# sangminwoo/SVOL

Hardware: AMD Instinct MI355X
Metric: frames/sec (fwd+matcher+bwd), T=32·P=196·d=256 (higher is better)
Workload: dtype bf16

## Files before the change

### svol_amd/csrc/attention_bf16.hip

```cpp
#include <cstdint>
#include <cstdlib>

#include "attn_call.h"

namespace {

constexpr float LOG2E = 1.4426950408889634f;
constexpr int KT = 128;
constexpr int IMG = KT * 64;
constexpr float LAZY_THR = 4.0f;

struct Args {
    const void *q, *k, *v, *o, *d_o;
    void *out_o, *dq, *dk, *dv;
    const float* kbias;
    float *lse2, *delta;
    int64_t ldq, ldk, ldv, ldo, lddo, lddq, lddk, lddv;
    int B, H, Lq, Lk, dh;
    float scale;
    float premul;
    int ksplit, tiles_per_split;
    float *ws_o, *ws_ml, *ws_dq;
    const int* tile_flags;
    int head_xcd, nxt;
    int tail_last;
    int* redo;
    unsigned *nl2, *nd2;
    float drop_p, drop_inv;
    uint64_t drop_seed;
    const int64_t* drop_step;
    int dq_rot;
};
__device__ __forceinline__ float attn_drop(uint64_t seed, uint64_t row, int key, float p, float inv) {
    return dropout_scale(seed, row, (uint32_t)key, p, inv);
}
__device__ __forceinline__ void attn_drop2(uint32_t rowmix, int key0, uint32_t thr16, float inv, float& s0, float& s1) {
    const uint32_t bits = drop_bits(rowmix, (uint32_t)key0 >> 1);
    s0 = drop_pick(bits, 0u, thr16, inv);
    s1 = drop_pick(bits, 1u, thr16, inv);
}

typedef __attribute__((address_space(3))) h16x4* lds_bf16x4_ptr;

__device__ __forceinline__ int img_off(int row, int ch) { return row * 64 + ((ch ^ ((row >> 2) & 3)) << 4); }

struct Stage { uint4 v[2]; };

__device__ __forceinline__ void load_regs(Stage& s, const h16_t* g, int64_t ld, int row0, int limit, int dh, int tid) {
#pragma unroll
    for (int i = 0; i < 2; ++i) {
        const int c = tid + 256 * i, row = c >> 2, ch = c & 3;
        s.v[i] = (row0 + row < limit && ch * 8 < dh) ? *reinterpret_cast<const uint4*>(g + (int64_t)(row0 + row) * ld + ch * 8)
                                                      : make_uint4(0, 0, 0, 0);
    }
}
__device__ __forceinline__ void store_lds(char* img, const Stage& s, int tid) {
#pragma unroll
    for (int i = 0; i < 2; ++i) {
        const int c = tid + 256 * i, row = c >> 2, ch = c & 3;
        *reinterpret_cast<uint4*>(img + img_off(row, ch)) = s.v[i];
    }
}

typedef __attribute__((address_space(3))) void* lds_vptr;
typedef const __attribute__((address_space(1))) void* gbl_vptr;
__device__ __forceinline__ void dma_piece(char* img, const h16_t* g, int64_t ld, int row0, int piece, int lane) {
    const int row = 16 * piece + (lane >> 2);
    const int ch = (lane & 3) ^ ((lane >> 4) & 3);
    const h16_t* src = g + (int64_t)(row0 + row) * ld + ch * 8;
    __builtin_amdgcn_global_load_lds((gbl_vptr)src, (lds_vptr)(img + piece * 1024), 16, 0, 0);
}
__device__ __forceinline__ void dma_tile(char* img, const h16_t* g, int64_t ld, int row0, int wave, int lane) {
    dma_piece(img, g, ld, row0, 2 * wave, lane);
    dma_piece(img, g, ld, row0, 2 * wave + 1, lane);
}
__device__ __forceinline__ void dma_wait_all() { asm volatile("s_waitcnt vmcnt(0)" ::: "memory"); }
__device__ __forceinline__ void dma_piece_async(char* img, const h16_t* g, int64_t ld, int row0, int piece, int lane) {
    const int row = 16 * piece + (lane >> 2);
    const int ch = (lane & 3) ^ ((lane >> 4) & 3);
    const h16_t* src = g + (int64_t)(row0 + row) * ld + ch * 8;
    const unsigned dst = __builtin_amdgcn_readfirstlane((unsigned)(size_t)(lds_vptr)(img + piece * 1024));
    asm volatile("s_mov_b32 m0, %0\n\tglobal_load_lds_dwordx4 %1, off" ::"s"(dst), "v"(src) : "m0");
}
__device__ __forceinline__ void dma_tile_async(char* img, const h16_t* g, int64_t ld, int row0, int wave, int lane) {
    dma_piece_async(img, g, ld, row0, 2 * wave, lane);
    dma_piece_async(img, g, ld, row0, 2 * wave + 1, lane);
}

__device__ __forceinline__ void load_lane_block(uint4 (&out)[2], const h16_t* g, int64_t ld, int row, bool valid, int dh,
                                                int h) {
#pragma unroll
    for (int s = 0; s < 2; ++s) {
        const int d0 = (2 * s + h) * 8;
        out[s] = (valid && d0 < dh) ? *reinterpret_cast<const uint4*>(g + (int64_t)row * ld + d0) : make_uint4(0, 0, 0, 0);
    }
}

__device__ __forceinline__ void read_rows(uint4 (&a)[2], const char* img, int row, int h) {
#pragma unroll
    for (int s = 0; s < 2; ++s) a[s] = *reinterpret_cast<const uint4*>(img + img_off(row, 2 * s + h));
}

__device__ __forceinline__ void read_tr(uint4 (&a)[2], const char* img, int sub, int lane) {
    const int g = lane >> 4, i = lane & 15, q = i >> 2, p = i & 3, hh = g >> 1;
    const int ch = 2 * (g & 1) + (p >> 1), inner = 8 * (p & 1);
#pragma unroll
    for (int s = 0; s < 2; ++s) {
        const int r1 = 32 * sub + 16 * s + 4 * hh + q;
        const h16x4 lo = SVOL_DS_READ_TR16_H16((lds_bf16x4_ptr)(img + img_off(r1, ch) + inner));
        const h16x4 hi = SVOL_DS_READ_TR16_H16((lds_bf16x4_ptr)(img + img_off(r1 + 8, ch) + inner));
        a[s] = __builtin_bit_cast(uint4, __builtin_shufflevector(lo, hi, 0, 1, 2, 3, 4, 5, 6, 7));
    }
}

__device__ __forceinline__ float max3(float a, float b, float c) {
    float r;
    asm("v_max3_f32 %0, %1, %2, %3" : "=v"(r) : "v"(a), "v"(b), "v"(c));
    return r;
}

__device__ __forceinline__ void mfma_results_ready(f32x16& a, f32x16& b, f32x16& c, f32x16& d) {
    asm volatile("s_nop 15\n\ts_nop 3" : "+v"(a), "+v"(b), "+v"(c), "+v"(d));
}

__device__ __forceinline__ void mfma_results_ready2(f32x16& a, f32x16& b) {
    asm volatile("s_nop 15\n\ts_nop 3" : "+v"(a), "+v"(b));
}

__device__ __forceinline__ f32x16 zero16() {
    f32x16 z;
#pragma unroll
    for (int i = 0; i < 16; ++i) z[i] = 0.f;
    return z;
}

__device__ __forceinline__ f32x16 mma_first(const uint4 (&a)[2], const uint4 (&b)[2]) {
    f32x16 acc = zero16();
#pragma unroll
    for (int s = 0; s < 2; ++s)
        acc = SVOL_MFMA_32x32x16_H16(__builtin_bit_cast(h16x8, a[s]), __builtin_bit_cast(h16x8, b[s]), acc, 0, 0,
                                                      0);
    return acc;
}

__device__ __forceinline__ void mma_second(f32x16& acc, const uint4 (&a)[2], const f32x16& x) {
#pragma unroll
    for (int s = 0; s < 2; ++s) {
        h16x8 b;
#pragma unroll
        for (int j = 0; j < 8; j += 2) {
            const h16x2 pr = cvt_pk_h16(x[8 * s + j], x[8 * s + j + 1]);
            b[j] = pr[0];
            b[j + 1] = pr[1];
        }
        acc = SVOL_MFMA_32x32x16_H16(__builtin_bit_cast(h16x8, a[s]), b, acc, 0, 0, 0);
    }
}

__device__ __forceinline__ void store_acc(const f32x16& acc, h16_t* out, int64_t ld, int row, bool valid, int dh, int h,
                                          float mul) {
    if (!valid) return;
#pragma unroll
    for (int g = 0; g < 4; ++g) {
        const int d0 = 8 * g + 4 * h;
        if (d0 < dh) {
            h16x4 v;
#pragma unroll
            for (int e = 0; e < 4; ++e) v[e] = (h16_t)(acc[4 * g + e] * mul);
            *reinterpret_cast<h16x4*>(out + (int64_t)row * ld + d0) = v;
        }
    }
}

__device__ __forceinline__ void stage_bias(float* sb, const float* kb, int row0, int limit, int tid) {
    if (tid < KT) {
        const int key = row0 + tid;
        sb[tid] = key < limit ? (kb ? kb[key] * LOG2E : 0.f) : -INFINITY;
    }
}

template <bool MASKED>
__global__ __launch_bounds__(256, 2) void attn_fwd_bf16(Args p) {
    const uint64_t dseed = drop_seed_at(p.drop_seed, p.drop_step);
    __shared__ __attribute__((aligned(16))) char smem[4 * IMG + 2 * KT * 4];
    char* sK = smem;
    char* sV = smem + 2 * IMG;
    float* sB = reinterpret_cast<float*>(smem + 4 * IMG);

    const int tid = threadIdx.x, lane = tid & 63, wave = tid >> 6;
    const int r = lane & 31, h = lane >> 5;
    const int b = blockIdx.z, hh = blockIdx.y;
    const int qt = blockIdx.x / p.ksplit, sp = blockIdx.x % p.ksplit;
    const int qrow = qt * 128 + wave * 32 + r;
    const bool qvalid = qrow < p.Lq;
    const h16_t* Q = reinterpret_cast<const h16_t*>(p.q) + (int64_t)b * p.Lq * p.ldq + hh * p.dh;
    const h16_t* K = reinterpret_cast<const h16_t*>(p.k) + (int64_t)b * p.Lk * p.ldk + hh * p.dh;
    const h16_t* V = reinterpret_cast<const h16_t*>(p.v) + (int64_t)b * p.Lk * p.ldv + hh * p.dh;
    const float* kb = p.kbias ? p.kbias + (int64_t)b * p.Lk : nullptr;
    const float c = p.premul != 0.f ? 1.f : p.scale * LOG2E;

    uint4 qb[2];
    load_lane_block(qb, Q, p.ldq, qrow, qvalid, p.dh, h);

    float m = -INFINITY, l = 0.f;
    f32x16 O = zero16();

    const int t0 = sp * p.tiles_per_split;
    const int nt = min((p.Lk + KT - 1) / KT, t0 + p.tiles_per_split);
    Stage sk, sv;
    load_regs(sk, K, p.ldk, t0 * KT, p.Lk, p.dh, tid);
    load_regs(sv, V, p.ldv, t0 * KT, p.Lk, p.dh, tid);
    store_lds(sK, sk, tid);
    store_lds(sV, sv, tid);
    if (MASKED) stage_bias(sB, kb, t0 * KT, p.Lk, tid);
    __syncthreads();

    for (int t = t0; t < nt; ++t) {
        const int cur = (t - t0) & 1;
        if (t + 1 < nt) {
            load_regs(sk, K, p.ldk, (t + 1) * KT, p.Lk, p.dh, tid);
            load_regs(sv, V, p.ldv, (t + 1) * KT, p.Lk, p.dh, tid);
        }
        const char* kimg = sK + cur * IMG;
        const char* vimg = sV + cur * IMG;
        const float* bias = sB + cur * KT;
        f32x16 S[4];
#pragma unroll
        for (int sub = 0; sub < 4; ++sub) {
            uint4 ka[2];
            read_rows(ka, kimg, sub * 32 + r, h);
            S[sub] = mma_first(ka, qb);
        }
        mfma_results_ready(S[0], S[1], S[2], S[3]);
        if (MASKED) {
#pragma unroll
            for (int sub = 0; sub < 4; ++sub)
#pragma unroll
                for (int g = 0; g < 4; ++g) {
                    const f32x4 bb = *reinterpret_cast<const f32x4*>(bias + sub * 32 + 8 * g + 4 * h);
#pragma unroll
                    for (int e = 0; e < 4; ++e) S[sub][4 * g + e] = S[sub][4 * g + e] * c + bb[e];
                }
        }
        float ml[4];
#pragma unroll
        for (int sub = 0; sub < 4; ++sub) {
            float mm = max3(S[sub][0], S[sub][1], S[sub][2]);
#pragma unroll
            for (int i = 3; i < 15; i += 2) mm = max3(mm, S[sub][i], S[sub][i + 1]);
            ml[sub] = max3(mm, S[sub][15], mm);
        }
        float mloc = max3(ml[0], ml[1], fmaxf(ml[2], ml[3]));
        {
            const HalfPair sw = swap_halves(__builtin_bit_cast(unsigned, mloc));
            mloc = fmaxf(__builtin_bit_cast(float, sw.lo), __builtin_bit_cast(float, sw.hi));
        }
        const float thr = MASKED ? LAZY_THR : LAZY_THR / c;
        if (__any(mloc > m + thr)) {
            const float m_new = fmaxf(m, mloc);
            const float m_use = (m_new == -INFINITY) ? 0.f : m_new;
            const float alpha = __builtin_amdgcn_exp2f(MASKED ? (m - m_use) : (m - m_use) * c);
            l *= alpha;
#pragma unroll
            for (int i = 0; i < 16; ++i) O[i] *= alpha;
            m = m_new;
        }
        const float m_use = (m == -INFINITY) ? 0.f : m;
        const float mc = MASKED ? -m_use : -m_use * c;
        float ls[4] = {0.f, 0.f, 0.f, 0.f};
#pragma unroll
        for (int sub = 0; sub < 4; ++sub)
#pragma unroll
            for (int i = 0; i < 16; ++i) {
                S[sub][i] = __builtin_amdgcn_exp2f(MASKED ? S[sub][i] + mc : __builtin_fmaf(S[sub][i], c, mc));
                ls[sub] += S[sub][i];
            }
        l += (ls[0] + ls[1]) + (ls[2] + ls[3]);
        if (p.drop_p > 0.f) {
            const uint32_t rm = drop_row(drop_seed32(dseed), (((uint64_t)b * p.H + hh) * p.Lq + (qvalid ? qrow : 0)));
            const uint32_t thr = drop_thr16(p.drop_p);
#pragma unroll
            for (int sub = 0; sub < 4; ++sub)
#pragma unroll
                for (int g = 0; g < 4; ++g)
#pragma unroll
                    for (int e = 0; e < 4; e += 2) {
                        float s0, s1;
                        attn_drop2(rm, t * KT + sub * 32 + 8 * g + 4 * h + e, thr, p.drop_inv, s0, s1);
                        S[sub][4 * g + e] *= s0;
                        S[sub][4 * g + e + 1] *= s1;
                    }
        }
#pragma unroll
        for (int sub = 0; sub < 4; ++sub) {
            uint4 va[2];
            read_tr(va, vimg, sub, lane);
            mma_second(O, va, S[sub]);
        }
        if (t + 1 < nt) {
            store_lds(sK + (cur ^ 1) * IMG, sk, tid);
            store_lds(sV + (cur ^ 1) * IMG, sv, tid);
            if (MASKED) stage_bias(sB + (cur ^ 1) * KT, kb, (t + 1) * KT, p.Lk, tid);
        }
        __syncthreads();
    }
    const float lt = l + __shfl_xor(l, 32, 64);
    const float m2 = MASKED ? m : m * c;
    if (p.ksplit > 1) {
        if (qvalid) {
            float* wo = p.ws_o + (((int64_t)sp * p.B + b) * p.Lq + qrow) * (p.H * p.dh) + hh * p.dh;
#pragma unroll
            for (int g = 0; g < 4; ++g) {
                const int d0 = 8 * g + 4 * h;
                if (d0 < p.dh) *reinterpret_cast<f32x4*>(wo + d0) = f32x4{O[4 * g], O[4 * g + 1], O[4 * g + 2], O[4 * g + 3]};
            }
            if (h == 0) {
                float* wm = p.ws_ml + ((((int64_t)sp * p.B + b) * p.H + hh) * p.Lq + qrow) * 2;
                wm[0] = m2;
                wm[1] = lt;
            }
        }
        return;
    }
    const float inv = lt > 0.f ? 1.f / lt : 0.f;
    h16_t* Oo = reinterpret_cast<h16_t*>(p.out_o) + (int64_t)b * p.Lq * p.ldo + hh * p.dh;
    store_acc(O, Oo, p.ldo, qrow, qvalid, p.dh, h, inv);
    if (qvalid && h == 0) p.lse2[((int64_t)b * p.H + hh) * p.Lq + qrow] = m2 + __builtin_amdgcn_logf(lt);
}

__global__ void attn_combine_bf16(Args p) {
    const int64_t idx = (int64_t)blockIdx.x * blockDim.x + threadIdx.x;
    const int64_t total = (int64_t)p.B * p.Lq * p.H;
    if (idx >= total) return;
    const int hh = (int)(idx % p.H);
    const int64_t row = idx / p.H;
    const int b = (int)(row / p.Lq), q = (int)(row % p.Lq);
    float M = -INFINITY;
    for (int i = 0; i < p.ksplit; ++i) M = fmaxf(M, p.ws_ml[((((int64_t)i * p.B + b) * p.H + hh) * p.Lq + q) * 2]);
    float L = 0.f, acc[32];
#pragma unroll
    for (int d = 0; d < 32; ++d) acc[d] = 0.f;
    for (int i = 0; i < p.ksplit; ++i) {
        const float* ml = p.ws_ml + ((((int64_t)i * p.B + b) * p.H + hh) * p.Lq + q) * 2;
        if (ml[0] == -INFINITY) continue;
        const float w = __builtin_amdgcn_exp2f(ml[0] - M);
        L += w * ml[1];
        const float* po = p.ws_o + (((int64_t)i * p.B + b) * p.Lq + q) * (p.H * p.dh) + hh * p.dh;
#pragma unroll
        for (int d = 0; d < 32; d += 4) {
            if (d < p.dh) {
                const f32x4 t = *reinterpret_cast<const f32x4*>(po + d);
#pragma unroll
                for (int e = 0; e < 4; ++e) acc[d + e] += w * t[e];
            }
        }
    }
    const float inv = L > 0.f ? 1.f / L : 0.f;
    h16_t* o = reinterpret_cast<h16_t*>(p.out_o) + row * p.ldo + hh * p.dh;
#pragma unroll
    for (int d = 0; d < 32; d += 4) {
        if (d < p.dh) {
            h16x4 v;
#pragma unroll
            for (int e = 0; e < 4; ++e) v[e] = (h16_t)(acc[d + e] * inv);
            *reinterpret_cast<h16x4*>(o + d) = v;
        }
    }
    p.lse2[((int64_t)b * p.H + hh) * p.Lq + q] = M + __builtin_amdgcn_logf(L);
}

__global__ void attn_delta_bf16(Args p) {
    const int64_t idx = (int64_t)blockIdx.x * blockDim.x + threadIdx.x;
    const int64_t total = (int64_t)p.B * p.Lq * p.H;
    if (idx >= total) return;
    const int hh = (int)(idx % p.H);
    const int64_t row = idx / p.H;
    const int b = (int)(row / p.Lq), q = (int)(row % p.Lq);
    const h16_t* o = reinterpret_cast<const h16_t*>(p.o) + row * p.ldo + hh * p.dh;
    const h16_t* d = reinterpret_cast<const h16_t*>(p.d_o) + row * p.lddo + hh * p.dh;
    float s = 0.f;
    for (int i = 0; i < p.dh; i += 8) {
        const h16x8 a = *reinterpret_cast<const h16x8*>(o + i), c = *reinterpret_cast<const h16x8*>(d + i);
#pragma unroll
        for (int e = 0; e < 8; ++e) s += (float)a[e] * (float)c[e];
    }
    p.delta[((int64_t)b * p.H + hh) * p.Lq + q] = s;
    if (p.ksplit > 1) {
        float* z = p.ws_dq + row * (p.H * p.dh) + hh * p.dh;
        for (int i = 0; i < p.dh; i += 4) *reinterpret_cast<f32x4*>(z + i) = f32x4{0.f, 0.f, 0.f, 0.f};
    }
}

__global__ void attn_dq_finish_bf16(Args p) {
    const int64_t idx = (int64_t)blockIdx.x * blockDim.x + threadIdx.x;
    const int64_t total = (int64_t)p.B * p.Lq * p.H;
    if (idx >= total) return;
    const int hh = (int)(idx % p.H);
    const int64_t row = idx / p.H;
    const float* z = p.ws_dq + row * (p.H * p.dh) + hh * p.dh;
    h16_t* o = reinterpret_cast<h16_t*>(p.dq) + row * p.lddq + hh * p.dh;
    for (int i = 0; i < p.dh; i += 4) {
        const f32x4 t = *reinterpret_cast<const f32x4*>(z + i);
        h16x4 v;
#pragma unroll
        for (int e = 0; e < 4; ++e) v[e] = (h16_t)(t[e] * p.scale);
        *reinterpret_cast<h16x4*>(o + i) = v;
    }
}

template <bool MASKED>
__global__ __launch_bounds__(256, 2) void attn_bwd_dq_bf16(Args p) {
    const uint64_t dseed = drop_seed_at(p.drop_seed, p.drop_step);
    __shared__ __attribute__((aligned(16))) char smem[4 * IMG + 2 * KT * 4];
    char* sK = smem;
    char* sV = smem + 2 * IMG;
    float* sB = reinterpret_cast<float*>(smem + 4 * IMG);

    const int tid = threadIdx.x, lane = tid & 63, wave = tid >> 6;
    const int r = lane & 31, h = lane >> 5;
    const int b = blockIdx.z, hh = blockIdx.y;
    const int qt = blockIdx.x / p.ksplit, sp = blockIdx.x % p.ksplit;
    const int qrow = qt * 128 + wave * 32 + r;
    const bool qvalid = qrow < p.Lq;
    const h16_t* Q = reinterpret_cast<const h16_t*>(p.q) + (int64_t)b * p.Lq * p.ldq + hh * p.dh;
    const h16_t* dO = reinterpret_cast<const h16_t*>(p.d_o) + (int64_t)b * p.Lq * p.lddo + hh * p.dh;
    const h16_t* K = reinterpret_cast<const h16_t*>(p.k) + (int64_t)b * p.Lk * p.ldk + hh * p.dh;
    const h16_t* V = reinterpret_cast<const h16_t*>(p.v) + (int64_t)b * p.Lk * p.ldv + hh * p.dh;
    const float* kb = p.kbias ? p.kbias + (int64_t)b * p.Lk : nullptr;
    const float c = p.premul != 0.f ? 1.f : p.scale * LOG2E;

    uint4 qb[2], dob[2];
    load_lane_block(qb, Q, p.ldq, qrow, qvalid, p.dh, h);
    load_lane_block(dob, dO, p.lddo, qrow, qvalid, p.dh, h);
    const int64_t sidx = ((int64_t)b * p.H + hh) * p.Lq + qrow;
    const float nlse = qvalid ? -p.lse2[sidx] : -INFINITY;
    const float dl = qvalid ? p.delta[sidx] : 0.f;

    f32x16 dQ = zero16();
    const int t0 = sp * p.tiles_per_split;
    const int nt = min((p.Lk + KT - 1) / KT, t0 + p.tiles_per_split);
    Stage sk, sv;
    load_regs(sk, K, p.ldk, t0 * KT, p.Lk, p.dh, tid);
    load_regs(sv, V, p.ldv, t0 * KT, p.Lk, p.dh, tid);
    store_lds(sK, sk, tid);
    store_lds(sV, sv, tid);
    if (MASKED) stage_bias(sB, kb, t0 * KT, p.Lk, tid);
    __syncthreads();

    for (int t = t0; t < nt; ++t) {
        const int cur = (t - t0) & 1;
        if (t + 1 < nt) {
            load_regs(sk, K, p.ldk, (t + 1) * KT, p.Lk, p.dh, tid);
            load_regs(sv, V, p.ldv, (t + 1) * KT, p.Lk, p.dh, tid);
        }
        const char* kimg = sK + cur * IMG;
        const char* vimg = sV + cur * IMG;
        const float* bias = sB + cur * KT;
#pragma unroll 2
        for (int sub = 0; sub < 4; ++sub) {
            uint4 a[2];
            read_rows(a, kimg, sub * 32 + r, h);
            f32x16 S = mma_first(a, qb);
            read_rows(a, vimg, sub * 32 + r, h);
            f32x16 dP = mma_first(a, dob);
            if (p.drop_p > 0.f) {
                const uint32_t rm = drop_row(drop_seed32(dseed), (((uint64_t)b * p.H + hh) * p.Lq + (qvalid ? qrow : 0)));
                const uint32_t thr = drop_thr16(p.drop_p);
#pragma unroll
                for (int g = 0; g < 4; ++g)
#pragma unroll
                    for (int e = 0; e < 4; e += 2) {
                        float s0, s1;
                        attn_drop2(rm, t * KT + sub * 32 + 8 * g + 4 * h + e, thr, p.drop_inv, s0, s1);
                        dP[4 * g + e] *= s0;
                        dP[4 * g + e + 1] *= s1;
                    }
            }
            if (MASKED) {
#pragma unroll
                for (int g = 0; g < 4; ++g) {
                    const f32x4 bb = *reinterpret_cast<const f32x4*>(bias + sub * 32 + 8 * g + 4 * h);
#pragma unroll
                    for (int e = 0; e < 4; ++e) {
                        const float pe = __builtin_amdgcn_exp2f(__builtin_fmaf(S[4 * g + e], c, bb[e] + nlse));
                        S[4 * g + e] = pe * (dP[4 * g + e] - dl);
                    }
                }
            } else {
#pragma unroll
                for (int i = 0; i < 16; ++i) {
                    const float pe = __builtin_amdgcn_exp2f(__builtin_fmaf(S[i], c, nlse));
                    S[i] = pe * (dP[i] - dl);
                }
            }
            read_tr(a, kimg, sub, lane);
            mma_second(dQ, a, S);
        }
        if (t + 1 < nt) {
            store_lds(sK + (cur ^ 1) * IMG, sk, tid);
            store_lds(sV + (cur ^ 1) * IMG, sv, tid);
            if (MASKED) stage_bias(sB + (cur ^ 1) * KT, kb, (t + 1) * KT, p.Lk, tid);
        }
        __syncthreads();
    }
    if (p.ksplit > 1) {
        if (qvalid) {
            float* z = p.ws_dq + ((int64_t)b * p.Lq + qrow) * (p.H * p.dh) + hh * p.dh;
#pragma unroll
            for (int g = 0; g < 4; ++g) {
                const int d0 = 8 * g + 4 * h;
                if (d0 < p.dh) {
#pragma unroll
                    for (int e = 0; e < 4; ++e) atomicAdd(z + d0 + e, dQ[4 * g + e]);
                }
            }
        }
        return;
    }
    h16_t* dQo = reinterpret_cast<h16_t*>(p.dq) + (int64_t)b * p.Lq * p.lddq + hh * p.dh;
    store_acc(dQ, dQo, p.lddq, qrow, qvalid, p.dh, h, p.scale);
}

template <bool KBIAS>
__global__ __launch_bounds__(256, 2) void attn_bwd_dkdv_bf16(Args p) {
    const uint64_t dseed = drop_seed_at(p.drop_seed, p.drop_step);
    __shared__ __attribute__((aligned(16))) char smem[4 * IMG + 4 * KT * 4];
    char* sQ = smem;
    char* sdO = smem + 2 * IMG;
    float* sL = reinterpret_cast<float*>(smem + 4 * IMG);
    float* sD = sL + 2 * KT;

    const int tid = threadIdx.x, lane = tid & 63, wave = tid >> 6;
    const int r = lane & 31, h = lane >> 5;
    const int b = blockIdx.z, hh = blockIdx.y;
    const int krow = blockIdx.x * 128 + wave * 32 + r;
    const bool kvalid = krow < p.Lk;
    const h16_t* Q = reinterpret_cast<const h16_t*>(p.q) + (int64_t)b * p.Lq * p.ldq + hh * p.dh;
    const h16_t* dO = reinterpret_cast<const h16_t*>(p.d_o) + (int64_t)b * p.Lq * p.lddo + hh * p.dh;
    const h16_t* K = reinterpret_cast<const h16_t*>(p.k) + (int64_t)b * p.Lk * p.ldk + hh * p.dh;
    const h16_t* V = reinterpret_cast<const h16_t*>(p.v) + (int64_t)b * p.Lk * p.ldv + hh * p.dh;
    const float c = p.premul != 0.f ? 1.f : p.scale * LOG2E;
    const float kbl = kvalid ? (p.kbias ? p.kbias[(int64_t)b * p.Lk + krow] * LOG2E : 0.f) : -INFINITY;
    const float* lse_g = p.lse2 + ((int64_t)b * p.H + hh) * p.Lq;
    const float* dl_g = p.delta + ((int64_t)b * p.H + hh) * p.Lq;

    uint4 kbk[2], vbk[2];
    load_lane_block(kbk, K, p.ldk, krow, kvalid, p.dh, h);
    load_lane_block(vbk, V, p.ldv, krow, kvalid, p.dh, h);

    f32x16 dK = zero16(), dV = zero16();
    const int nt = (p.Lq + KT - 1) / KT;
    Stage sq, sdo;
    float rl = 0.f, rd = 0.f;
    auto load_stats = [&](int row0) {
        if (tid < KT) {
            const int qi = row0 + tid;
            rl = qi < p.Lq ? -lse_g[qi] : -INFINITY;
            rd = qi < p.Lq ? dl_g[qi] : 0.f;
        }
    };
    auto store_stats = [&](int buf) {
        if (tid < KT) { sL[buf * KT + tid] = rl; sD[buf * KT + tid] = rd; }
    };
    load_regs(sq, Q, p.ldq, 0, p.Lq, p.dh, tid);
    load_regs(sdo, dO, p.lddo, 0, p.Lq, p.dh, tid);
    load_stats(0);
    store_lds(sQ, sq, tid);
    store_lds(sdO, sdo, tid);
    store_stats(0);
    __syncthreads();

    for (int t = 0; t < nt; ++t) {
        const int cur = t & 1;
        if (t + 1 < nt) {
            load_regs(sq, Q, p.ldq, (t + 1) * KT, p.Lq, p.dh, tid);
            load_regs(sdo, dO, p.lddo, (t + 1) * KT, p.Lq, p.dh, tid);
            load_stats((t + 1) * KT);
        }
        const char* qimg = sQ + cur * IMG;
        const char* doimg = sdO + cur * IMG;
        const float* nl = sL + cur * KT;
        const float* dd = sD + cur * KT;
#pragma unroll 1
        for (int sub = 0; sub < 4; ++sub) {
            uint4 a[2];
            read_rows(a, qimg, sub * 32 + r, h);
            f32x16 S = mma_first(a, kbk);
#pragma unroll
            for (int g = 0; g < 4; ++g) {
                const f32x4 ls = *reinterpret_cast<const f32x4*>(nl + sub * 32 + 8 * g + 4 * h);
#pragma unroll
                for (int e = 0; e < 4; ++e)
                    S[4 * g + e] = __builtin_amdgcn_exp2f(__builtin_fmaf(S[4 * g + e], c, KBIAS ? kbl + ls[e] : ls[e]));
            }
            read_tr(a, doimg, sub, lane);
            f32x16 MS;
#pragma unroll
            for (int i = 0; i < 16; ++i) MS[i] = 1.f;
            if (p.drop_p > 0.f) {
                const uint32_t s0 = drop_seed32(dseed), thr = drop_thr16(p.drop_p), odd = (uint32_t)lane & 1u;
                const uint64_t rbase = ((uint64_t)b * p.H + hh) * p.Lq;
                const bool rows32 = rbase + (uint64_t)p.Lq <= 0xffffffffull;
#pragma unroll
                for (int g = 0; g < 4; ++g)
#pragma unroll
                    for (int e = 0; e < 4; e += 2) {
                        const int q0 = t * KT + sub * 32 + 8 * g + 4 * h + e;
                        const int qm = min(q0 + (int)odd, p.Lq - 1);
                        const uint32_t rm = rows32 ? (s0 ^ (((uint32_t)rbase + (uint32_t)qm) * 0x9E3779B1u)) : drop_row(s0, rbase + (uint64_t)qm);
                        const uint32_t mine = drop_bits(rm, (uint32_t)krow >> 1);
                        const uint32_t other = (uint32_t)__builtin_amdgcn_mov_dpp((int)mine, 0xB1, 0xf, 0xf, true);
                        MS[4 * g + e] = drop_pick(odd ? other : mine, odd, thr, p.drop_inv);
                        MS[4 * g + e + 1] = drop_pick(odd ? mine : other, odd, thr, p.drop_inv);
                    }
                f32x16 Pd = S;
#pragma unroll
                for (int i = 0; i < 16; ++i) Pd[i] *= MS[i];
                mma_second(dV, a, Pd);
            } else {
                mma_second(dV, a, S);
            }
            read_rows(a, doimg, sub * 32 + r, h);
            f32x16 dP = mma_first(a, vbk);
            if (p.drop_p > 0.f) {
#pragma unroll
                for (int i = 0; i < 16; ++i) dP[i] *= MS[i];
            }
#pragma unroll
            for (int g = 0; g < 4; ++g) {
                const f32x4 dl = *reinterpret_cast<const f32x4*>(dd + sub * 32 + 8 * g + 4 * h);
#pragma unroll
                for (int e = 0; e < 4; ++e) S[4 * g + e] = S[4 * g + e] * (dP[4 * g + e] - dl[e]);
            }
            read_tr(a, qimg, sub, lane);
            mma_second(dK, a, S);
        }
        if (t + 1 < nt) {
            store_lds(sQ + (cur ^ 1) * IMG, sq, tid);
            store_lds(sdO + (cur ^ 1) * IMG, sdo, tid);
            store_stats(cur ^ 1);
        }
        __syncthreads();
    }
    h16_t* dKo = reinterpret_cast<h16_t*>(p.dk) + (int64_t)b * p.Lk * p.lddk + hh * p.dh;
    h16_t* dVo = reinterpret_cast<h16_t*>(p.dv) + (int64_t)b * p.Lk * p.lddv + hh * p.dh;
    store_acc(dK, dKo, p.lddk, krow, kvalid, p.dh, h, p.premul != 0.f ? p.scale / p.premul : p.scale);
    store_acc(dV, dVo, p.lddv, krow, kvalid, p.dh, h, 1.f);
}

__device__ __forceinline__ f32x16 splat16(float x) {
    f32x16 z;
#pragma unroll
    for (int i = 0; i < 16; ++i) z[i] = x;
    return z;
}
__device__ __forceinline__ f32x16 mma_first_c(const uint4 (&a)[2], const uint4 (&b)[2], const f32x16& c0) {
    f32x16 acc;
    asm("s_nop 1\n\tv_mfma_f32_32x32x16_" SVOL_H16_ASM " %0, %1, %2, %3"
        : "=&v"(acc)
        : "v"(__builtin_bit_cast(h16x8, a[0])), "v"(__builtin_bit_cast(h16x8, b[0])), "v"(c0));
    return SVOL_MFMA_32x32x16_H16(__builtin_bit_cast(h16x8, a[1]), __builtin_bit_cast(h16x8, b[1]), acc, 0, 0,
                                                   0);
}
__device__ __forceinline__ f32x16 rows16(const float* v, int sub, int h) {
    f32x16 z;

#pragma unroll
    for (int g = 0; g < 4; ++g) {
        const f32x4 t = *reinterpret_cast<const f32x4*>(v + sub * 32 + 8 * g + 4 * h);
#pragma unroll
        for (int e = 0; e < 4; ++e) z[4 * g + e] = t[e];
    }
    return z;
}

__device__ __forceinline__ void block_coords(const Args& p, int& xt, int& hh, int& b) {
    if (p.head_xcd) {
        const int id = blockIdx.x, xcd = id & 7, slot = id >> 3;
        int hl;
        const int two = p.head_xcd == 2 ? 2 : 1;
        if (p.tail_last) {
            const int nfull = p.nxt - 1, hpx = (p.B * p.H) >> 3;
            if (slot < hpx * nfull) {
                const int g = slot / (two * nfull), r = slot - g * two * nfull;
                hl = g * two + (two == 2 ? (r & 1) : 0);
                xt = two == 2 ? (r >> 1) : r;
            } else { hl = slot - hpx * nfull; xt = nfull; }
        } else {
            const int g = slot / (two * p.nxt), r = slot - g * two * p.nxt;
            hl = g * two + (two == 2 ? (r & 1) : 0);
            xt = two == 2 ? (r >> 1) : r;
        }
        const int head = p.head_xcd == 2 ? (((hl >> 1) * 8 + xcd) * 2 + (hl & 1)) : hl * 8 + xcd;
        hh = head % p.H;
        b = head / p.H;
    } else {
        xt = blockIdx.x;
        hh = blockIdx.y;
        b = blockIdx.z;
    }
}

__device__ __forceinline__ unsigned split_bf16x2(float x) {
    const h16_t hi = (h16_t)x;
    const float rem = x - (float)hi;
    const h16_t lo = (h16_t)rem;
    return (unsigned)__builtin_bit_cast(unsigned short, hi) | ((unsigned)__builtin_bit_cast(unsigned short, lo) << 16);
}

__device__ __forceinline__ float key_bias_log2(const float* kb, int key, int Lk) {
    return key < Lk ? (kb ? kb[key] * LOG2E : 0.f) : -INFINITY;
}
__device__ __forceinline__ f32x16 add_key_bias(const f32x16& S, const float* kb, int key, int Lk, int h) {
    const float bv = key_bias_log2(kb, key, Lk);
    const unsigned pair = bv == -INFINITY ? SVOL_H16_NINF_LO : split_bf16x2(bv);
    const uint4 a = h == 0 ? make_uint4(pair, 0u, 0u, 0u) : make_uint4(0u, 0u, 0u, 0u);
    const uint4 o = h == 0 ? make_uint4(SVOL_H16_ONE2, 0u, 0u, 0u) : make_uint4(0u, 0u, 0u, 0u);
    return SVOL_MFMA_32x32x16_H16(__builtin_bit_cast(h16x8, a), __builtin_bit_cast(h16x8, o), S, 0, 0, 0);
}
__global__ __launch_bounds__(64) void attn_tile_flags_bf16(const float* __restrict__ kbias, int Lk, int nt, int* __restrict__ flags) {
    const int t = blockIdx.x, b = blockIdx.y, lane = threadIdx.x;
    const float* kb = kbias ? kbias + (int64_t)b * Lk : nullptr;
    const float b0 = key_bias_log2(kb, t * KT + lane, Lk), b1 = key_bias_log2(kb, t * KT + 64 + lane, Lk);
    int flag = 0;
    if (__any(b0 != 0.f || b1 != 0.f)) flag = __all(b0 == -INFINITY && b1 == -INFINITY) ? 2 : 1;
    if (lane == 0) flags[(int64_t)b * nt + t] = flag;
}

template <bool MASKED>
__device__ __forceinline__ void attn_fwd_pre_body(const Args p) {
    __shared__ __attribute__((aligned(16))) char smem[4 * IMG];
    char* sK = smem;
    char* sV = smem + 2 * IMG;
    const int tid = threadIdx.x, lane = tid & 63, wave = tid >> 6;
    const int r = lane & 31, h = lane >> 5;
    int xt, hh, b;
    block_coords(p, xt, hh, b);
    const int qrow = xt * 128 + wave * 32 + r;
    const bool qvalid = qrow < p.Lq;
    const h16_t* Q = reinterpret_cast<const h16_t*>(p.q) + (int64_t)b * p.Lq * p.ldq + hh * p.dh;
    const h16_t* K = reinterpret_cast<const h16_t*>(p.k) + (int64_t)b * p.Lk * p.ldk + hh * p.dh;
    const h16_t* V = reinterpret_cast<const h16_t*>(p.v) + (int64_t)b * p.Lk * p.ldv + hh * p.dh;
    const float* kb = (MASKED && p.kbias) ? p.kbias + (int64_t)b * p.Lk : nullptr;

    uint4 qb[2];
    load_lane_block(qb, Q, p.ldq, qrow, qvalid, p.dh, h);
    float m = 0.f, l = 0.f;
    f32x16 O = zero16();
    f32x16 Cm = zero16();
    bool started = false;

    const int nt = MASKED ? (p.Lk + KT - 1) / KT : p.Lk / KT;
    Stage sk, sv;
    load_regs(sk, K, p.ldk, 0, p.Lk, p.dh, tid);
    load_regs(sv, V, p.ldv, 0, p.Lk, p.dh, tid);
    const int* fl = MASKED ? p.tile_flags + (int64_t)b * nt : nullptr;
    unsigned long long mixed = 0, dead = 0;
    store_lds(sK, sk, tid);
    store_lds(sV, sv, tid);
    __syncthreads();
    for (int t = 0; t < nt; ++t) {
        const int cur = t & 1;
        if (t + 1 < nt) {
            load_regs(sk, K, p.ldk, (t + 1) * KT, p.Lk, p.dh, tid);
            load_regs(sv, V, p.ldv, (t + 1) * KT, p.Lk, p.dh, tid);
        }
        if (MASKED && (t & 63) == 0) {
            const int f = (t + lane < nt) ? fl[t + lane] : 2;
            mixed = __ballot(f == 1);
            dead = __ballot(f == 2);
        }
        const int flag = MASKED ? (int)((mixed >> (t & 63)) & 1) + 2 * (int)((dead >> (t & 63)) & 1) : 0;
        if (!MASKED || flag != 2) {
            const char* kimg = sK + cur * IMG;
            const char* vimg = sV + cur * IMG;
            f32x16 S[4];
#pragma unroll
            for (int sub = 0; sub < 4; ++sub) {
                uint4 ka[2];
                read_rows(ka, kimg, sub * 32 + r, h);
                S[sub] = mma_first_c(ka, qb, Cm);
            }
            if (MASKED && flag == 1) {
#pragma unroll
                for (int sub = 0; sub < 4; ++sub) S[sub] = add_key_bias(S[sub], kb, t * KT + sub * 32 + r, p.Lk, h);
            }
            mfma_results_ready(S[0], S[1], S[2], S[3]);
            float ml[4];
#pragma unroll
            for (int sub = 0; sub < 4; ++sub) {
                float mm = max3(S[sub][0], S[sub][1], S[sub][2]);
#pragma unroll
                for (int i = 3; i < 15; i += 2) mm = max3(mm, S[sub][i], S[sub][i + 1]);
                ml[sub] = max3(mm, S[sub][15], mm);
            }
            float mloc = max3(ml[0], ml[1], fmaxf(ml[2], ml[3]));
            {
                const HalfPair sw = swap_halves(__builtin_bit_cast(unsigned, mloc));
                mloc = fmaxf(__builtin_bit_cast(float, sw.lo), __builtin_bit_cast(float, sw.hi));
            }
            const bool first = MASKED ? !started : (t == 0);
            if (first || __any(mloc > LAZY_THR)) {
                const float dm = first ? mloc : fmaxf(mloc, 0.f);
                if (!first) {
                    const float alpha = __builtin_amdgcn_exp2f(-dm);
                    l *= alpha;
#pragma unroll
                    for (int i = 0; i < 16; ++i) O[i] *= alpha;
                }
                m += dm;
                Cm = splat16(-m);
#pragma unroll
                for (int sub = 0; sub < 4; ++sub)
#pragma unroll
                    for (int i = 0; i < 16; ++i) S[sub][i] -= dm;
            }
            started = true;
            float ls[4] = {0.f, 0.f, 0.f, 0.f};
#pragma unroll
            for (int sub = 0; sub < 4; ++sub)
#pragma unroll
                for (int i = 0; i < 16; ++i) {
                    S[sub][i] = __builtin_amdgcn_exp2f(S[sub][i]);
                    ls[sub] += S[sub][i];
                }
            l += (ls[0] + ls[1]) + (ls[2] + ls[3]);
#pragma unroll
            for (int sub = 0; sub < 4; ++sub) {
                uint4 va[2];
                read_tr(va, vimg, sub, lane);
                mma_second(O, va, S[sub]);
            }
        }
        if (t + 1 < nt) {
            store_lds(sK + (cur ^ 1) * IMG, sk, tid);
            store_lds(sV + (cur ^ 1) * IMG, sv, tid);
        }
        __syncthreads();
    }
    const float lt = l + __shfl_xor(l, 32, 64);
    const float inv = lt > 0.f ? 1.f / lt : 0.f;
    h16_t* Oo = reinterpret_cast<h16_t*>(p.out_o) + (int64_t)b * p.Lq * p.ldo + hh * p.dh;
    store_acc(O, Oo, p.ldo, qrow, qvalid, p.dh, h, inv);
    if (qvalid && h == 0) p.lse2[((int64_t)b * p.H + hh) * p.Lq + qrow] = m + __builtin_amdgcn_logf(lt);
}
__global__ __launch_bounds__(256, 2) void attn_fwd_bf16_pre(Args p) {
    __shared__ __attribute__((aligned(16))) char smem[4 * IMG];
    if (p.redo && !p.redo[blockIdx.x]) return;
    char* sK = smem;
    char* sV = smem + 2 * IMG;
    const int tid = threadIdx.x, lane = tid & 63, wave = tid >> 6;
    const int r = lane & 31, h = lane >> 5;
    int xt, hh, b;
    block_coords(p, xt, hh, b);
    const int qrow = xt * 128 + wave * 32 + r;
    const bool qvalid = qrow < p.Lq;
    const h16_t* Q = reinterpret_cast<const h16_t*>(p.q) + (int64_t)b * p.Lq * p.ldq + hh * p.dh;
    const h16_t* K = reinterpret_cast<const h16_t*>(p.k) + (int64_t)b * p.Lk * p.ldk + hh * p.dh;
    const h16_t* V = reinterpret_cast<const h16_t*>(p.v) + (int64_t)b * p.Lk * p.ldv + hh * p.dh;

    uint4 qb[2];
    load_lane_block(qb, Q, p.ldq, qrow, qvalid, p.dh, h);
    float m = 0.f, l = 0.f;
    f32x16 O = zero16();
    f32x16 Cm = zero16();

    const int nt = p.Lk / KT;
    Stage sk, sv;
    load_regs(sk, K, p.ldk, 0, p.Lk, p.dh, tid);
    load_regs(sv, V, p.ldv, 0, p.Lk, p.dh, tid);
    store_lds(sK, sk, tid);
    store_lds(sV, sv, tid);
    __syncthreads();
    for (int t = 0; t < nt; ++t) {
        const int cur = t & 1;
        if (t + 1 < nt) {
            load_regs(sk, K, p.ldk, (t + 1) * KT, p.Lk, p.dh, tid);
            load_regs(sv, V, p.ldv, (t + 1) * KT, p.Lk, p.dh, tid);
        }
        const char* kimg = sK + cur * IMG;
        const char* vimg = sV + cur * IMG;
        f32x16 S[4];
#pragma unroll
        for (int sub = 0; sub < 4; ++sub) {
            uint4 ka[2];
            read_rows(ka, kimg, sub * 32 + r, h);
            S[sub] = mma_first_c(ka, qb, Cm);
        }
        mfma_results_ready(S[0], S[1], S[2], S[3]);
        float ml[4];
#pragma unroll
        for (int sub = 0; sub < 4; ++sub) {
            float mm = max3(S[sub][0], S[sub][1], S[sub][2]);
#pragma unroll
            for (int i = 3; i < 15; i += 2) mm = max3(mm, S[sub][i], S[sub][i + 1]);
            ml[sub] = max3(mm, S[sub][15], mm);
        }
        float mloc = max3(ml[0], ml[1], fmaxf(ml[2], ml[3]));
        {
            const HalfPair sw = swap_halves(__builtin_bit_cast(unsigned, mloc));
            mloc = fmaxf(__builtin_bit_cast(float, sw.lo), __builtin_bit_cast(float, sw.hi));
        }
        if (t == 0 || __any(mloc > LAZY_THR)) {
            const float dm = (t == 0) ? mloc : fmaxf(mloc, 0.f);
            if (t != 0) {
                const float alpha = __builtin_amdgcn_exp2f(-dm);
                l *= alpha;
#pragma unroll
                for (int i = 0; i < 16; ++i) O[i] *= alpha;
            }
            m += dm;
            Cm = splat16(-m);
#pragma unroll
            for (int sub = 0; sub < 4; ++sub)
#pragma unroll
                for (int i = 0; i < 16; ++i) S[sub][i] -= dm;
        }
        float ls[4] = {0.f, 0.f, 0.f, 0.f};
#pragma unroll
        for (int sub = 0; sub < 4; ++sub)
#pragma unroll
            for (int i = 0; i < 16; ++i) {
                S[sub][i] = __builtin_amdgcn_exp2f(S[sub][i]);
                ls[sub] += S[sub][i];
            }
        l += (ls[0] + ls[1]) + (ls[2] + ls[3]);
#pragma unroll
        for (int sub = 0; sub < 4; ++sub) {
            uint4 va[2];
            read_tr(va, vimg, sub, lane);
            mma_second(O, va, S[sub]);
        }
        if (t + 1 < nt) {
            store_lds(sK + (cur ^ 1) * IMG, sk, tid);
            store_lds(sV + (cur ^ 1) * IMG, sv, tid);
        }
        __syncthreads();
    }
    const float lt = l + __shfl_xor(l, 32, 64);
    const float inv = lt > 0.f ? 1.f / lt : 0.f;
    h16_t* Oo = reinterpret_cast<h16_t*>(p.out_o) + (int64_t)b * p.Lq * p.ldo + hh * p.dh;
    store_acc(O, Oo, p.ldo, qrow, qvalid, p.dh, h, inv);
    if (qvalid && h == 0) p.lse2[((int64_t)b * p.H + hh) * p.Lq + qrow] = m + __builtin_amdgcn_logf(lt);
}
__global__ __launch_bounds__(256, 2) void attn_fwd_bf16_pre_masked(Args p) { attn_fwd_pre_body<true>(p); }

__device__ __forceinline__ f32x16 mma_c_first(const uint4& a0, const uint4& b0, const f32x16& c0) {
    f32x16 acc;
    asm("s_nop 1\n\tv_mfma_f32_32x32x16_" SVOL_H16_ASM " %0, %1, %2, %3"
        : "=&v"(acc)
        : "v"(__builtin_bit_cast(h16x8, a0)), "v"(__builtin_bit_cast(h16x8, b0)), "v"(c0));
    return acc;
}
__device__ __forceinline__ f32x16 mma_acc(const uint4& a1, const uint4& b1, const f32x16& acc) {
    return SVOL_MFMA_32x32x16_H16(__builtin_bit_cast(h16x8, a1), __builtin_bit_cast(h16x8, b1), acc, 0, 0, 0);
}
template <int LO>
__device__ __forceinline__ void ds_chunk(f32x16& S, const f32x16& dP) {
#pragma unroll
    for (int i = LO; i < LO + 4; i += 2) {
        const f32x2 e = {__builtin_amdgcn_exp2f(S[i]), __builtin_amdgcn_exp2f(S[i + 1])};
        const f32x2 d = {dP[i], dP[i + 1]};
        const f32x2 m = e * d;
        S[i] = m[0];
        S[i + 1] = m[1];
    }
}
#define SVOL_FENCE() __builtin_amdgcn_sched_barrier(0)
__device__ __forceinline__ void dq_phase(f32x16& Sn, f32x16& dPn, const uint4 (&ka)[2], const uint4 (&va)[2], const uint4 (&qbn)[2],
                                         const uint4 (&dobn)[2], const f32x16& Cln, const f32x16& Cdn, f32x16& Sc, const f32x16& dPc,
                                         f32x16& dQc, const uint4 (&kt)[2]) {
    Sn = mma_c_first(ka[0], qbn[0], Cln);
    SVOL_FENCE();
    ds_chunk<0>(Sc, dPc);
    SVOL_FENCE();
    Sn = mma_acc(ka[1], qbn[1], Sn);
    SVOL_FENCE();
    ds_chunk<4>(Sc, dPc);
    SVOL_FENCE();
    dPn = mma_c_first(va[0], dobn[0], Cdn);
    SVOL_FENCE();
    ds_chunk<8>(Sc, dPc);
    SVOL_FENCE();
    dPn = mma_acc(va[1], dobn[1], dPn);
    SVOL_FENCE();
    ds_chunk<12>(Sc, dPc);
    SVOL_FENCE();
    mma_second(dQc, kt, Sc);
}
__device__ __forceinline__ void dq_finish(f32x16& Sc, const f32x16& dPc, f32x16& dQc, const uint4 (&kt)[2]) {
    ds_chunk<0>(Sc, dPc);
    ds_chunk<4>(Sc, dPc);
    ds_chunk<8>(Sc, dPc);
    ds_chunk<12>(Sc, dPc);
    mma_second(dQc, kt, Sc);
}

template <bool MASKED>
__device__ __forceinline__ void attn_bwd_dq_pre_body(const Args& p) {
    __shared__ __attribute__((aligned(16))) char smem[4 * IMG];
    char* sK = smem;
    char* sV = smem + 2 * IMG;
    const int tid = threadIdx.x, lane = tid & 63, wave = tid >> 6;
// ... 126 lines not shown
    hh = __builtin_amdgcn_readfirstlane(hh);
    b = __builtin_amdgcn_readfirstlane(b);
    const h16_t* Q = reinterpret_cast<const h16_t*>(p.q) + (int64_t)b * p.Lq * p.ldq + hh * p.dh;
    const h16_t* dO = reinterpret_cast<const h16_t*>(p.d_o) + (int64_t)b * p.Lq * p.lddo + hh * p.dh;
    const h16_t* O = reinterpret_cast<const h16_t*>(p.o) + (int64_t)b * p.Lq * p.ldo + hh * p.dh;
    const h16_t* K = reinterpret_cast<const h16_t*>(p.k) + (int64_t)b * p.Lk * p.ldk + hh * p.dh;
    const h16_t* V = reinterpret_cast<const h16_t*>(p.v) + (int64_t)b * p.Lk * p.ldv + hh * p.dh;
    dma_tile(sK, K, p.ldk, 0, wave, lane);
    dma_tile(sV, V, p.ldv, 0, wave, lane);

    int qrow[2];
    bool qvalid[2];
    uint4 qb[2][2], dob[2][2];
    f32x16 Cl[2], Cd[2], dQ[2];
    const bool single = p.Lq - xt * 256 <= 128;
#pragma unroll
    for (int u = 0; u < 2; ++u) {
        qrow[u] = single ? (u == 0 ? xt * 256 + wave * 32 + r : p.Lq) : xt * 256 + wave * 64 + u * 32 + r;
        qvalid[u] = qrow[u] < p.Lq;
        load_lane_block(qb[u], Q, p.ldq, qrow[u], qvalid[u], p.dh, h);
        load_lane_block(dob[u], dO, p.lddo, qrow[u], qvalid[u], p.dh, h);
        const int64_t sidx = ((int64_t)b * p.H + hh) * p.Lq + qrow[u];
        Cl[u] = splat16(qvalid[u] ? -p.lse2[sidx] : -INFINITY);
        float dl = 0.f;
        {
            uint4 ob[2];
            load_lane_block(ob, O, p.ldo, qrow[u], qvalid[u], p.dh, h);
#pragma unroll
            for (int s_ = 0; s_ < 2; ++s_) {
                const h16x8 a = __builtin_bit_cast(h16x8, ob[s_]), c = __builtin_bit_cast(h16x8, dob[u][s_]);
#pragma unroll
                for (int e = 0; e < 8; ++e) dl += (float)a[e] * (float)c[e];
            }
            const HalfPair sw = swap_halves(__builtin_bit_cast(unsigned, dl));
            dl = __builtin_bit_cast(float, sw.lo) + __builtin_bit_cast(float, sw.hi);
        }
        if (qvalid[u] && h == 0) {
            p.delta[sidx] = dl;
            if (p.nl2) {
                p.nl2[sidx] = split_bf16x2(-p.lse2[sidx]);
                p.nd2[sidx] = split_bf16x2(-dl);
            }
        }
        Cd[u] = splat16(qvalid[u] ? -dl : 0.f);
        dQ[u] = zero16();
    }
    const int nt = p.Lk / KT;
    dma_wait_all();
    __syncthreads();
    f32x16 S0, S1, dP0, dP1;
    uint4 ka[2], va[2];
    read_rows(ka, sK, r, h);
    read_rows(va, sV, r, h);
    S0 = mma_first_c(ka, qb[0], Cl[0]);
    dP0 = mma_first_c(va, dob[0], Cd[0]);
    for (int t = 0; t < nt; ++t) {
        const int cur = t & 1;
        const bool more = t + 1 < nt;
        if (more) {
            dma_tile_async(sK + (cur ^ 1) * IMG, K, p.ldk, (t + 1) * KT, wave, lane);
            dma_tile_async(sV + (cur ^ 1) * IMG, V, p.ldv, (t + 1) * KT, wave, lane);
        }
        const char* kimg = sK + cur * IMG;
        const char* vimg = sV + cur * IMG;
#pragma unroll
        for (int sub = 0; sub < 4; ++sub) {
            uint4 kt[2];
            read_tr(kt, kimg, sub, lane);
            dq_phase(S1, dP1, ka, va, qb[1], dob[1], Cl[1], Cd[1], S0, dP0, dQ[0], kt);
            if (sub < 3) {
                read_rows(ka, kimg, (sub + 1) * 32 + r, h);
                read_rows(va, vimg, (sub + 1) * 32 + r, h);
                dq_phase(S0, dP0, ka, va, qb[0], dob[0], Cl[0], Cd[0], S1, dP1, dQ[1], kt);
            } else {
                dma_wait_all();
                __syncthreads();
                if (more) {
                    read_rows(ka, sK + (cur ^ 1) * IMG, r, h);
                    read_rows(va, sV + (cur ^ 1) * IMG, r, h);
                    dq_phase(S0, dP0, ka, va, qb[0], dob[0], Cl[0], Cd[0], S1, dP1, dQ[1], kt);
                } else {
                    dq_finish(S1, dP1, dQ[1], kt);
                }
            }
        }
    }
    h16_t* dQo = reinterpret_cast<h16_t*>(p.dq) + (int64_t)b * p.Lq * p.lddq + hh * p.dh;
    int tid_e = threadIdx.x;
    asm volatile("" : "+v"(tid_e));
    const int r_e = tid_e & 31, h_e = (tid_e >> 5) & 1, wave_e = tid_e >> 6;
#pragma unroll
    for (int u = 0; u < 2; ++u) {
        const int qrow_e = single ? (u == 0 ? xt * 256 + wave_e * 32 + r_e : p.Lq) : xt * 256 + wave_e * 64 + u * 32 + r_e;
        store_acc(dQ[u], dQo, p.lddq, qrow_e, qrow_e < p.Lq, p.dh, h_e, p.scale);
    }
}

template <bool MASKED, bool DMA = false>
__device__ __forceinline__ void attn_bwd_dkdv_pre_body(const Args& p) {
    __shared__ __attribute__((aligned(16))) char smem[4 * IMG + 4 * KT * 4];
    char* sQ = smem;
    char* sdO = smem + 2 * IMG;
    unsigned* sL = reinterpret_cast<unsigned*>(smem + 4 * IMG);
    unsigned* sD = sL + 2 * KT;
    const int tid = threadIdx.x, lane = tid & 63, wave = DMA ? __builtin_amdgcn_readfirstlane(tid >> 6) : (tid >> 6);
    const int r = lane & 31, h = lane >> 5;
    int xt, hh, b;
    block_coords(p, xt, hh, b);
    const int krow = xt * 128 + wave * 32 + r;
    const bool kvalid = krow < p.Lk;
    const h16_t* Q = reinterpret_cast<const h16_t*>(p.q) + (int64_t)b * p.Lq * p.ldq + hh * p.dh;
    const h16_t* dO = reinterpret_cast<const h16_t*>(p.d_o) + (int64_t)b * p.Lq * p.lddo + hh * p.dh;
    const h16_t* K = reinterpret_cast<const h16_t*>(p.k) + (int64_t)b * p.Lk * p.ldk + hh * p.dh;
    const h16_t* V = reinterpret_cast<const h16_t*>(p.v) + (int64_t)b * p.Lk * p.ldv + hh * p.dh;
    const float* lse_g = p.lse2 + ((int64_t)b * p.H + hh) * p.Lq;
    const float* dl_g = p.delta + ((int64_t)b * p.H + hh) * p.Lq;

    uint4 kbk[2], vbk[2];
    load_lane_block(kbk, K, p.ldk, krow, kvalid, p.dh, h);
    load_lane_block(vbk, V, p.ldv, krow, kvalid, p.dh, h);
    f32x16 dK = zero16(), dV = zero16();
    const int nt = (p.Lq + KT - 1) / KT;
    Stage sq, sdo;
    float rl = 0.f, rd = 0.f;
    auto load_stats = [&](int row0) {
        if (tid < KT) {
            const int qi = row0 + tid;
            rl = qi < p.Lq ? -lse_g[qi] : SVOL_H16_NEG_BIG;
            rd = qi < p.Lq ? -dl_g[qi] : 0.f;
        }
    };
    auto store_stats = [&](int buf) {
        if (tid < KT) { sL[buf * KT + tid] = split_bf16x2(rl); sD[buf * KT + tid] = split_bf16x2(rd); }
    };
    const uint4 ones = h == 0 ? make_uint4(SVOL_H16_ONE2, 0u, 0u, 0u) : make_uint4(0u, 0u, 0u, 0u);
    float kbl = 0.f;
    if (MASKED) kbl = kvalid ? (p.kbias ? p.kbias[(int64_t)b * p.Lk + krow] * LOG2E : 0.f) : -INFINITY;
    const bool wave_dead = MASKED && __all(kbl == -INFINITY);
    const unsigned kb_pair = kbl == -INFINITY ? SVOL_H16_NINF_LO : split_bf16x2(kbl);
    const uint4 ones_s = (MASKED && h == 0) ? make_uint4(SVOL_H16_ONE2, kb_pair, 0u, 0u) : ones;
    const unsigned q_one = MASKED ? SVOL_H16_ONE2 : 0u;
    const unsigned* nl_h = DMA ? p.nl2 + ((int64_t)b * p.H + hh) * p.Lq : nullptr;
    const unsigned* nd_h = DMA ? p.nd2 + ((int64_t)b * p.H + hh) * p.Lq : nullptr;
    auto dma_stats = [&](int buf, int row0) {
        if (wave < 2 && lane < 32) {
            const unsigned* src = (wave == 0 ? nl_h : nd_h) + row0 + lane * 4;
            unsigned* dst = (wave == 0 ? sL : sD) + buf * KT;
            __builtin_amdgcn_global_load_lds((gbl_vptr)src, (lds_vptr)dst, 16, 0, 0);
        }
    };
    auto dma_stats_async = [&](int buf, int row0) {
        if (wave < 2) {
            const unsigned* src = (wave == 0 ? nl_h : nd_h) + row0 + (lane & 31) * 4;
            const unsigned dst = __builtin_amdgcn_readfirstlane((unsigned)(size_t)(lds_vptr)((wave == 0 ? sL : sD) + buf * KT));
            if (lane < 32) asm volatile("s_mov_b32 m0, %0\n\tglobal_load_lds_dwordx4 %1, off" ::"s"(dst), "v"(src) : "m0");
        }
    };
    if (DMA) {
        dma_tile(sQ, Q, p.ldq, 0, wave, lane);
        dma_tile(sdO, dO, p.lddo, 0, wave, lane);
        dma_stats(0, 0);
        dma_wait_all();
    } else {
        load_regs(sq, Q, p.ldq, 0, p.Lq, p.dh, tid);
        load_regs(sdo, dO, p.lddo, 0, p.Lq, p.dh, tid);
        load_stats(0);
        store_lds(sQ, sq, tid);
        store_lds(sdO, sdo, tid);
        store_stats(0);
    }
    __syncthreads();
    for (int t = 0; t < nt; ++t) {
        const int cur = t & 1;
        if (t + 1 < nt) {
            if (DMA) {
                dma_tile_async(sQ + (cur ^ 1) * IMG, Q, p.ldq, (t + 1) * KT, wave, lane);
                dma_tile_async(sdO + (cur ^ 1) * IMG, dO, p.lddo, (t + 1) * KT, wave, lane);
                dma_stats_async(cur ^ 1, (t + 1) * KT);
            } else {
                load_regs(sq, Q, p.ldq, (t + 1) * KT, p.Lq, p.dh, tid);
                load_regs(sdo, dO, p.lddo, (t + 1) * KT, p.Lq, p.dh, tid);
                load_stats((t + 1) * KT);
            }
        }
        const char* qimg = sQ + cur * IMG;
        const char* doimg = sdO + cur * IMG;
        const unsigned* nl = sL + cur * KT;
        const unsigned* nd = sD + cur * KT;
        auto first_products = [&](int sub, f32x16& S, f32x16& dP) {
            uint4 a[2];
            const uint4 el = make_uint4(nl[sub * 32 + r], q_one, 0u, 0u);
            const uint4 ed = make_uint4(nd[sub * 32 + r], 0u, 0u, 0u);
            read_rows(a, qimg, sub * 32 + r, h);
            S = SVOL_MFMA_32x32x16_H16(__builtin_bit_cast(h16x8, el), __builtin_bit_cast(h16x8, ones_s),
                                                        zero16(), 0, 0, 0);
            S = SVOL_MFMA_32x32x16_H16(__builtin_bit_cast(h16x8, a[0]), __builtin_bit_cast(h16x8, kbk[0]), S, 0, 0, 0);
            S = SVOL_MFMA_32x32x16_H16(__builtin_bit_cast(h16x8, a[1]), __builtin_bit_cast(h16x8, kbk[1]), S, 0, 0, 0);
            read_rows(a, doimg, sub * 32 + r, h);
            dP = SVOL_MFMA_32x32x16_H16(__builtin_bit_cast(h16x8, ed), __builtin_bit_cast(h16x8, ones),
                                                         zero16(), 0, 0, 0);
            dP = SVOL_MFMA_32x32x16_H16(__builtin_bit_cast(h16x8, a[0]), __builtin_bit_cast(h16x8, vbk[0]), dP, 0, 0, 0);
            dP = SVOL_MFMA_32x32x16_H16(__builtin_bit_cast(h16x8, a[1]), __builtin_bit_cast(h16x8, vbk[1]), dP, 0, 0, 0);
        };
        f32x16 S, dP, Sn, dPn;
        if (!wave_dead) first_products(0, S, dP);
#pragma unroll
        for (int sub = 0; sub < (wave_dead ? 0 : 4); ++sub) {
            if (sub + 1 < 4) first_products(sub + 1, Sn, dPn);
            uint4 a[2];
#pragma unroll
            for (int i = 0; i < 16; ++i) S[i] = __builtin_amdgcn_exp2f(S[i]);
            read_tr(a, doimg, sub, lane);
            mma_second(dV, a, S);
#pragma unroll
            for (int i = 0; i < 16; i += 2) {
                const f32x2 m = f32x2{S[i], S[i + 1]} * f32x2{dP[i], dP[i + 1]};
                S[i] = m[0];
                S[i + 1] = m[1];
            }
            read_tr(a, qimg, sub, lane);
            mma_second(dK, a, S);
            if (sub + 1 < 4) { S = Sn; dP = dPn; }
        }
        if (t + 1 < nt && !DMA) {
            store_lds(sQ + (cur ^ 1) * IMG, sq, tid);
            store_lds(sdO + (cur ^ 1) * IMG, sdo, tid);
            store_stats(cur ^ 1);
        }
        if (DMA) dma_wait_all();
        __syncthreads();
    }
    h16_t* dKo = reinterpret_cast<h16_t*>(p.dk) + (int64_t)b * p.Lk * p.lddk + hh * p.dh;
    h16_t* dVo = reinterpret_cast<h16_t*>(p.dv) + (int64_t)b * p.Lk * p.lddv + hh * p.dh;
    store_acc(dK, dKo, p.lddk, krow, kvalid, p.dh, h, p.scale / p.premul);
    store_acc(dV, dVo, p.lddv, krow, kvalid, p.dh, h, 1.f);
}
__global__ __launch_bounds__(256, 2) void attn_bwd_dkdv_bf16_pre(Args p) { attn_bwd_dkdv_pre_body<false>(p); }
__global__ __launch_bounds__(256, 2) void attn_bwd_dkdv_bf16_pre_dma(Args p) { attn_bwd_dkdv_pre_body<false, true>(p); }
__global__ __launch_bounds__(256, 2) void attn_bwd_dkdv_bf16_pre_masked(Args p) { attn_bwd_dkdv_pre_body<true>(p); }

constexpr int SP_KB = 4;
constexpr int SP_WKEYS = 32 * SP_KB;
constexpr int SP_KEYS = 4 * SP_WKEYS;
constexpr int SP_PART = 4 * 4 * 64 * 16;
constexpr int SP_LDS = 4 * IMG + 4 * IMG + 2 * SP_PART + 4 * KT * 4 + 512;

__device__ __forceinline__ int ds_off(int key, int g, int half) {
    return key * 64 + ((g ^ ((key >> 2) & 3)) << 4) + ((half ^ ((key >> 1) & 1)) << 3);
}
__device__ __forceinline__ void read_tr_nat(uint4 (&a)[2], const char* img, int sub, int lane) {
    const int g = lane >> 4, i = lane & 15, q = i >> 2, p = i & 3, hh = g >> 1;
    const int ch = 2 * (g & 1) + (p >> 1), inner = 8 * (p & 1);
#pragma unroll
    for (int s = 0; s < 2; ++s) {
        const int r1 = 32 * sub + 16 * s + 8 * hh + q;
        const h16x4 lo = SVOL_DS_READ_TR16_H16((lds_bf16x4_ptr)(img + img_off(r1, ch) + inner));
        const h16x4 hi = SVOL_DS_READ_TR16_H16((lds_bf16x4_ptr)(img + img_off(r1 + 4, ch) + inner));
        a[s] = __builtin_bit_cast(uint4, __builtin_shufflevector(lo, hi, 0, 1, 2, 3, 4, 5, 6, 7));
    }
}
__device__ __forceinline__ void read_ds_tr(uint4 (&a)[2], const char* img, int lane) {
    const int gg = lane >> 4, i = lane & 15, qq = i >> 2, p = i & 3, hh = gg >> 1;
    const int g = 2 * (gg & 1) + (p >> 1), half = p & 1;
#pragma unroll
    for (int s = 0; s < 2; ++s) {
        const int key = 16 * s + 8 * hh + qq;
        const h16x4 lo = SVOL_DS_READ_TR16_H16((lds_bf16x4_ptr)(img + ds_off(key, g, half)));
        const h16x4 hi = SVOL_DS_READ_TR16_H16((lds_bf16x4_ptr)(img + ds_off(key + 4, g, half)));
        a[s] = __builtin_bit_cast(uint4, __builtin_shufflevector(lo, hi, 0, 1, 2, 3, 4, 5, 6, 7));
    }
}
__device__ __forceinline__ void pack16(uint4 (&o)[2], const f32x16& x) {
#pragma unroll
    for (int s = 0; s < 2; ++s) {
        h16x8 b;
#pragma unroll
        for (int j = 0; j < 8; j += 2) {
            const h16x2 pr = cvt_pk_h16(x[8 * s + j], x[8 * s + j + 1]);
            b[j] = pr[0];
            b[j + 1] = pr[1];
        }
        o[s] = __builtin_bit_cast(uint4, b);
    }
}
__device__ __forceinline__ void mma_packed(f32x16& acc, const uint4 (&a)[2], const uint4 (&b)[2]) {
#pragma unroll
    for (int s = 0; s < 2; ++s)
        acc = SVOL_MFMA_32x32x16_H16(__builtin_bit_cast(h16x8, a[s]), __builtin_bit_cast(h16x8, b[s]), acc, 0, 0, 0);
}
__device__ __forceinline__ void sp_barrier() { asm volatile("s_waitcnt lgkmcnt(0)\n\ts_barrier" ::: "memory"); }

template <bool KBIAS>
__global__ __launch_bounds__(256, 2) void attn_bwd_fq_bf16(Args p) {
    __shared__ __attribute__((aligned(16))) char smem[3 * IMG + 2 * KT * 4 + 4 * 2048];
    char* sQ = smem;
    char* sdO = smem + IMG;
    char* sK = smem + 2 * IMG;
    float* sL = reinterpret_cast<float*>(smem + 3 * IMG);
    float* sD = sL + KT;
    char* sT = smem + 3 * IMG + 2 * KT * 4;
    float* sRed = reinterpret_cast<float*>(smem);
    const int tid = threadIdx.x, lane = tid & 63, wave = tid >> 6;
    const int r = lane & 31, h = lane >> 5;
    const int b = blockIdx.z, hh = blockIdx.y;
    const h16_t* Q = reinterpret_cast<const h16_t*>(p.q) + (int64_t)b * p.Lq * p.ldq + hh * 32;
    const h16_t* dO = reinterpret_cast<const h16_t*>(p.d_o) + (int64_t)b * p.Lq * p.lddo + hh * 32;
    const h16_t* K = reinterpret_cast<const h16_t*>(p.k) + (int64_t)b * p.Lk * p.ldk + hh * 32;
    const h16_t* V = reinterpret_cast<const h16_t*>(p.v) + (int64_t)b * p.Lk * p.ldv + hh * 32;
    h16_t* dKo = reinterpret_cast<h16_t*>(p.dk) + (int64_t)b * p.Lk * p.lddk + hh * 32;
    h16_t* dVo = reinterpret_cast<h16_t*>(p.dv) + (int64_t)b * p.Lk * p.lddv + hh * 32;
    const float c = p.premul != 0.f ? 1.f : p.scale * LOG2E;
    const float kmul = p.premul != 0.f ? p.scale / p.premul : p.scale;
    const int nsub = (p.Lq + 31) >> 5;
    const int ntk = (p.Lk + KT - 1) / KT;
    const int t0 = blockIdx.x * p.tiles_per_split, t1 = min(ntk, t0 + p.tiles_per_split);
    Stage st;
    {
        Stage sq, sdo;
        load_regs(sq, Q, p.ldq, 0, p.Lq, 32, tid);
        load_regs(sdo, dO, p.lddo, 0, p.Lq, 32, tid);
        load_regs(st, K, p.ldk, t0 * KT, p.Lk, 32, tid);
        if (tid < KT) {
            const int64_t si = ((int64_t)b * p.H + hh) * p.Lq + tid;
            sL[tid] = tid < p.Lq ? -p.lse2[si] : -INFINITY;
            sD[tid] = tid < p.Lq ? p.delta[si] : 0.f;
        }
        store_lds(sQ, sq, tid);
        store_lds(sdO, sdo, tid);
        store_lds(sK, st, tid);
    }
    __syncthreads();
    f32x16 dQ[4];
#pragma unroll
    for (int i = 0; i < 4; ++i) dQ[i] = zero16();
    char* img = sT + wave * 2048;
    for (int t = t0; t < t1; ++t) {
        const int krow = t * KT + wave * 32 + r;
        const bool kvalid = krow < p.Lk;
        uint4 kbk[2], vbk[2], kd[2];
        read_rows(kbk, sK, wave * 32 + r, h);
        read_tr_nat(kd, sK, wave, lane);
        load_lane_block(vbk, V, p.ldv, krow, kvalid, 32, h);
        if (t + 1 < t1) load_regs(st, K, p.ldk, (t + 1) * KT, p.Lk, 32, tid);
        float kbl = kvalid ? 0.f : -INFINITY;
        if (KBIAS && kvalid) kbl = p.kbias[(int64_t)b * p.Lk + krow] * LOG2E;
        f32x16 dKa = zero16(), dVa = zero16();
        if (!__all(kbl == -INFINITY)) {
#pragma unroll
            for (int sub = 0; sub < 4; ++sub) {
                if (sub >= nsub) break;
                uint4 a[2];
                read_rows(a, sQ, sub * 32 + r, h);
                f32x16 S = mma_first(a, kbk);
#pragma unroll
                for (int g = 0; g < 4; ++g) {
                    const f32x4 ls = *reinterpret_cast<const f32x4*>(sL + sub * 32 + 8 * g + 4 * h);
#pragma unroll
                    for (int e = 0; e < 4; ++e) S[4 * g + e] = __builtin_amdgcn_exp2f(__builtin_fmaf(S[4 * g + e], c, kbl + ls[e]));
                }
                read_tr(a, sdO, sub, lane);
                mma_second(dVa, a, S);
                read_rows(a, sdO, sub * 32 + r, h);
                const f32x16 dP = mma_first(a, vbk);
#pragma unroll
                for (int g = 0; g < 4; ++g) {
                    const f32x4 dl = *reinterpret_cast<const f32x4*>(sD + sub * 32 + 8 * g + 4 * h);
#pragma unroll
                    for (int e = 0; e < 4; ++e) S[4 * g + e] = S[4 * g + e] * (dP[4 * g + e] - dl[e]);
                }
                uint4 ds[2];
                pack16(ds, S);
                read_tr(a, sQ, sub, lane);
                mma_packed(dKa, a, ds);
                *reinterpret_cast<uint2*>(img + ds_off(r, 0, h)) = make_uint2(ds[0].x, ds[0].y);
                *reinterpret_cast<uint2*>(img + ds_off(r, 1, h)) = make_uint2(ds[0].z, ds[0].w);
                *reinterpret_cast<uint2*>(img + ds_off(r, 2, h)) = make_uint2(ds[1].x, ds[1].y);
                *reinterpret_cast<uint2*>(img + ds_off(r, 3, h)) = make_uint2(ds[1].z, ds[1].w);
                __builtin_amdgcn_fence(__ATOMIC_RELEASE, "wavefront");
                __builtin_amdgcn_wave_barrier();
                __builtin_amdgcn_fence(__ATOMIC_ACQUIRE, "wavefront");
                read_ds_tr(a, img, lane);
                mma_packed(dQ[sub], a, kd);
                __builtin_amdgcn_wave_barrier();
            }
        }
        store_acc(dKa, dKo, p.lddk, krow, kvalid, 32, h, kmul);
        store_acc(dVa, dVo, p.lddv, krow, kvalid, 32, h, 1.f);
        __syncthreads();
        if (t + 1 < t1) {
            store_lds(sK, st, tid);
            __syncthreads();
        }
    }
#pragma unroll
    for (int sub = 0; sub < 4; ++sub) {
        if (sub >= nsub) break;
#pragma unroll
        for (int g = 0; g < 4; ++g)
#pragma unroll
            for (int e = 0; e < 4; ++e) sRed[(wave * 32 + 8 * g + 4 * h + e) * 32 + r] = dQ[sub][4 * g + e];
        __syncthreads();
        {
            const int row = tid >> 3, d0 = (tid & 7) * 4;
            f32x4 v = *reinterpret_cast<const f32x4*>(sRed + row * 32 + d0);
#pragma unroll
            for (int w = 1; w < 4; ++w) {
                const f32x4 u = *reinterpret_cast<const f32x4*>(sRed + (w * 32 + row) * 32 + d0);
#pragma unroll
                for (int e = 0; e < 4; ++e) v[e] += u[e];
            }
            const int q = sub * 32 + row;
            if (q < p.Lq) {
                float* z = p.ws_dq + ((int64_t)b * p.Lq + q) * (p.H * 32) + hh * 32 + d0;
#pragma unroll
                for (int e = 0; e < 4; ++e) unsafeAtomicAdd(z + e, v[e]);
            }
        }
        __syncthreads();
    }
}

template <bool ZERO>
__global__ __launch_bounds__(256) void attn_bwd_sp_prep_bf16(Args p) {
    __shared__ float s_lse[8][33], s_dl[8][33];
    const int tid = threadIdx.x;
    const int64_t row0 = (int64_t)blockIdx.x * 32;
    const int b = (int)(row0 / p.Lq), q0 = (int)(row0 % p.Lq);
    {
        const int hh = tid >> 5, rl = tid & 31;
        if (hh < p.H) s_lse[hh][rl] = p.lse2[((int64_t)b * p.H + hh) * p.Lq + q0 + rl];
    }
    const int rl = tid >> 3, hh = tid & 7;
    float dl = 0.f;
    if (hh < p.H) {
        const int64_t row = row0 + rl;
        const h16_t* o = reinterpret_cast<const h16_t*>(p.o) + row * p.ldo + hh * 32;
        const h16_t* d = reinterpret_cast<const h16_t*>(p.d_o) + row * p.lddo + hh * 32;
#pragma unroll
        for (int i = 0; i < 32; i += 8) {
            const h16x8 a = *reinterpret_cast<const h16x8*>(o + i), c = *reinterpret_cast<const h16x8*>(d + i);
#pragma unroll
            for (int e = 0; e < 8; ++e) dl += (float)a[e] * (float)c[e];
        }
        if constexpr (ZERO) {
            float* z = p.ws_dq + row * (p.H * 32) + hh * 32;
#pragma unroll
            for (int i = 0; i < 32; i += 4) *reinterpret_cast<f32x4*>(z + i) = f32x4{0.f, 0.f, 0.f, 0.f};
        }
        s_dl[hh][rl] = dl;
    }
    __syncthreads();
    {
        const int h2 = tid >> 5, r2 = tid & 31;
        if (h2 < p.H) {
            const int64_t si = ((int64_t)b * p.H + h2) * p.Lq + q0 + r2;
            reinterpret_cast<float*>(p.nl2)[si] = -s_lse[h2][r2];
            reinterpret_cast<float*>(p.nd2)[si] = -s_dl[h2][r2];
            p.delta[si] = s_dl[h2][r2];
        }
    }
}
__global__ __launch_bounds__(256) void attn_dq_round_bf16(Args p) {
    const int64_t i = ((int64_t)blockIdx.x * blockDim.x + threadIdx.x) * 8;
    const int64_t W = (int64_t)p.H * 32, total = (int64_t)p.B * p.Lq * W;
    if (i >= total) {
        const int tk = p.Lk % (4 * 128);
        const int64_t j = i - ((total + 2047) / 2048) * 2048;
        if (tk == 0 || j < 0 || j >= (int64_t)p.B * p.H * 2 * tk * 32) return;
        const int64_t per = (int64_t)2 * tk * 32;
        const int bh = (int)(j / per), rem = (int)(j % per), kv = rem / (tk * 32), key = (rem / 32) % tk, d0 = rem % 32;
        const float* src = p.ws_dq + total + (int64_t)bh * 4 * per + rem;
        f32x4 a = {0.f, 0.f, 0.f, 0.f}, c = a;
#pragma unroll
        for (int part = 0; part < 4; ++part) { a += *reinterpret_cast<const f32x4*>(src + part * per); c += *reinterpret_cast<const f32x4*>(src + part * per + 4); }
        const float mul = kv == 0 ? p.scale / p.premul : 1.f;
        h16x8 v;
#pragma unroll
        for (int e = 0; e < 4; ++e) { v[e] = (h16_t)(a[e] * mul); v[4 + e] = (h16_t)(c[e] * mul); }
        const int b_ = bh / p.H, hh_ = bh % p.H;
        const int64_t row = (int64_t)b_ * p.Lk + (p.Lk - tk) + key;
        h16_t* o = kv == 0 ? reinterpret_cast<h16_t*>(p.dk) + row * p.lddk : reinterpret_cast<h16_t*>(p.dv) + row * p.lddv;
        *reinterpret_cast<h16x8*>(o + hh_ * 32 + d0) = v;
        return;
    }
    const int64_t row = i / W, c = i % W;
    const f32x4 a = *reinterpret_cast<const f32x4*>(p.ws_dq + i), b = *reinterpret_cast<const f32x4*>(p.ws_dq + i + 4);
    h16x8 v;
#pragma unroll
    for (int e = 0; e < 4; ++e) { v[e] = (h16_t)(a[e] * p.scale); v[4 + e] = (h16_t)(b[e] * p.scale); }
    *reinterpret_cast<h16x8*>(reinterpret_cast<h16_t*>(p.dq) + row * p.lddq + c) = v;
}

__global__ __launch_bounds__(256) void attn_sp_zero_image(float* __restrict__ z, int64_t n4) {
    const int64_t stride = (int64_t)gridDim.x * 256;
    for (int64_t i = (int64_t)blockIdx.x * 256 + threadIdx.x; i < n4; i += stride)
        reinterpret_cast<f32x4*>(z)[i] = f32x4{0.f, 0.f, 0.f, 0.f};
}

typedef __attribute__((ext_vector_type(4))) unsigned u32x4;
__device__ __forceinline__ u32x4 to_acc(u32x4 r) {
    asm volatile("; operand -> AGPR" : "+a"(r));
    return r;
}
__device__ __forceinline__ u32x4 as_u32x4(const uint4& v) { return u32x4{v.x, v.y, v.z, v.w}; }
#define SP_FENCE() __builtin_amdgcn_sched_barrier(0)
__device__ __forceinline__ void sp_mfma_c(f32x16& d, const uint4& a, const u32x4& b, const f32x16& c) {
    asm volatile("v_mfma_f32_32x32x16_" SVOL_H16_ASM " %0, %1, %2, %3" : "=&v"(d) : "v"(as_u32x4(a)), "a"(b), "v"(c));
}
__device__ __forceinline__ void sp_mfma_z(f32x16& d, const uint4& a, const u32x4& b) {
    asm volatile("v_mfma_f32_32x32x16_" SVOL_H16_ASM " %0, %1, %2, 0" : "=&v"(d) : "v"(as_u32x4(a)), "a"(b));
}
__device__ __forceinline__ void sp_mfma_v(f32x16& d, const uint4& a, const u32x4& b) {
    asm volatile("v_mfma_f32_32x32x16_" SVOL_H16_ASM " %0, %1, %2, %0" : "+v"(d) : "v"(as_u32x4(a)), "a"(b));
}
__device__ __forceinline__ void sp_mfma_a(f32x16& acc, const uint4& a, const u32x4& b) {
    asm volatile("v_mfma_f32_32x32x16_" SVOL_H16_ASM " %0, %1, %2, %0" : "+a"(acc) : "v"(as_u32x4(a)), "v"(b));
}
__device__ __forceinline__ unsigned cvt_pk_u32(float a, float b) { return __builtin_bit_cast(unsigned, cvt_pk_h16(a, b)); }

struct SpStep {
    uint4 qa[2], doa[2];
    f32x16 Cl, Cd;
};
constexpr int SP_OFF_Q = 4 * KT * 4 + 512;
constexpr int SP_OFF_T = SP_OFF_Q + 4 * IMG;
constexpr int SP_OFF_P = SP_OFF_Q + 8 * IMG;

template <int NKB>
__device__ __forceinline__ void attn_bwd_sp_body(const Args& p, char* smem, int hh, int b, int kbase, int t_begin, int t_end, float* tail_out) {
    float* sL = reinterpret_cast<float*>(smem);
    float* sD = sL + 2 * KT;
    float* sNeg = sL + 4 * KT;
    char* sQ = smem + SP_OFF_Q;
    char* sPart = smem + SP_OFF_P;
    const int tid = threadIdx.x, lane = tid & 63, wave = __builtin_amdgcn_readfirstlane(tid >> 6);
    const int r = lane & 31, h = lane >> 5;
    constexpr int dqw = 8 * 32;
    const h16_t* Q = reinterpret_cast<const h16_t*>(p.q) + (int64_t)b * p.Lq * p.ldq + hh * 32;
    const h16_t* dO = reinterpret_cast<const h16_t*>(p.d_o) + (int64_t)b * p.Lq * p.lddo + hh * 32;
    const h16_t* K = reinterpret_cast<const h16_t*>(p.k) + (int64_t)b * p.Lk * p.ldk + hh * 32;
    const h16_t* V = reinterpret_cast<const h16_t*>(p.v) + (int64_t)b * p.Lk * p.ldv + hh * 32;
    const float* nl_g = reinterpret_cast<const float*>(p.nl2) + ((int64_t)b * p.H + hh) * p.Lq;
    const float* nd_g = reinterpret_cast<const float*>(p.nd2) + ((int64_t)b * p.H + hh) * p.Lq;
    const int key0 = kbase + wave * 32 * NKB;
    char* sT = smem + SP_OFF_T + wave * IMG;
    const int ntl = t_end - t_begin;

    u32x4 kbk[NKB][2], vbk[NKB][2], kd[NKB][2];
    f32x16 dK[NKB], dV[NKB];
    {
        char* sS = sQ + wave * IMG;
#pragma unroll
        for (int pc = 0; pc < 2 * NKB; ++pc) dma_piece(sS, K, p.ldk, key0, pc, lane);
        dma_wait_all();
#pragma unroll
        for (int kb = 0; kb < NKB; ++kb) {
            uint4 t0[2], t1[2];
            read_rows(t0, sS, kb * 32 + r, h);
            read_tr_nat(t1, sS, kb, lane);
#pragma unroll
            for (int s = 0; s < 2; ++s) { kbk[kb][s] = to_acc(as_u32x4(t0[s])); kd[kb][s] = to_acc(as_u32x4(t1[s])); }
        }
        asm volatile("s_waitcnt lgkmcnt(0)" ::: "memory");
#pragma unroll
        for (int pc = 0; pc < 2 * NKB; ++pc) dma_piece(sS, V, p.ldv, key0, pc, lane);
        dma_wait_all();
#pragma unroll
        for (int kb = 0; kb < NKB; ++kb) {
            uint4 t0[2];
            read_rows(t0, sS, kb * 32 + r, h);
#pragma unroll
            for (int s = 0; s < 2; ++s) vbk[kb][s] = to_acc(as_u32x4(t0[s]));
        }
        asm volatile("s_waitcnt lgkmcnt(0)" ::: "memory");
#pragma unroll
        for (int kb = 0; kb < NKB; ++kb) {
            dK[kb] = zero16();
            dV[kb] = zero16();
            asm volatile("; accumulators -> AGPR" : "+a"(dK[kb]), "+a"(dV[kb]));
        }
    }
#pragma unroll
    for (int buf = 0; buf < 2; ++buf)
#pragma unroll
        for (int g = 0; g < 4; ++g)
            *reinterpret_cast<f32x4*>(sPart + buf * SP_PART + ((wave * 4 + g) * 64 + lane) * 16) = f32x4{0.f, 0.f, 0.f, 0.f};
    if (tid < KT) sNeg[tid] = -INFINITY;

    const int prow = t_begin * KT + 32 * wave + (lane >> 2), pch = ((lane & 3) ^ ((lane >> 4) & 3)) * 8;
    const h16_t* gq = Q + (int64_t)prow * p.ldq + pch;
    const h16_t* gdo = dO + (int64_t)prow * p.lddo + pch;
    const float* gst = (wave < 2 ? nl_g : nd_g) + t_begin * KT + (wave & 1) * 64 + (lane & 15) * 4;
    const unsigned lds_q = (unsigned)(size_t)(lds_vptr)sQ + wave * 2048, lds_st = (unsigned)(size_t)(lds_vptr)((wave < 2 ? sL : sD) + (wave & 1) * 64);
    auto dma_tile_at = [&](int tl, int buf) {
        const h16_t* a = gq + (int64_t)tl * KT * p.ldq;
        const h16_t* c = gdo + (int64_t)tl * KT * p.lddo;
        const unsigned dq_ = __builtin_amdgcn_readfirstlane(lds_q + buf * IMG), dd_ = dq_ + 2 * IMG;
        asm volatile("s_mov_b32 m0, %0\n\tglobal_load_lds_dwordx4 %1, off" ::"s"(dq_), "v"(a) : "m0");
        asm volatile("s_mov_b32 m0, %0\n\tglobal_load_lds_dwordx4 %1, off" ::"s"(dq_ + 1024), "v"(a + 16 * p.ldq) : "m0");
        asm volatile("s_mov_b32 m0, %0\n\tglobal_load_lds_dwordx4 %1, off" ::"s"(dd_), "v"(c) : "m0");
        asm volatile("s_mov_b32 m0, %0\n\tglobal_load_lds_dwordx4 %1, off" ::"s"(dd_ + 1024), "v"(c + 16 * p.lddo) : "m0");
        const unsigned ds_ = __builtin_amdgcn_readfirstlane(lds_st + buf * KT * 4);
        const float* e = gst + tl * KT;
        if (lane < 16) asm volatile("s_mov_b32 m0, %0\n\tglobal_load_lds_dwordx4 %1, off" ::"s"(ds_), "v"(e) : "m0");
    };
    const unsigned o_rows0 = img_off(r, h), o_rows1 = img_off(r, 2 + h);
    unsigned o_trl, o_trh;
    {
        const int g = lane >> 4, i = lane & 15, q = i >> 2, pp = i & 3, h2 = g >> 1;
        const int ch = 2 * (g & 1) + (pp >> 1), inner = 8 * (pp & 1);
        o_trl = img_off(4 * h2 + q, ch) + inner;
        o_trh = img_off(4 * h2 + q + 8, ch) + inner;
    }
    const unsigned o_st = 16 * h;
    auto tr_pair = [&](uint4 (&a)[2], const char* img) {
#pragma unroll
        for (int s = 0; s < 2; ++s) {
            const h16x4 lo = SVOL_DS_READ_TR16_H16((lds_bf16x4_ptr)(img + o_trl + 1024 * s));
// ... 382 lines not shown
            SP4_E(S, 7); SP4_M(1); SP4_M(2); SP4_M(3); SP4_CD(0); SP4_CP(2);
            SP4_MF(sp_mfma_v(Sn, qa[1], kbk[kn][1]));
            if (kb == 1) *reinterpret_cast<f32x4*>(sPart + ((sub - 1) & 1) * SP_PART + ((wave * 4 + 2) * 64 + lane) * 16) = f32x4{dQp[8], dQp[9], dQp[10], dQp[11]};
            if (kb == 2) load_c2(Cd, cdn, 0);
            if (kb == 3) {
                float* dst = dq_base + (int64_t)min(max(st - 2, 0), last_step) * 32 * dqw + dq_lane;
                unsafeAtomicAdd(dst + 2 * dqw, rsum[2]);
                unsafeAtomicAdd(dst + 3 * dqw, rsum[3]);
            }
            SP_FENCE();
            SP4_E(S, 8); SP4_E(S, 9); SP4_M(4); SP4_M(5); SP4_CD(1);
            SP4_MF(sp_mfma_v(dPn, doa[1], vbk[kn][1]));
            SP4_W(0);
            if (kb == 2) load_c1(Cd, cdn, 2);
            SP_FENCE();
            SP4_CP(3); SP4_E(S, 10); SP4_M(6); SP4_M(7); SP4_CD(2);
            SP4_MF(sp_mfma_a(dV[kb], dot[0], pw0));
            if (kb == 1) *reinterpret_cast<f32x4*>(sPart + ((sub - 1) & 1) * SP_PART + ((wave * 4 + 3) * 64 + lane) * 16) = f32x4{dQp[12], dQp[13], dQp[14], dQp[15]};
            if (kb == 2) {
                load_c1(Cd, cdn, 3);
                qa[0] = *reinterpret_cast<const uint4*>(qn + o_rows0);
            }
            if (kb == 3) tr_one(dot[0], qn + 2 * IMG, 0);
            SP_FENCE();
            SP4_E(S, 11); SP4_E(S, 12); SP4_CD(3); SP4_CP(4); SP4_M(8);
            SP4_MF(if (ks == 0) sp_mfma_z(dQp, dsa[0], kd[0][0]); else sp_mfma_v(dQp, dsa[0], kd[ks][0]));
            SP4_W(1);
            if (kb == 2) qa[1] = *reinterpret_cast<const uint4*>(qn + o_rows1);
            SP_FENCE();
            SP4_E(S, 13); SP4_M(9); SP4_M(10); SP4_M(11); SP4_CD(4); SP4_CP(5);
            SP4_MF(sp_mfma_a(dK[kb], qt[0], dw0));
            if (kb == 1) {
                red[0] = *reinterpret_cast<const f32x4*>(pr_base + (sub & 1) * SP_PART + 0 * 4 * 64 * 16);
                red[1] = *reinterpret_cast<const f32x4*>(pr_base + (sub & 1) * SP_PART + 1 * 4 * 64 * 16);
            }
            if (kb == 2) {
                doa[0] = *reinterpret_cast<const uint4*>(qn + 2 * IMG + o_rows0);
                doa[1] = *reinterpret_cast<const uint4*>(qn + 2 * IMG + o_rows1);
            }
            if (kb == 3) tr_one(qt[0], qn, 0);
            SP_FENCE();
            SP4_E(S, 14); SP4_E(S, 15); SP4_M(12); SP4_M(13); SP4_CD(5);
            SP4_MF(sp_mfma_v(dQp, dsa[1], kd[ks][1]));
            SP4_W(2);
            SP_FENCE();
            SP4_CP(6); SP4_CP(7); SP4_M(14); SP4_M(15); SP4_CD(6);
            if (kb == 2) { SP4_ADD(rsum, red[0], red[1]); }
            SP4_MF(sp_mfma_a(dV[kb], dot[1], pw1));
            if (kb == 1) {
                red[2] = *reinterpret_cast<const f32x4*>(pr_base + (sub & 1) * SP_PART + 2 * 4 * 64 * 16);
                red[3] = *reinterpret_cast<const f32x4*>(pr_base + (sub & 1) * SP_PART + 3 * 4 * 64 * 16);
            }
            if (kb == 3) tr_one(dot[1], qn + 2 * IMG, 1);
            SP_FENCE();
            SP4_CD(7); SP4_E(Sn, 0); SP4_E(Sn, 1);
            if (kb == 2) { SP4_ADD(rsum, rsum, red[2]); }
            SP4_MF(sp_mfma_a(dK[kb], qt[1], dw1));
            SP4_W(3);
            ds_tr_one(dsa[0], img, 0);
            SP_FENCE();
            SP4_E(Sn, 2); SP4_E(Sn, 3); SP4_E(Sn, 4);
            if (kb == 2) { SP4_ADD(rsum, rsum, red[3]); }
            S = Sn;
            dP = dPn;
        }
        if (sub == 2 && tl >= 1) asm volatile("s_waitcnt vmcnt(12)" ::: "memory");
        asm volatile("s_waitcnt lgkmcnt(8)\n\ts_barrier" ::: "memory");
        }
    }
#undef SP4_E
#undef SP4_M
#undef SP4_CP
#undef SP4_CD
#undef SP4_W
#undef SP4_MF
#undef SP4_ADD
    asm volatile("s_nop 15\n\ts_nop 7" ::: "memory");
    h16_t* dKo = reinterpret_cast<h16_t*>(p.dk) + (int64_t)b * p.Lk * p.lddk + hh * 32;
    h16_t* dVo = reinterpret_cast<h16_t*>(p.dv) + (int64_t)b * p.Lk * p.lddv + hh * 32;
#pragma unroll
    for (int kb = 0; kb < NKB; ++kb) {
        store_acc(dK[kb], dKo, p.lddk, key0 + kb * 32 + r, true, 32, h, p.scale / p.premul);
        store_acc(dV[kb], dVo, p.lddv, key0 + kb * 32 + r, true, 32, h, 1.f);
    }
}
__device__ __forceinline__ void fw_mfma_c(f32x16& d, const uint4& a, const uint4& b, const f32x16& c) {
    asm volatile("v_mfma_f32_32x32x16_" SVOL_H16_ASM " %0, %1, %2, %3" : "=&v"(d) : "v"(as_u32x4(a)), "v"(as_u32x4(b)), "v"(c));
}
__device__ __forceinline__ void fw_mfma_v(f32x16& d, const uint4& a, const uint4& b) {
    asm volatile("v_mfma_f32_32x32x16_" SVOL_H16_ASM " %0, %1, %2, %0" : "+v"(d) : "v"(as_u32x4(a)), "v"(as_u32x4(b)));
}
__device__ __forceinline__ void fw_mfma_p(f32x16& d, const uint4& a, const u32x4& b) {
    asm volatile("v_mfma_f32_32x32x16_" SVOL_H16_ASM " %0, %1, %2, %0" : "+v"(d) : "v"(as_u32x4(a)), "v"(b));
}
__global__ __launch_bounds__(256, 2) void attn_fwd_bf16_fast2(Args p) {
    __shared__ __attribute__((aligned(16))) char smem[6 * IMG];
    char* sK = smem;
    char* sV = smem + 3 * IMG;
    const int tid = threadIdx.x, lane = tid & 63, wave = __builtin_amdgcn_readfirstlane(tid >> 6);
    const int r = lane & 31, h = lane >> 5;
    int xt, hh, b;
    block_coords(p, xt, hh, b);
    const int qrow = xt * 128 + wave * 32 + r;
    const bool qvalid = qrow < p.Lq;
    const h16_t* Q = reinterpret_cast<const h16_t*>(p.q) + (int64_t)b * p.Lq * p.ldq + hh * p.dh;
    const h16_t* K = reinterpret_cast<const h16_t*>(p.k) + (int64_t)b * p.Lk * p.ldk + hh * p.dh;
    const h16_t* V = reinterpret_cast<const h16_t*>(p.v) + (int64_t)b * p.Lk * p.ldv + hh * p.dh;
    uint4 qb[2];
    load_lane_block(qb, Q, p.ldq, qrow, qvalid, p.dh, h);
    const int nt = p.Lk / KT;
    dma_tile(sK, K, p.ldk, 0, wave, lane);
    dma_tile(sV, V, p.ldv, 0, wave, lane);
    if (nt > 1) {
        dma_tile(sK + IMG, K, p.ldk, KT, wave, lane);
        dma_tile(sV + IMG, V, p.ldv, KT, wave, lane);
    }
    dma_wait_all();
    __syncthreads();
    float m;
    {
        float mm = -INFINITY;
#pragma unroll
        for (int sub = 0; sub < 4; ++sub) {
            uint4 ka[2];
            read_rows(ka, sK, sub * 32 + r, h);
            const f32x16 S0 = mma_first(ka, qb);
#pragma unroll
            for (int i = 0; i < 16; ++i) mm = fmaxf(mm, S0[i]);
        }
        const HalfPair sw = swap_halves(__builtin_bit_cast(unsigned, mm));
        m = fmaxf(__builtin_bit_cast(float, sw.lo), __builtin_bit_cast(float, sw.hi));
    }
    const f32x16 Cm = splat16(-m);
    f32x16 O = zero16();
    float lacc[4] = {0.f, 0.f, 0.f, 0.f};
    const unsigned o_rows0 = img_off(r, h), o_rows1 = img_off(r, 2 + h);
    unsigned o_trl, o_trh;
    {
        const int g = lane >> 4, i = lane & 15, q = i >> 2, pp = i & 3, h2 = g >> 1;
        const int ch = 2 * (g & 1) + (pp >> 1), inner = 8 * (pp & 1);
        o_trl = img_off(4 * h2 + q, ch) + inner;
        o_trh = img_off(4 * h2 + q + 8, ch) + inner;
    }
    f32x16 S;
    uint4 kn[2];
    {
        uint4 ka[2];
        read_rows(ka, sK, r, h);
        read_rows(kn, sK, 32 + r, h);
        asm volatile("s_nop 1\n\tv_mfma_f32_32x32x16_" SVOL_H16_ASM " %0, %1, %2, %3" : "=&v"(S) : "v"(as_u32x4(ka[0])), "v"(as_u32x4(qb[0])), "v"(Cm));
        fw_mfma_v(S, ka[1], qb[1]);
        asm volatile("s_nop 15\n\ts_nop 15" : "+v"(S), "+v"(O));
    }
#define FW_E(i) asm volatile("v_exp_f32 %0, %0" : "+v"(S[i]))
#define FW_A(i) asm volatile("v_add_f32 %0, %0, %1" : "+v"(lacc[(i) & 3]) : "v"(S[i]))
#define FW_C(j) asm volatile("v_cvt_pk_" SVOL_H16_ASM "_f32 %0, %1, %2" : "=v"(((j) < 4 ? P0 : P1)[(j) & 3]) : "v"(S[2 * (j)]), "v"(S[2 * (j) + 1]))
#define FW_MF(stmt) do { SP_FENCE(); stmt; SP_FENCE(); } while (0)
    const int prow = 32 * wave + (lane >> 2), pch = ((lane & 3) ^ ((lane >> 4) & 3)) * 8;
    const h16_t* gk2 = K + ((int64_t)2 * KT + prow) * p.ldk + pch;
    const h16_t* gv2 = V + ((int64_t)2 * KT + prow) * p.ldv + pch;
    const unsigned lds_k = (unsigned)(size_t)(lds_vptr)sK + wave * 2048, lds_v = (unsigned)(size_t)(lds_vptr)sV + wave * 2048;
    int cur = 0;
    for (int t = 0; t < nt; ++t) {
        const int nxt = cur == 2 ? 0 : cur + 1, nxt2 = nxt == 2 ? 0 : nxt + 1;
        const char* kimg = sK + cur * IMG;
        const char* vimg = sV + cur * IMG;
        const bool more = t + 1 < nt;
#pragma unroll
        for (int sub = 0; sub < 4; ++sub) {
            if (sub == 2 && more) {
                dma_wait_all();
                __syncthreads();
                if (t + 2 < nt) {
                    const unsigned dk_ = __builtin_amdgcn_readfirstlane(lds_k + nxt2 * IMG), dv_ = __builtin_amdgcn_readfirstlane(lds_v + nxt2 * IMG);
                    asm volatile("s_mov_b32 m0, %0\n\tglobal_load_lds_dwordx4 %1, off" ::"s"(dk_), "v"(gk2) : "m0");
                    asm volatile("s_mov_b32 m0, %0\n\tglobal_load_lds_dwordx4 %1, off" ::"s"(dk_ + 1024), "v"(gk2 + 16 * p.ldk) : "m0");
                    asm volatile("s_mov_b32 m0, %0\n\tglobal_load_lds_dwordx4 %1, off" ::"s"(dv_), "v"(gv2) : "m0");
                    asm volatile("s_mov_b32 m0, %0\n\tglobal_load_lds_dwordx4 %1, off" ::"s"(dv_ + 1024), "v"(gv2 + 16 * p.ldv) : "m0");
                    gk2 += (int64_t)KT * p.ldk;
                    gv2 += (int64_t)KT * p.ldv;
                }
            }
            const char* nrow = sub < 2 ? kimg + (sub + 2) * 2048 : sK + nxt * IMG + (sub - 2) * 2048;
            uint4 va[2];
            f32x16 Sn;
            u32x4 P0, P1;
            SP_FENCE();
#pragma unroll
            for (int ks = 0; ks < 2; ++ks) {
                const h16x4 lo = SVOL_DS_READ_TR16_H16((lds_bf16x4_ptr)(vimg + sub * 2048 + o_trl + 1024 * ks));
                const h16x4 hi = SVOL_DS_READ_TR16_H16((lds_bf16x4_ptr)(vimg + sub * 2048 + o_trh + 1024 * ks));
                va[ks] = __builtin_bit_cast(uint4, __builtin_shufflevector(lo, hi, 0, 1, 2, 3, 4, 5, 6, 7));
            }
            SP_FENCE();
            FW_E(0); FW_E(1); FW_E(2); FW_E(3); FW_E(4); FW_E(5); FW_E(6); FW_E(7);
            FW_MF(fw_mfma_c(Sn, kn[0], qb[0], Cm));
            FW_E(8); FW_E(9); FW_E(10); FW_E(11); FW_A(0); FW_A(1); FW_A(2); FW_A(3); FW_A(4); FW_A(5); FW_A(6); FW_A(7);
            FW_MF(fw_mfma_v(Sn, kn[1], qb[1]));
            kn[0] = *reinterpret_cast<const uint4*>(nrow + o_rows0);
            kn[1] = *reinterpret_cast<const uint4*>(nrow + o_rows1);
            SP_FENCE();
            FW_C(0); FW_C(1); FW_C(2); FW_C(3); FW_E(12); FW_E(13); FW_E(14); FW_E(15);
            FW_MF(fw_mfma_p(O, va[0], P0));
            FW_C(4); FW_C(5); FW_C(6); FW_C(7); FW_A(8); FW_A(9); FW_A(10); FW_A(11); FW_A(12); FW_A(13); FW_A(14); FW_A(15);
            FW_MF(fw_mfma_p(O, va[1], P1));
            S = Sn;
        }
        cur = nxt;
    }
#undef FW_E
#undef FW_A
#undef FW_C
#undef FW_MF
    asm volatile("s_nop 15\n\ts_nop 7" : "+v"(O));
    const float l = (lacc[0] + lacc[1]) + (lacc[2] + lacc[3]);
    const float lt = l + __shfl_xor(l, 32, 64);
    const int bad = __syncthreads_or(qvalid && !(lt < SVOL_H16_PSUM_MAX));
    if (tid == 0) p.redo[blockIdx.x] = bad ? 1 : 0;
    if (bad) return;
    const float inv = lt > 0.f ? 1.f / lt : 0.f;
    h16_t* Oo = reinterpret_cast<h16_t*>(p.out_o) + (int64_t)b * p.Lq * p.ldo + hh * p.dh;
    store_acc(O, Oo, p.ldo, qrow, qvalid, p.dh, h, inv);
    if (qvalid && h == 0) p.lse2[((int64_t)b * p.H + hh) * p.Lq + qrow] = m + __builtin_amdgcn_logf(lt);
}

struct SpWork { int hh, b, kbase, t0, t1, part; bool tail; };
__device__ __forceinline__ SpWork sp_work(const Args& p) {
    SpWork w;
    const int nfull = p.Lk / SP_KEYS, n_main = p.B * p.H * nfull, nt = p.Lq / KT;
    int id = blockIdx.x;
    w.tail = id >= n_main;
    if (w.tail) id -= n_main;
    const int xcd = id & 7, slot = id >> 3, per = w.tail ? 4 : nfull;
    int hl, xt;
    if (p.head_xcd == 2) { const int g = slot / (2 * per), r = slot - g * 2 * per; hl = g * 2 + (r & 1); xt = r >> 1; }
    else { hl = slot / per; xt = slot - hl * per; }
    const int head = p.head_xcd == 2 ? (((hl >> 1) * 8 + xcd) * 2 + (hl & 1)) : hl * 8 + xcd;
    w.hh = head % p.H;
    w.b = head / p.H;
    w.part = w.tail ? xt : 0;
    w.kbase = w.tail ? nfull * SP_KEYS : xt * SP_KEYS;
    w.t0 = w.tail ? xt * nt / 4 : 0;
    w.t1 = w.tail ? (xt + 1) * nt / 4 : nt;
    return w;
}
__device__ __forceinline__ float* sp_tail_ptr(const Args& p, const SpWork& w) {
    const int tk = p.Lk % SP_KEYS;
    return p.ws_dq + (int64_t)p.B * p.Lq * p.H * 32 + ((int64_t)(w.b * p.H + w.hh) * 4 + w.part) * 2 * tk * 32;
}
__device__ __forceinline__ void attn_bwd_sp_dispatch(const Args& p, char* smem) {
    const SpWork w = sp_work(p);
    if (!w.tail) {
        attn_bwd_sp_body4(p, smem, w.hh, w.b, w.kbase, w.t0, w.t1);
        return;
    }
    float* to = sp_tail_ptr(p, w);
    const int tk = p.Lk % SP_KEYS;
    if (w.t1 <= w.t0) {
        for (int i = threadIdx.x; i < 2 * tk * 32; i += 256) to[i] = 0.f;
        return;
    }
    if (tk == 384) attn_bwd_sp_body<3>(p, smem, w.hh, w.b, w.kbase, w.t0, w.t1, to);
    else if (tk == 256) attn_bwd_sp_body<2>(p, smem, w.hh, w.b, w.kbase, w.t0, w.t1, to);
    else attn_bwd_sp_body<1>(p, smem, w.hh, w.b, w.kbase, w.t0, w.t1, to);
}
__global__ __launch_bounds__(256, 1) void attn_bwd_sp_bf16(Args p) {
    __shared__ __attribute__((aligned(1024))) char smem[SP_LDS];
    attn_bwd_sp_dispatch(p, smem);
}
static inline unsigned sp_round_grid(int B, int H, int Lq, int Lk) {
    return (unsigned)(((int64_t)B * Lq * H * 32 + 2047) / 2048 + ((int64_t)B * H * 2 * (Lk % SP_KEYS) * 32 + 2047) / 2048);
}
static inline unsigned sp_grid(int B, int H, int Lk) { return (unsigned)(B * H * (Lk / SP_KEYS + (Lk % SP_KEYS ? 4 : 0))); }

}

constexpr int KSPLIT_WGS = 256;
static int64_t ksplit_ws_floats(int ks, int B, int H, int Lq, int dh) {
    return (int64_t)ks * B * Lq * H * dh + (int64_t)ks * B * H * Lq * 2 + (int64_t)B * Lq * H * dh;
}
static int plan_ksplit(int B, int H, int Lq, int Lk, int dh, int64_t ws_floats, int* tiles_per_split) {
    const int nt = (Lk + KT - 1) / KT;
    const int64_t wgs = (int64_t)((Lq + 127) / 128) * H * B;
    *tiles_per_split = nt;
    if (wgs >= 192 || nt < 8) return 1;
    int want = (int)((KSPLIT_WGS + wgs - 1) / wgs);
    if (want > 16) want = 16;
    int tps = (nt + want - 1) / want;
    if (tps < 2) tps = 2;
    const int ks = (nt + tps - 1) / tps;
    if (ks < 2 || ksplit_ws_floats(ks, B, H, Lq, dh) > ws_floats) return 1;
    *tiles_per_split = tps;
    return ks;
}
constexpr int SP_MIN_LK = 2 * SP_KEYS;
enum class Fwd { fast2_redo, pre_all, pre_masked, general_m, general_u, ksplit_m, ksplit_u };
enum class Bwd { bwd_sp, bwd_rot_dma, bwd_rot, bwd_pre, bwd_pre_masked, fq_m, fq_u, two_pass_m, two_pass_u };
struct Grid { dim3 dim; int head_xcd, nxt, tail_last; };
struct Plan {
    bool masked, pre;
    Fwd fwd; Bwd bwd;
    int ntk, fwd_ksplit, fwd_tps, bwd_ksplit, bwd_tps;
    Grid gf, gq, gk;
    int fq_tps; dim3 fq_grid;
    int64_t need_cls, need_redo, need_sp, need_ksplit, need;
};
static Plan attn_plan(int B, int H, int Lq, int Lk, int dh, bool premul, bool kbias, bool dropout, bool ws, int64_t ws_bytes,
                      bool det = svol_deterministic()) {
    static const bool no_fewq = getenv("SVOL_ATTN_NO_FEWQ") != nullptr;
    Plan pl{};
    const int ntk = pl.ntk = pl.fwd_tps = (Lk + KT - 1) / KT, nq128 = (Lq + 127) / 128;
    int tps;
    const int ks_free = plan_ksplit(B, H, Lq, Lk, dh, INT64_MAX, &tps);
    const bool sp_shape = !det && dh == 32 && H == 8 && (B * H) % 8 == 0 && Lq % KT == 0 && Lk % KT == 0 && Lk >= SP_MIN_LK;
    pl.need_cls = (int64_t)B * ntk;
    pl.need_redo = (int64_t)B * H * nq128;
    pl.need_sp = sp_shape ? (int64_t)B * Lq * H * 32 + (int64_t)B * H * 4 * 2 * (Lk % SP_KEYS) * 32 : 0;
    pl.need_ksplit = ks_free > 1 ? ksplit_ws_floats(ks_free, B, H, Lq, dh) : 0;
    pl.need = ks_free > 1 ? pl.need_ksplit : max(max(pl.need_cls, pl.need_redo), pl.need_sp);
    pl.masked = kbias || (Lk % KT) != 0;
    pl.pre = premul && !dropout && (!pl.masked || (ks_free == 1 && ws && ws_bytes >= 4 * pl.need_cls));
    pl.fwd_ksplit = (ws && !pl.pre) ? plan_ksplit(B, H, Lq, Lk, dh, ws_bytes / 4, &pl.fwd_tps) : 1;
    pl.bwd_ksplit = det ? 1 : pl.fwd_ksplit;
    pl.bwd_tps = det ? ntk : pl.fwd_tps;
    const int hx = (pl.pre && (B * H) % 8 == 0) ? (((B * H) % 16 == 0 && H % 2 == 0 && dh == 32) ? 2 : 1) : 0;
    auto grid = [&](int nx) {
        return hx ? Grid{dim3((unsigned)(B * H * nx)), hx, nx, 0} : Grid{dim3((unsigned)nx, (unsigned)H, (unsigned)B), 0, 0, 0};
    };
    pl.gf = grid(nq128 * pl.fwd_ksplit);
    pl.gq = pl.pre ? grid((Lq + 255) / 256) : grid(nq128 * pl.bwd_ksplit);
    if (hx) pl.gq.tail_last = (Lq % 256 >= 1 && Lq % 256 <= 128 && pl.gq.nxt > 1) ? 1 : 0;
    pl.gk = grid((Lk + 127) / 128);
    if (pl.pre && pl.masked) pl.fwd = Fwd::pre_masked;
    else if (pl.pre) pl.fwd = (hx && dh == 32 && ws && ws_bytes >= 4 * pl.need_redo) ? Fwd::fast2_redo : Fwd::pre_all;
    else if (pl.fwd_ksplit > 1) pl.fwd = pl.masked ? Fwd::ksplit_m : Fwd::ksplit_u;
    else pl.fwd = pl.masked ? Fwd::general_m : Fwd::general_u;
    if (pl.pre && pl.masked) pl.bwd = Bwd::bwd_pre_masked;
    else if (pl.pre && hx && sp_shape && ws && ws_bytes >= 4 * pl.need_sp) pl.bwd = Bwd::bwd_sp;
    else if (pl.pre && dh == 32) pl.bwd = Lq % KT == 0 ? Bwd::bwd_rot_dma : Bwd::bwd_rot;
    else if (pl.pre) pl.bwd = Bwd::bwd_pre;
    else if (!no_fewq && !det && pl.bwd_ksplit > 1 && Lq <= KT && dh == 32 && !dropout) pl.bwd = kbias ? Bwd::fq_m : Bwd::fq_u;
    else pl.bwd = pl.masked ? Bwd::two_pass_m : Bwd::two_pass_u;
    const int chunks = min(ntk, max(1, 512 / (B * H)));
    pl.fq_tps = (ntk + chunks - 1) / chunks;
    pl.fq_grid = dim3((unsigned)((ntk + pl.fq_tps - 1) / pl.fq_tps), (unsigned)H, (unsigned)B);
    return pl;
}
static Plan attn_plan(const AttnCall& c) {
    return attn_plan(c.B, c.H, c.Lq, c.Lk, c.dh, c.premul != 0.f, c.kbias != nullptr, c.drop_p > 0.f, c.ws != nullptr, c.ws_bytes);
}
int64_t svol_attn_ws_floats_bf16(int B, int H, int Lq, int Lk, int dh) {
    return attn_plan(B, H, Lq, Lk, dh, false, false, false,  false, 0).need;
}
static bool sp_planned(int B, int H, int Lq, int Lk, int dh, bool ws, int64_t ws_bytes) {
    return attn_plan(B, H, Lq, Lk, dh,  true,  false,  false, ws, ws_bytes).bwd == Bwd::bwd_sp;
}
int64_t svol_attn_sp_image_bytes_bf16(int B, int H, int Lq, int Lk, int dh, int64_t ws_bytes) {
    return sp_planned(B, H, Lq, Lk, dh, true, ws_bytes) ? (int64_t)B * Lq * H * 32 * 4 : 0;
}
constexpr int SP_ZERO_WGS = 64;
int svol_attn_sp_zero_bf16_launch(float* ws, int64_t ws_bytes, int B, int H, int Lq, int Lk, int dh, hipStream_t s) {
    if (!sp_planned(B, H, Lq, Lk, dh, ws != nullptr, ws_bytes)) return SVOL_E_UNSUPPORTED;
    const int64_t n4 = (int64_t)B * Lq * H * 32 / 4;
    const int64_t want = (n4 + 255) / 256;
    hipLaunchKernelGGL(attn_sp_zero_image, dim3((unsigned)(want < SP_ZERO_WGS ? want : SP_ZERO_WGS)), dim3(256), 0, s, ws, n4);
    return hipGetLastError() == hipSuccess ? SVOL_OK : SVOL_E_LAUNCH;
}
static Args make_args(const AttnCall& c, int ksplit, int tiles_per_split, const Grid& g) {
    Args p{};
    attn_fill(p, c);
    p.ksplit = ksplit; p.tiles_per_split = tiles_per_split;
    if (ksplit > 1) {
        p.ws_o = c.ws;
        p.ws_ml = p.ws_o + (int64_t)p.ksplit * p.B * p.Lq * p.H * p.dh;
        p.ws_dq = p.ws_ml + (int64_t)p.ksplit * p.B * p.H * p.Lq * 2;
    }
    p.head_xcd = g.head_xcd; p.nxt = g.nxt; p.tail_last = g.tail_last;
    return p;
}

int svol_attn_fwd_bf16_launch(const AttnCall& c) {
    const Plan pl = attn_plan(c);
    Args p = make_args(c, pl.fwd_ksplit, pl.fwd_tps, pl.gf);
    const dim3 grid = pl.gf.dim, wg(256);
    hipStream_t s = c.stream;
    switch (pl.fwd) {
    case Fwd::pre_masked:
        p.tile_flags = reinterpret_cast<const int*>(c.ws);
        hipLaunchKernelGGL(attn_tile_flags_bf16, dim3((unsigned)pl.ntk, (unsigned)c.B), dim3(64), 0, s, c.kbias, c.Lk, pl.ntk, reinterpret_cast<int*>(c.ws));
        hipLaunchKernelGGL(attn_fwd_bf16_pre_masked, grid, wg, 0, s, p);
        break;
    case Fwd::fast2_redo:
        p.redo = reinterpret_cast<int*>(c.ws);
        hipLaunchKernelGGL(attn_fwd_bf16_fast2, grid, wg, 0, s, p);
        [[fallthrough]];
    case Fwd::pre_all: hipLaunchKernelGGL(attn_fwd_bf16_pre, grid, wg, 0, s, p); break;
    case Fwd::general_m:
    case Fwd::ksplit_m: hipLaunchKernelGGL(attn_fwd_bf16<true>, grid, wg, 0, s, p); break;
    case Fwd::general_u:
    case Fwd::ksplit_u: hipLaunchKernelGGL(attn_fwd_bf16<false>, grid, wg, 0, s, p); break;
    }
    const int64_t total = (int64_t)c.B * c.Lq * c.H;
    if (pl.fwd_ksplit > 1) hipLaunchKernelGGL(attn_combine_bf16, dim3((unsigned)((total + 127) / 128)), dim3(128), 0, s, p);
    return hipGetLastError() == hipSuccess ? SVOL_OK : SVOL_E_LAUNCH;
}

int svol_attn_bwd_bf16_launch(const AttnCall& c) {
    const Plan pl = attn_plan(c);
    Args pq = make_args(c, pl.bwd_ksplit, pl.bwd_tps, pl.gq), pk = make_args(c, pl.bwd_ksplit, pl.bwd_tps, pl.gk);
    const int64_t total = (int64_t)c.B * c.Lq * c.H;
    const dim3 gd((unsigned)((total + 255) / 256)), wg(256);
    hipStream_t s = c.stream;
    auto bind_rows = [&](Args& a) { a.nl2 = reinterpret_cast<unsigned*>(c.delta + total); a.nd2 = reinterpret_cast<unsigned*>(c.delta + 2 * total); };
    void (*dq)(Args) = nullptr, (*dkdv)(Args) = nullptr;
    if (!pl.pre) hipLaunchKernelGGL(attn_delta_bf16, gd, wg, 0, s, pq);
    switch (pl.bwd) {
    case Bwd::bwd_pre_masked:
        pq.tile_flags = pk.tile_flags = reinterpret_cast<const int*>(c.ws);
        hipLaunchKernelGGL(attn_tile_flags_bf16, dim3((unsigned)pl.ntk, (unsigned)c.B), dim3(64), 0, s, c.kbias, c.Lk, pl.ntk, reinterpret_cast<int*>(c.ws));
        dq = attn_bwd_dq_bf16_pre_masked, dkdv = attn_bwd_dkdv_bf16_pre_masked;
        break;
    case Bwd::bwd_sp:
        pq.ws_dq = c.ws;
        bind_rows(pq);
        hipLaunchKernelGGL((c.flags & SVOL_ATTN_DQ_PREZEROED) ? attn_bwd_sp_prep_bf16<false> : attn_bwd_sp_prep_bf16<true>,
                           dim3((unsigned)((int64_t)c.B * c.Lq / 32)), wg, 0, s, pq);
        break;
    case Bwd::bwd_rot_dma:
        bind_rows(pq), bind_rows(pk);
        dq = attn_bwd_dq_bf16_rot, dkdv = attn_bwd_dkdv_bf16_pre_dma;
        break;
    case Bwd::bwd_rot: dq = attn_bwd_dq_bf16_rot, dkdv = attn_bwd_dkdv_bf16_pre; break;
    case Bwd::bwd_pre: dq = attn_bwd_dq_bf16_pre, dkdv = attn_bwd_dkdv_bf16_pre; break;
    case Bwd::fq_m:
    case Bwd::fq_u: {
        Args pf = pq;
        pf.tiles_per_split = pl.fq_tps;
        hipLaunchKernelGGL(pl.bwd == Bwd::fq_m ? attn_bwd_fq_bf16<true> : attn_bwd_fq_bf16<false>, pl.fq_grid, wg, 0, s, pf);
        hipLaunchKernelGGL(attn_dq_finish_bf16, gd, wg, 0, s, pq);
        break;
    }
    case Bwd::two_pass_m: dq = attn_bwd_dq_bf16<true>, dkdv = attn_bwd_dkdv_bf16<true>; break;
    case Bwd::two_pass_u: dq = attn_bwd_dq_bf16<false>, dkdv = attn_bwd_dkdv_bf16<false>; break;
    }
    if (dq) {
        hipLaunchKernelGGL(dq, pl.gq.dim, wg, 0, s, pq);
        if (pl.bwd_ksplit > 1) hipLaunchKernelGGL(attn_dq_finish_bf16, gd, wg, 0, s, pq);
        hipLaunchKernelGGL(dkdv, pl.gk.dim, wg, 0, s, pk);
    }
    if (c.ev_prep) (void)hipEventRecord(static_cast<hipEvent_t>(c.ev_prep), s);
    if (pl.bwd == Bwd::bwd_sp) {
        hipLaunchKernelGGL(attn_bwd_sp_bf16, dim3(sp_grid(c.B, c.H, c.Lk)), wg, 0, s, pq);
        hipLaunchKernelGGL(attn_dq_round_bf16, dim3(sp_round_grid(c.B, c.H, c.Lq, c.Lk)), wg, 0, s, pq);
    }
    return hipGetLastError() == hipSuccess ? SVOL_OK : SVOL_E_LAUNCH;
}
```

### svol_amd/csrc/gemm_ws_bf16.hip

```cpp
#include "gemm_call.h"

namespace {

struct WsArgs {
    const h16_t* A; const h16_t* W; void* C;
    const float* bias; const float* colscale; h16_t* pre; const void* res; const h16_t* aux; float* colsum;
    int64_t lda, ldw, ldc, ldp, ldr, ldaux;
    int M, N, act, tiles_per_wg, nchunk;
};

typedef __attribute__((address_space(3))) void* lds_void_ptr;

constexpr int WS_K = 256;
constexpr int TR = 16;
constexpr int A_PLANE = TR * WS_K * 2;

typedef unsigned u32x4_t __attribute__((ext_vector_type(4)));

template <int N> __device__ __forceinline__ void ws_wait_vm() { asm volatile("s_waitcnt vmcnt(%0)" ::"n"(N) : "memory"); }
__device__ __forceinline__ void ws_wait_vm_dyn(int n) {
    switch (n) {
#define C_(x) case x: ws_wait_vm<x>(); break;
        C_(0) C_(1) C_(2) C_(3) C_(4) C_(5) C_(6) C_(7) C_(8) C_(9) C_(10) C_(11) C_(12) C_(13) C_(14) C_(15) C_(16)
        C_(17) C_(18) C_(19) C_(20) C_(21) C_(22) C_(23) C_(24) C_(25) C_(26) C_(27) C_(28) C_(29) C_(30) C_(31) C_(32)
#undef C_
        default: ws_wait_vm<32>(); break;
    }
}

__device__ __forceinline__ int ws_col(int t, int i) { return (t >> 1) * 32 + (i >> 2) * 8 + (t & 1) * 4 + (i & 3); }

template <int MODE> struct WsCfg;
template <> struct WsCfg<0> { static constexpr int SLOT = A_PLANE, STG = 4, ND = 2; };
template <> struct WsCfg<1> { static constexpr int SLOT = A_PLANE + TR * 256 * 4, STG = 3, ND = 6; };
template <> struct WsCfg<2> { static constexpr int SLOT = 2 * A_PLANE, STG = 4, ND = 4; };

template <int MODE>
__device__ __forceinline__ void gemm_ws_body(const WsArgs& p) {
    constexpr int SLOT = WsCfg<MODE>::SLOT, STG = WsCfg<MODE>::STG, ND = WsCfg<MODE>::ND;
    __shared__ __attribute__((aligned(1024))) char smem[STG * SLOT];
    const int tid = threadIdx.x, lane = tid & 63;
    const int wave = __builtin_amdgcn_readfirstlane(tid >> 6);
    const int fr = lane & 15, fq = lane >> 4;
    const int chunk_id = blockIdx.x % p.nchunk, cg = blockIdx.x / p.nchunk;
    const int cg0 = cg * 256;
    const int c0 = cg0 + wave * 64;
    const bool active = c0 < p.N;
    const int tile0 = chunk_id * p.tiles_per_wg;
    const int row_base = tile0 * TR;
    const int rows_here = min(p.tiles_per_wg * TR, p.M - row_base);
    const int ntile = (rows_here + TR - 1) / TR;
    const int ns = !active ? 0 : (MODE == 0 ? (p.pre ? 4 : 2) : (MODE == 1 ? 4 : 2));

    const __amdgpu_buffer_rsrc_t rA = __builtin_amdgcn_make_buffer_rsrc(
        (void*)(p.A + (int64_t)row_base * p.lda), 0, (int)((((int64_t)rows_here - 1) * p.lda + WS_K) * 2), 0x00020000);
    int voffA[2];
#pragma unroll
    for (int j = 0; j < 2; ++j) {
        const int row = (wave * 2 + j) * 2 + (lane >> 5), s = lane & 31;
        voffA[j] = (int)(((int64_t)row * p.lda + ((s ^ row) & 31) * 8) * 2);
    }
    __amdgpu_buffer_rsrc_t rX = rA;
    int voffX[4] = {0, 0, 0, 0};
    if constexpr (MODE == 1) {
        const float* R = reinterpret_cast<const float*>(p.res) + (int64_t)row_base * p.ldr + cg0;
        const int cols = min(256, p.N - cg0);
        rX = __builtin_amdgcn_make_buffer_rsrc((void*)R, 0, (int)((((int64_t)rows_here - 1) * p.ldr + cols) * 4), 0x00020000);
#pragma unroll
        for (int j = 0; j < 4; ++j) {
            const int row = wave * 4 + j, s = lane;
            voffX[j] = (int)(((int64_t)row * p.ldr + (((s & 48) | ((s ^ row) & 15))) * 4) * 4);
        }
    } else if constexpr (MODE == 2) {
        const h16_t* X = p.aux + (int64_t)row_base * p.ldaux + cg0;
        const int cols = min(256, p.N - cg0);
        rX = __builtin_amdgcn_make_buffer_rsrc((void*)X, 0, (int)((((int64_t)rows_here - 1) * p.ldaux + cols) * 2), 0x00020000);
#pragma unroll
        for (int j = 0; j < 2; ++j) {
            const int row = (wave * 2 + j) * 2 + (lane >> 5), s = lane & 31;
            voffX[j] = (int)(((int64_t)row * p.ldaux + ((s ^ row) & 31) * 8) * 2);
        }
    }
    auto issue = [&](int slot, int tile) {
        char* sl = smem + slot * SLOT;
        const int soA = (int)((int64_t)tile * TR * p.lda * 2);
#pragma unroll
        for (int j = 0; j < 2; ++j)
            __builtin_amdgcn_raw_ptr_buffer_load_lds(rA, (lds_void_ptr)(sl + (wave * 2 + j) * 1024), 16, voffA[j], soA, 0, 0);
        if constexpr (MODE == 1) {
            const int so = (int)((int64_t)tile * TR * p.ldr * 4);
#pragma unroll
            for (int j = 0; j < 4; ++j)
                __builtin_amdgcn_raw_ptr_buffer_load_lds(rX, (lds_void_ptr)(sl + A_PLANE + (wave * 4 + j) * 1024), 16, voffX[j], so, 0, 0);
        } else if constexpr (MODE == 2) {
            const int so = (int)((int64_t)tile * TR * p.ldaux * 2);
#pragma unroll
            for (int j = 0; j < 2; ++j)
                __builtin_amdgcn_raw_ptr_buffer_load_lds(rX, (lds_void_ptr)(sl + A_PLANE + (wave * 2 + j) * 1024), 16, voffX[j], so, 0, 0);
        }
    };

    uint4 wf[4][8];
#pragma unroll
    for (int t = 0; t < 4; ++t) {
        const h16_t* wrow = p.W + (int64_t)(c0 + ws_col(t, fr)) * p.ldw + fq * 8;
#pragma unroll
        for (int ks = 0; ks < 8; ++ks) wf[t][ks] = active ? *reinterpret_cast<const uint4*>(wrow + ks * 32) : make_uint4(0, 0, 0, 0);
    }
    float bias8[2][8], scale8[2][8];
#pragma unroll
    for (int hf = 0; hf < 2; ++hf)
#pragma unroll
        for (int e = 0; e < 8; ++e) {
            const int n = c0 + hf * 32 + fq * 8 + e;
            bias8[hf][e] = (active && p.bias) ? p.bias[n] : 0.f;
            scale8[hf][e] = (MODE == 0 && active && p.colscale) ? p.colscale[n] : 1.f;
        }
    float csum[2][8];
#pragma unroll
    for (int hf = 0; hf < 2; ++hf)
#pragma unroll
        for (int e = 0; e < 8; ++e) csum[hf][e] = 0.f;

    const unsigned lds0 = (unsigned)(size_t)(lds_void_ptr)smem;
    const unsigned aoff = (unsigned)(fr * 512 + ((fq ^ fr) & 3) * 16);

#pragma unroll
    for (int s = 0; s < STG - 1; ++s)
        if (s < ntile) issue(s, s);

    for (int j = 0; j < ntile; ++j) {
        ws_wait_vm_dyn(ND * min(STG - 2, ntile - 1 - j) + ns * min(j, STG - 1));
        __builtin_amdgcn_s_barrier();
        if (j + STG - 1 < ntile) issue((j + STG - 1) % STG, j + STG - 1);
        const unsigned sl = lds0 + (unsigned)((j % STG) * SLOT);
        uint4 af[8];
        {
            const unsigned b = sl + aoff;
            const unsigned x = (unsigned)((fr & 12) * 16);
            asm volatile(
                "ds_read_b128 %0, %8\n\t"
                "ds_read_b128 %1, %9\n\t"
                "ds_read_b128 %2, %10\n\t"
                "ds_read_b128 %3, %11\n\t"
                "ds_read_b128 %4, %8 offset:256\n\t"
                "ds_read_b128 %5, %9 offset:256\n\t"
                "ds_read_b128 %6, %10 offset:256\n\t"
                "ds_read_b128 %7, %11 offset:256\n\t"
                "s_waitcnt lgkmcnt(0)"
                : "=&v"(af[0]), "=&v"(af[1]), "=&v"(af[2]), "=&v"(af[3]), "=&v"(af[4]), "=&v"(af[5]), "=&v"(af[6]), "=&v"(af[7])
                : "v"(b + ((0u * 64) ^ x)), "v"(b + ((1u * 64) ^ x)), "v"(b + ((2u * 64) ^ x)), "v"(b + ((3u * 64) ^ x))
                : "memory");
        }
        f32x4 acc[4];
#pragma unroll
        for (int t = 0; t < 4; ++t) acc[t] = f32x4{0.f, 0.f, 0.f, 0.f};
#pragma unroll
        for (int ks = 0; ks < 8; ++ks)
#pragma unroll
            for (int t = 0; t < 4; ++t)
                acc[t] = SVOL_MFMA_16x16x32_H16(__builtin_bit_cast(h16x8, wf[t][ks]),
                                                                 __builtin_bit_cast(h16x8, af[ks]), acc[t], 0, 0, 0);
        const int m = row_base + j * TR + fr;
        float v[2][8];
#pragma unroll
        for (int hf = 0; hf < 2; ++hf)
#pragma unroll
            for (int e = 0; e < 8; ++e) v[hf][e] = acc[2 * hf + (e >> 2)][e & 3];
        if constexpr (MODE == 0) {
#pragma unroll
            for (int hf = 0; hf < 2; ++hf)
#pragma unroll
                for (int e = 0; e < 8; ++e) v[hf][e] = (v[hf][e] + bias8[hf][e]) * scale8[hf][e];
            if (active && m < p.M) {
                if (p.pre) {
#pragma unroll
                    for (int hf = 0; hf < 2; ++hf) {
                        h16x8 o;
#pragma unroll
                        for (int e = 0; e < 8; ++e) o[e] = (h16_t)pre_save_fast(v[hf][e], p.act);
                        *reinterpret_cast<h16x8*>(p.pre + (int64_t)m * p.ldp + c0 + hf * 32 + fq * 8) = o;
                    }
                }
                h16_t* C = reinterpret_cast<h16_t*>(p.C);
                if (act_is_gelu(p.act)) {
#pragma unroll
                    for (int hf = 0; hf < 2; ++hf)
#pragma unroll
                        for (int e = 0; e < 8; ++e) v[hf][e] = gelu_fast(v[hf][e]);
                } else if (p.act == SVOL_ACT_RELU) {
#pragma unroll
                    for (int hf = 0; hf < 2; ++hf)
#pragma unroll
                        for (int e = 0; e < 8; ++e) v[hf][e] = fmaxf(v[hf][e], 0.f);
                }
#pragma unroll
                for (int hf = 0; hf < 2; ++hf) {
                    h16x8 o;
#pragma unroll
                    for (int e = 0; e < 8; ++e) o[e] = (h16_t)v[hf][e];
                    *reinterpret_cast<h16x8*>(C + (int64_t)m * p.ldc + c0 + hf * 32 + fq * 8) = o;
                }
            }
        } else if constexpr (MODE == 1) {
            f32x4 rr[4];
            {
                const unsigned rb = sl + A_PLANE + (unsigned)(fr * 1024 + wave * 256);
                const unsigned q0 = (unsigned)(((fq * 2) ^ fr) & 15), q1 = (unsigned)(((fq * 2 + 1) ^ fr) & 15);
                const unsigned q2 = (unsigned)(((8 + fq * 2) ^ fr) & 15), q3 = (unsigned)(((8 + fq * 2 + 1) ^ fr) & 15);
                asm volatile(
                    "ds_read_b128 %0, %4\n\t"
                    "ds_read_b128 %1, %5\n\t"
                    "ds_read_b128 %2, %6\n\t"
                    "ds_read_b128 %3, %7\n\t"
                    "s_waitcnt lgkmcnt(0)"
                    : "=&v"(rr[0]), "=&v"(rr[1]), "=&v"(rr[2]), "=&v"(rr[3])
                    : "v"(rb + q0 * 16), "v"(rb + q1 * 16), "v"(rb + q2 * 16), "v"(rb + q3 * 16)
                    : "memory");
            }
            if (active && m < p.M) {
                float* C = reinterpret_cast<float*>(p.C);
#pragma unroll
                for (int hf = 0; hf < 2; ++hf)
#pragma unroll
                    for (int q = 0; q < 2; ++q) {
                        f32x4 o;
#pragma unroll
                        for (int e = 0; e < 4; ++e) o[e] = v[hf][4 * q + e] + bias8[hf][4 * q + e] + rr[2 * hf + q][e];
                        *reinterpret_cast<f32x4*>(C + (int64_t)m * p.ldc + c0 + hf * 32 + fq * 8 + 4 * q) = o;
                    }
            }
        } else {
            uint4 ax[2];
            {
                const unsigned xb = sl + A_PLANE + (unsigned)(fr * 512);
                const unsigned q0 = (unsigned)(((wave * 8 + fq) ^ fr) & 31), q1 = (unsigned)(((wave * 8 + 4 + fq) ^ fr) & 31);
                asm volatile(
                    "ds_read_b128 %0, %2\n\t"
                    "ds_read_b128 %1, %3\n\t"
                    "s_waitcnt lgkmcnt(0)"
                    : "=&v"(ax[0]), "=&v"(ax[1])
                    : "v"(xb + q0 * 16), "v"(xb + q1 * 16)
                    : "memory");
            }
            const bool ok = active && m < p.M;
#pragma unroll
            for (int hf = 0; hf < 2; ++hf) {
                const h16x8 a8 = __builtin_bit_cast(h16x8, ax[hf]);
                h16x8 o;
#pragma unroll
                for (int e = 0; e < 8; ++e) {
                    float d = v[hf][e] * dact_fast((float)a8[e], p.act);
                    d = ok ? d : 0.f;
                    csum[hf][e] += d;
                    o[e] = (h16_t)d;
                }
                if (ok) *reinterpret_cast<h16x8*>(reinterpret_cast<h16_t*>(p.C) + (int64_t)m * p.ldc + c0 + hf * 32 + fq * 8) = o;
            }
        }
    }
    if constexpr (MODE == 2) {
        if (p.colsum) {
#pragma unroll
            for (int hf = 0; hf < 2; ++hf)
#pragma unroll
                for (int e = 0; e < 8; ++e) {
                    float s = csum[hf][e];
                    s += __shfl_xor(s, 1, 64);
                    s += __shfl_xor(s, 2, 64);
                    s += __shfl_xor(s, 4, 64);
                    s += __shfl_xor(s, 8, 64);
                    if (fr == 0 && active) atomicAdd(p.colsum + c0 + hf * 32 + fq * 8 + e, s);
                }
        }
    }
}

__global__ __launch_bounds__(256, 2) void gemm_ws_bf16_m0(WsArgs p) { gemm_ws_body<0>(p); }
__global__ __launch_bounds__(256, 2) void gemm_ws_bf16_m1(WsArgs p) { gemm_ws_body<1>(p); }
__global__ __launch_bounds__(256, 2) void gemm_ws_bf16_m2(WsArgs p) { gemm_ws_body<2>(p); }


__device__ __forceinline__ void store_b128_guarded(u32x4_t v, __amdgpu_buffer_rsrc_t rsrc, int voffset, int soffset) {
    __builtin_amdgcn_raw_buffer_store_b128(v, rsrc, voffset, soffset, 0);
    asm volatile("s_nop 1" ::"v"(v));
}

template <int MODE, int ACT, bool PRE, bool SCALE, int VPM>
__device__ __forceinline__ void gemm_wsp_body(const WsArgs& p) {
    static_assert(MODE == 0 || MODE == 2, "bf16 outputs only");
    constexpr int SLOT = WsCfg<MODE>::SLOT, STG = 4, ND = WsCfg<MODE>::ND;
    constexpr int NS = MODE == 0 ? (PRE ? 4 : 2) : 2;
    __shared__ __attribute__((aligned(1024))) char smem[STG * SLOT];
    const int tid = threadIdx.x, lane = tid & 63;
    const int wave = __builtin_amdgcn_readfirstlane(tid >> 6);
    const int fr = lane & 15, fq = lane >> 4;
    const int chunk_id = blockIdx.x % p.nchunk, cg = blockIdx.x / p.nchunk;
    const int cg0 = cg * 256;
    const int c0 = cg0 + wave * 64;
    const bool active = c0 < p.N;
    const int tile0 = chunk_id * p.tiles_per_wg;
    const int row_base = tile0 * TR;
    const int rows_here = min(p.tiles_per_wg * TR, p.M - row_base);
    const int ntile = (rows_here + TR - 1) / TR;

    const __amdgpu_buffer_rsrc_t rA = __builtin_amdgcn_make_buffer_rsrc(
        (void*)(p.A + (int64_t)row_base * p.lda), 0, (int)((((int64_t)rows_here - 1) * p.lda + WS_K) * 2), 0x00020000);
    int voffA[2];
#pragma unroll
    for (int j = 0; j < 2; ++j) {
        const int row = (wave * 2 + j) * 2 + (lane >> 5), s = lane & 31;
        voffA[j] = (int)(((int64_t)row * p.lda + ((s ^ row) & 31) * 8) * 2);
    }
    __amdgpu_buffer_rsrc_t rX = rA;
    int voffX[2] = {0, 0};
    if constexpr (MODE == 2) {
        const h16_t* X = p.aux + (int64_t)row_base * p.ldaux + cg0;
        const int cols = min(256, p.N - cg0);
        rX = __builtin_amdgcn_make_buffer_rsrc((void*)X, 0, (int)((((int64_t)rows_here - 1) * p.ldaux + cols) * 2), 0x00020000);
#pragma unroll
        for (int j = 0; j < 2; ++j) {
            const int row = (wave * 2 + j) * 2 + (lane >> 5), s = lane & 31;
            voffX[j] = (int)(((int64_t)row * p.ldaux + ((s ^ row) & 31) * 8) * 2);
        }
    }
    auto issue = [&](int slot, int tile) {
        char* sl = smem + slot * SLOT;
        const int soA = (int)((int64_t)tile * TR * p.lda * 2);
#pragma unroll
        for (int j = 0; j < 2; ++j)
            __builtin_amdgcn_raw_ptr_buffer_load_lds(rA, (lds_void_ptr)(sl + (wave * 2 + j) * 1024), 16, voffA[j], soA, 0, 0);
        if constexpr (MODE == 2) {
            const int so = (int)((int64_t)tile * TR * p.ldaux * 2);
#pragma unroll
            for (int j = 0; j < 2; ++j)
                __builtin_amdgcn_raw_ptr_buffer_load_lds(rX, (lds_void_ptr)(sl + A_PLANE + (wave * 2 + j) * 1024), 16, voffX[j], so, 0, 0);
        }
    };

    uint4 wf[4][8];
#pragma unroll
    for (int t = 0; t < 4; ++t) {
        const h16_t* wrow = p.W + (int64_t)(c0 + ws_col(t, fr)) * p.ldw + fq * 8;
#pragma unroll
        for (int ks = 0; ks < 8; ++ks) wf[t][ks] = active ? *reinterpret_cast<const uint4*>(wrow + ks * 32) : make_uint4(0, 0, 0, 0);
    }
    float bias8[2][8], scale8[2][8];
#pragma unroll
    for (int hf = 0; hf < 2; ++hf)
#pragma unroll
        for (int e = 0; e < 8; ++e) {
            const int n = c0 + hf * 32 + fq * 8 + e;
            bias8[hf][e] = (MODE == 0 && active && p.bias) ? p.bias[n] : 0.f;
            scale8[hf][e] = (MODE == 0 && SCALE && active && p.colscale) ? p.colscale[n] : 1.f;
        }
    float csum[2][8];
#pragma unroll
    for (int hf = 0; hf < 2; ++hf)
#pragma unroll
        for (int e = 0; e < 8; ++e) csum[hf][e] = 0.f;

    const unsigned lds0 = (unsigned)(size_t)(lds_void_ptr)smem;
    const unsigned aoff = (unsigned)(fr * 512 + ((fq ^ fr) & 3) * 16);
    const unsigned ax_x = (unsigned)((fr & 12) * 16);
    const unsigned xq0 = (unsigned)(A_PLANE + fr * 512 + (((wave * 8 + fq) ^ fr) & 31) * 16);
    const unsigned xq1 = (unsigned)(A_PLANE + fr * 512 + (((wave * 8 + 4 + fq) ^ fr) & 31) * 16);
    const __amdgpu_buffer_rsrc_t rC = __builtin_amdgcn_make_buffer_rsrc(
        (void*)(reinterpret_cast<h16_t*>(p.C) + (int64_t)row_base * p.ldc), 0,
        active ? (int)((((int64_t)rows_here - 1) * p.ldc + p.N) * 2) : 0, 0x00020000);
    const __amdgpu_buffer_rsrc_t rP = __builtin_amdgcn_make_buffer_rsrc(
        (void*)(PRE ? p.pre + (int64_t)row_base * p.ldp : nullptr), 0,
        (PRE && active) ? (int)((((int64_t)rows_here - 1) * p.ldp + p.N) * 2) : 0, 0x00020000);
    const int voffC = (int)(((int64_t)fr * p.ldc + c0 + fq * 8) * 2), voffP = (int)(((int64_t)fr * p.ldp + c0 + fq * 8) * 2);
    const int cstep = (int)(TR * p.ldc * 2), pstep = (int)(TR * p.ldp * 2);

    u32x4_t af[8], ax[2] = {u32x4_t{0, 0, 0, 0}, u32x4_t{0, 0, 0, 0}};
    auto read_frags = [&](int slot) {
        const unsigned sl = lds0 + (unsigned)(slot * SLOT);
        const unsigned b = sl + aoff;
        asm volatile(
            "ds_read_b128 %0, %8\n\t"
            "ds_read_b128 %1, %9\n\t"
            "ds_read_b128 %2, %10\n\t"
            "ds_read_b128 %3, %11\n\t"
            "ds_read_b128 %4, %8 offset:256\n\t"
            "ds_read_b128 %5, %9 offset:256\n\t"
            "ds_read_b128 %6, %10 offset:256\n\t"
            "ds_read_b128 %7, %11 offset:256"
            : "=&v"(af[0]), "=&v"(af[1]), "=&v"(af[2]), "=&v"(af[3]), "=&v"(af[4]), "=&v"(af[5]), "=&v"(af[6]), "=&v"(af[7])
            : "v"(b + ((0u * 64) ^ ax_x)), "v"(b + ((1u * 64) ^ ax_x)), "v"(b + ((2u * 64) ^ ax_x)), "v"(b + ((3u * 64) ^ ax_x))
            : "memory");
        if constexpr (MODE == 2) {
            asm volatile(
                "ds_read_b128 %0, %2\n\t"
                "ds_read_b128 %1, %3"
                : "=&v"(ax[0]), "=&v"(ax[1])
                : "v"(sl + xq0), "v"(sl + xq1)
                : "memory");
        }
    };
    auto wait_frags = [&]() {
        asm volatile("s_waitcnt lgkmcnt(0)"
                     : "+v"(af[0]), "+v"(af[1]), "+v"(af[2]), "+v"(af[3]), "+v"(af[4]), "+v"(af[5]), "+v"(af[6]), "+v"(af[7]),
                       "+v"(ax[0]), "+v"(ax[1]));
    };
    auto mfma_slab = [&](f32x4 (&acc)[4]) {
#pragma unroll
        for (int t = 0; t < 4; ++t) acc[t] = f32x4{0.f, 0.f, 0.f, 0.f};
#pragma unroll
        for (int ks = 0; ks < 8; ++ks)
#pragma unroll
            for (int t = 0; t < 4; ++t)
                acc[t] = SVOL_MFMA_16x16x32_H16(__builtin_bit_cast(h16x8, wf[t][ks]),
                                                                 __builtin_bit_cast(h16x8, af[ks]), acc[t], 0, 0, 0);
    };
    auto epilogue = [&](int j, const f32x4 (&acc)[4], const u32x4_t (&axj)[2]) {
        float v[2][8];
#pragma unroll
        for (int hf = 0; hf < 2; ++hf)
#pragma unroll
            for (int e = 0; e < 8; ++e) v[hf][e] = acc[2 * hf + (e >> 2)][e & 3];
        if constexpr (MODE == 0) {
#pragma unroll
            for (int hf = 0; hf < 2; ++hf)
#pragma unroll
                for (int e = 0; e < 8; ++e) {
                    v[hf][e] += bias8[hf][e];
                    if constexpr (SCALE) v[hf][e] *= scale8[hf][e];
                }
            if constexpr (PRE) {
                h16x8 o[2];
#pragma unroll
                for (int hf = 0; hf < 2; ++hf)
#pragma unroll
                    for (int e = 0; e < 8; ++e) o[hf][e] = (h16_t)pre_save_fast(v[hf][e], ACT);
                store_b128_guarded(__builtin_bit_cast(u32x4_t, o[0]), rP, voffP, j * pstep);
                store_b128_guarded(__builtin_bit_cast(u32x4_t, o[1]), rP, voffP + 64, j * pstep);
            }
            h16x8 o[2];
#pragma unroll
            for (int hf = 0; hf < 2; ++hf)
#pragma unroll
                for (int e = 0; e < 8; ++e) {
                    float y = v[hf][e];
                    if constexpr (ACT == SVOL_ACT_GELU || ACT == SVOL_ACT_GELU_D) y = gelu_fast(y);
                    if constexpr (ACT == SVOL_ACT_RELU) y = fmaxf(y, 0.f);
                    o[hf][e] = (h16_t)y;
                }
            store_b128_guarded(__builtin_bit_cast(u32x4_t, o[0]), rC, voffC, j * cstep);
            store_b128_guarded(__builtin_bit_cast(u32x4_t, o[1]), rC, voffC + 64, j * cstep);
        } else {
            h16x8 o[2];
#pragma unroll
            for (int hf = 0; hf < 2; ++hf) {
                const h16x8 a8 = __builtin_bit_cast(h16x8, axj[hf]);
#pragma unroll
                for (int e = 0; e < 8; ++e) {
                    const float d = v[hf][e] * dact_fast((float)a8[e], ACT);
                    csum[hf][e] += d;
                    o[hf][e] = (h16_t)d;
                }
            }
            store_b128_guarded(__builtin_bit_cast(u32x4_t, o[0]), rC, voffC, j * cstep);
            store_b128_guarded(__builtin_bit_cast(u32x4_t, o[1]), rC, voffC + 64, j * cstep);
        }
    };

#pragma unroll
    for (int s = 0; s < STG; ++s)
        if (s < ntile) issue(s, s);
    ws_wait_vm_dyn(ND * min(STG - 1, ntile - 1));
    __builtin_amdgcn_s_barrier();
    read_frags(0);
    wait_frags();
    f32x4 acc[4];
    mfma_slab(acc);
    for (int j = 0; j + 1 < ntile; ++j) {
        const int nd = min(STG - 2, ntile - 2 - j), nst = min(j, STG - 1);
        if (nd == STG - 2 && nst == STG - 1) ws_wait_vm<ND * (STG - 2) + NS * (STG - 1)>();
        else ws_wait_vm_dyn(ND * nd + NS * nst);
        __builtin_amdgcn_s_barrier();
        if (j + STG < ntile) issue(j % STG, j + STG);
        f32x4 accp[4];
        u32x4_t axp[2];
#pragma unroll
        for (int t = 0; t < 4; ++t) accp[t] = acc[t];
        axp[0] = ax[0];
        axp[1] = ax[1];
        read_frags((j + 1) % STG);
        wait_frags();
        mfma_slab(acc);
        epilogue(j, accp, axp);
#pragma unroll
        for (int i = 0; i < 32; ++i) {
            __builtin_amdgcn_sched_group_barrier(0x008, 1, 0);
            __builtin_amdgcn_sched_group_barrier(0x002, VPM, 0);
        }
    }
    {
        u32x4_t axp[2] = {ax[0], ax[1]};
        epilogue(ntile - 1, acc, axp);
    }
    if constexpr (MODE == 2) {
        if (p.colsum) {
#pragma unroll
            for (int hf = 0; hf < 2; ++hf)
#pragma unroll
                for (int e = 0; e < 8; ++e) {
                    float s = csum[hf][e];
                    s += __shfl_xor(s, 1, 64);
                    s += __shfl_xor(s, 2, 64);
                    s += __shfl_xor(s, 4, 64);
                    s += __shfl_xor(s, 8, 64);
                    if (fr == 0 && active) atomicAdd(p.colsum + c0 + hf * 32 + fq * 8 + e, s);
                }
        }
    }
}

#define WSP_KERNEL(name, MODE, ACT, PRE, SCALE, VPM) \
    __global__ __launch_bounds__(256, 2) void name(WsArgs p) { gemm_wsp_body<MODE, ACT, PRE, SCALE, VPM>(p); }
WSP_KERNEL(gemm_wsp_bf16_none, 0, SVOL_ACT_NONE, false, false, 2)
WSP_KERNEL(gemm_wsp_bf16_none_scale, 0, SVOL_ACT_NONE, false, true, 2)
WSP_KERNEL(gemm_wsp_bf16_gelu, 0, SVOL_ACT_GELU, false, false, 7)
WSP_KERNEL(gemm_wsp_bf16_gelu_pre, 0, SVOL_ACT_GELU, true, false, 8)
WSP_KERNEL(gemm_wsp_bf16_gelu_dpre, 0, SVOL_ACT_GELU_D, true, false, 9)
WSP_KERNEL(gemm_wsp_bf16_relu, 0, SVOL_ACT_RELU, false, false, 2)
WSP_KERNEL(gemm_wsp_bf16_dgelu, 2, SVOL_ACT_GELU, false, false, 9)
WSP_KERNEL(gemm_wsp_bf16_dmul, 2, SVOL_ACT_GELU_D, false, false, 3)
WSP_KERNEL(gemm_wsp_bf16_drelu, 2, SVOL_ACT_RELU, false, false, 3)
#undef WSP_KERNEL

}

static int ws_plan(const GemmCall& c, WsArgs& p, dim3& grid, void (*&kern)(WsArgs)) {
    const int64_t M = c.M, N = c.N;
    const int act = c.act;
    if (c.kwrap != c.K || c.K != WS_K || N % 64 || M < 4096) return SVOL_E_UNSUPPORTED;
    int mode;
    if (c.epi == 1) {
        if (!c.aux || c.out_f32) return SVOL_E_UNSUPPORTED;
        mode = 2;
    } else if (c.out_f32) {
        if (!c.res || act != SVOL_ACT_NONE || c.pre || c.colscale) return SVOL_E_UNSUPPORTED;
        mode = 1;
    } else {
        if (c.res || (act != SVOL_ACT_NONE && act != SVOL_ACT_GELU && act != SVOL_ACT_RELU && act != SVOL_ACT_GELU_D)) return SVOL_E_UNSUPPORTED;
        if (act == SVOL_ACT_GELU_D && !c.pre) return SVOL_E_INVALID;
        mode = 0;
    }
    if (c.lda % 8 || c.ldb % 8 || !aligned16(c.A) || !aligned16(c.B) || !aligned16(c.C)) return SVOL_E_UNSUPPORTED;
    if (mode == 1 ? (c.ldc % 4 || c.ldr % 4 || !aligned16(c.res)) : (c.ldc % 8 != 0)) return SVOL_E_UNSUPPORTED;
    if (c.pre && (c.ldp % 8 || !aligned16(c.pre))) return SVOL_E_UNSUPPORTED;
    if (mode == 2 && (c.ldaux % 8 || !aligned16(c.aux))) return SVOL_E_UNSUPPORTED;
    const int64_t ntile = (M + TR - 1) / TR;
    const int64_t ncg = (N + 255) / 256;
    int64_t tpw = (ntile * ncg + (ncg <= 2 ? 255 : 511)) / (ncg <= 2 ? 256 : 512);
    if (tpw < 4) tpw = 4;
    if (tpw > 64) tpw = 64;
    const int64_t ldmax = c.lda > c.ldr * 2 ? c.lda : c.ldr * 2;
    int64_t ldbig = ldmax > c.ldaux ? ldmax : c.ldaux;
    if (c.ldc > ldbig) ldbig = c.ldc;
    if (c.pre && c.ldp > ldbig) ldbig = c.ldp;
    if (tpw * TR * ldbig * 2 >= (1ll << 31)) return SVOL_E_UNSUPPORTED;
    int64_t nchunk = (ntile + tpw - 1) / tpw;
    if (ncg > 1 && nchunk > 8 && nchunk % 8) {
        const int64_t n8 = (nchunk + 7) / 8 * 8;
        const int64_t t8 = (ntile + n8 - 1) / n8;
        if (t8 >= 1 && (ntile + t8 - 1) / t8 == n8) { tpw = t8; nchunk = n8; }
    }
    if (nchunk * ncg > (1ll << 30)) return SVOL_E_UNSUPPORTED;
    p = WsArgs{(const h16_t*)c.A, (const h16_t*)c.B, c.C, c.bias, c.colscale, (h16_t*)c.pre, c.res, (const h16_t*)c.aux, c.colsum,
               c.lda, c.ldb, c.ldc, c.ldp, c.ldr, c.ldaux, (int)M, (int)N, act, (int)tpw, (int)nchunk};
    grid = dim3((unsigned)(ncg * nchunk));
    kern = mode == 0 ? gemm_ws_bf16_m0 : (mode == 1 ? gemm_ws_bf16_m1 : gemm_ws_bf16_m2);
    if (mode == 0) {
        if (act == SVOL_ACT_NONE && !c.pre) kern = c.colscale ? gemm_wsp_bf16_none_scale : gemm_wsp_bf16_none;
        else if (act == SVOL_ACT_GELU && !c.colscale) kern = c.pre ? gemm_wsp_bf16_gelu_pre : gemm_wsp_bf16_gelu;
        else if (act == SVOL_ACT_GELU_D && !c.colscale) kern = gemm_wsp_bf16_gelu_dpre;
        else if (act == SVOL_ACT_RELU && !c.pre && !c.colscale) kern = gemm_wsp_bf16_relu;
    } else if (mode == 2) {
        kern = act == SVOL_ACT_RELU ? gemm_wsp_bf16_drelu : (act == SVOL_ACT_GELU_D ? gemm_wsp_bf16_dmul : gemm_wsp_bf16_dgelu);
    }
    return SVOL_OK;
}

int svol_gemm_ws_bf16(const GemmCall& c) {
    WsArgs p; dim3 grid; void (*kern)(WsArgs);
    if (const int rc = ws_plan(c, p, grid, kern)) return rc;
    hipLaunchKernelGGL(kern, grid, dim3(256), 0, c.stream, p);
    return hipGetLastError() == hipSuccess ? SVOL_OK : SVOL_E_LAUNCH;
}
```

Measured before the change: 15420.

## Deal attention and GEMM workgroups across XCDs for L2 locality

Attention kernels (forward, fused-dq backward) now get a flattened 1-D grid whose block index is mapped through block_coords_uniform, so blocks sharing a head land on the same XCD. The non-premul path also uses this mapping when B*H divides by 8. The weight-stationary GEMM reorders block IDs in groups of 8 so that chunks sharing a column group are spread round-robin across XCDs, padding the grid and early-exiting surplus blocks. The aim is better per-XCD L2 reuse of K/V and weight tiles, at the cost of a few idle padded blocks and extra index arithmetic. Much of the attention kernel code appears to have been moved or rewritten, with the body not fully visible.

```diff
diff --git a/svol_amd/csrc/attention_bf16.hip b/svol_amd/csrc/attention_bf16.hip
--- a/svol_amd/csrc/attention_bf16.hip
+++ b/svol_amd/csrc/attention_bf16.hip
@@ -179,501 +179,6 @@
     }
 }
 
-template <bool MASKED>
-__global__ __launch_bounds__(256, 2) void attn_fwd_bf16(Args p) {
-    const uint64_t dseed = drop_seed_at(p.drop_seed, p.drop_step);
-    __shared__ __attribute__((aligned(16))) char smem[4 * IMG + 2 * KT * 4];
-    char* sK = smem;
-    char* sV = smem + 2 * IMG;
-    float* sB = reinterpret_cast<float*>(smem + 4 * IMG);
-
-    const int tid = threadIdx.x, lane = tid & 63, wave = tid >> 6;
-    const int r = lane & 31, h = lane >> 5;
-    const int b = blockIdx.z, hh = blockIdx.y;
-    const int qt = blockIdx.x / p.ksplit, sp = blockIdx.x % p.ksplit;
-    const int qrow = qt * 128 + wave * 32 + r;
-    const bool qvalid = qrow < p.Lq;
-    const h16_t* Q = reinterpret_cast<const h16_t*>(p.q) + (int64_t)b * p.Lq * p.ldq + hh * p.dh;
-    const h16_t* K = reinterpret_cast<const h16_t*>(p.k) + (int64_t)b * p.Lk * p.ldk + hh * p.dh;
-    const h16_t* V = reinterpret_cast<const h16_t*>(p.v) + (int64_t)b * p.Lk * p.ldv + hh * p.dh;
-    const float* kb = p.kbias ? p.kbias + (int64_t)b * p.Lk : nullptr;
-    const float c = p.premul != 0.f ? 1.f : p.scale * LOG2E;
-
-    uint4 qb[2];
-    load_lane_block(qb, Q, p.ldq, qrow, qvalid, p.dh, h);
-
-    float m = -INFINITY, l = 0.f;
-    f32x16 O = zero16();
-
-    const int t0 = sp * p.tiles_per_split;
-    const int nt = min((p.Lk + KT - 1) / KT, t0 + p.tiles_per_split);
-    Stage sk, sv;
-    load_regs(sk, K, p.ldk, t0 * KT, p.Lk, p.dh, tid);
-    load_regs(sv, V, p.ldv, t0 * KT, p.Lk, p.dh, tid);
-    store_lds(sK, sk, tid);
-    store_lds(sV, sv, tid);
-    if (MASKED) stage_bias(sB, kb, t0 * KT, p.Lk, tid);
-    __syncthreads();
-
-    for (int t = t0; t < nt; ++t) {
-        const int cur = (t - t0) & 1;
-        if (t + 1 < nt) {
-            load_regs(sk, K, p.ldk, (t + 1) * KT, p.Lk, p.dh, tid);
-            load_regs(sv, V, p.ldv, (t + 1) * KT, p.Lk, p.dh, tid);
-        }
-        const char* kimg = sK + cur * IMG;
-        const char* vimg = sV + cur * IMG;
-        const float* bias = sB + cur * KT;
-        f32x16 S[4];
-#pragma unroll
-        for (int sub = 0; sub < 4; ++sub) {
-            uint4 ka[2];
-            read_rows(ka, kimg, sub * 32 + r, h);
-            S[sub] = mma_first(ka, qb);
-        }
-        mfma_results_ready(S[0], S[1], S[2], S[3]);
-        if (MASKED) {
-#pragma unroll
-            for (int sub = 0; sub < 4; ++sub)
-#pragma unroll
-                for (int g = 0; g < 4; ++g) {
-                    const f32x4 bb = *reinterpret_cast<const f32x4*>(bias + sub * 32 + 8 * g + 4 * h);
-#pragma unroll
-                    for (int e = 0; e < 4; ++e) S[sub][4 * g + e] = S[sub][4 * g + e] * c + bb[e];
-                }
-        }
-        float ml[4];
-#pragma unroll
-        for (int sub = 0; sub < 4; ++sub) {
-            float mm = max3(S[sub][0], S[sub][1], S[sub][2]);
-#pragma unroll
-            for (int i = 3; i < 15; i += 2) mm = max3(mm, S[sub][i], S[sub][i + 1]);
-            ml[sub] = max3(mm, S[sub][15], mm);
-        }
-        float mloc = max3(ml[0], ml[1], fmaxf(ml[2], ml[3]));
-        {
-            const HalfPair sw = swap_halves(__builtin_bit_cast(unsigned, mloc));
-            mloc = fmaxf(__builtin_bit_cast(float, sw.lo), __builtin_bit_cast(float, sw.hi));
-        }
-        const float thr = MASKED ? LAZY_THR : LAZY_THR / c;
-        if (__any(mloc > m + thr)) {
-            const float m_new = fmaxf(m, mloc);
-            const float m_use = (m_new == -INFINITY) ? 0.f : m_new;
-            const float alpha = __builtin_amdgcn_exp2f(MASKED ? (m - m_use) : (m - m_use) * c);
-            l *= alpha;
-#pragma unroll
-            for (int i = 0; i < 16; ++i) O[i] *= alpha;
-            m = m_new;
-        }
-        const float m_use = (m == -INFINITY) ? 0.f : m;
-        const float mc = MASKED ? -m_use : -m_use * c;
-        float ls[4] = {0.f, 0.f, 0.f, 0.f};
-#pragma unroll
-        for (int sub = 0; sub < 4; ++sub)
-#pragma unroll
-            for (int i = 0; i < 16; ++i) {
-                S[sub][i] = __builtin_amdgcn_exp2f(MASKED ? S[sub][i] + mc : __builtin_fmaf(S[sub][i], c, mc));
-                ls[sub] += S[sub][i];
-            }
-        l += (ls[0] + ls[1]) + (ls[2] + ls[3]);
-        if (p.drop_p > 0.f) {
-            const uint32_t rm = drop_row(drop_seed32(dseed), (((uint64_t)b * p.H + hh) * p.Lq + (qvalid ? qrow : 0)));
-            const uint32_t thr = drop_thr16(p.drop_p);
-#pragma unroll
-            for (int sub = 0; sub < 4; ++sub)
-#pragma unroll
-                for (int g = 0; g < 4; ++g)
-#pragma unroll
-                    for (int e = 0; e < 4; e += 2) {
-                        float s0, s1;
-                        attn_drop2(rm, t * KT + sub * 32 + 8 * g + 4 * h + e, thr, p.drop_inv, s0, s1);
-                        S[sub][4 * g + e] *= s0;
-                        S[sub][4 * g + e + 1] *= s1;
-                    }
-        }
-#pragma unroll
-        for (int sub = 0; sub < 4; ++sub) {
-            uint4 va[2];
-            read_tr(va, vimg, sub, lane);
-            mma_second(O, va, S[sub]);
-        }
-        if (t + 1 < nt) {
-            store_lds(sK + (cur ^ 1) * IMG, sk, tid);
-            store_lds(sV + (cur ^ 1) * IMG, sv, tid);
-            if (MASKED) stage_bias(sB + (cur ^ 1) * KT, kb, (t + 1) * KT, p.Lk, tid);
-        }
-        __syncthreads();
-    }
-    const float lt = l + __shfl_xor(l, 32, 64);
-    const float m2 = MASKED ? m : m * c;
-    if (p.ksplit > 1) {
-        if (qvalid) {
-            float* wo = p.ws_o + (((int64_t)sp * p.B + b) * p.Lq + qrow) * (p.H * p.dh) + hh * p.dh;
-#pragma unroll
-            for (int g = 0; g < 4; ++g) {
-                const int d0 = 8 * g + 4 * h;
-                if (d0 < p.dh) *reinterpret_cast<f32x4*>(wo + d0) = f32x4{O[4 * g], O[4 * g + 1], O[4 * g + 2], O[4 * g + 3]};
-            }
-            if (h == 0) {
-                float* wm = p.ws_ml + ((((int64_t)sp * p.B + b) * p.H + hh) * p.Lq + qrow) * 2;
-                wm[0] = m2;
-                wm[1] = lt;
-            }
-        }
-        return;
-    }
-    const float inv = lt > 0.f ? 1.f / lt : 0.f;
-    h16_t* Oo = reinterpret_cast<h16_t*>(p.out_o) + (int64_t)b * p.Lq * p.ldo + hh * p.dh;
-    store_acc(O, Oo, p.ldo, qrow, qvalid, p.dh, h, inv);
-    if (qvalid && h == 0) p.lse2[((int64_t)b * p.H + hh) * p.Lq + qrow] = m2 + __builtin_amdgcn_logf(lt);
-}
-
-__global__ void attn_combine_bf16(Args p) {
-    const int64_t idx = (int64_t)blockIdx.x * blockDim.x + threadIdx.x;
-    const int64_t total = (int64_t)p.B * p.Lq * p.H;
-    if (idx >= total) return;
-    const int hh = (int)(idx % p.H);
-    const int64_t row = idx / p.H;
-    const int b = (int)(row / p.Lq), q = (int)(row % p.Lq);
-    float M = -INFINITY;
-    for (int i = 0; i < p.ksplit; ++i) M = fmaxf(M, p.ws_ml[((((int64_t)i * p.B + b) * p.H + hh) * p.Lq + q) * 2]);
-    float L = 0.f, acc[32];
-#pragma unroll
-    for (int d = 0; d < 32; ++d) acc[d] = 0.f;
-    for (int i = 0; i < p.ksplit; ++i) {
-        const float* ml = p.ws_ml + ((((int64_t)i * p.B + b) * p.H + hh) * p.Lq + q) * 2;
-        if (ml[0] == -INFINITY) continue;
-        const float w = __builtin_amdgcn_exp2f(ml[0] - M);
-        L += w * ml[1];
-        const float* po = p.ws_o + (((int64_t)i * p.B + b) * p.Lq + q) * (p.H * p.dh) + hh * p.dh;
-#pragma unroll
-        for (int d = 0; d < 32; d += 4) {
-            if (d < p.dh) {
-                const f32x4 t = *reinterpret_cast<const f32x4*>(po + d);
-#pragma unroll
-                for (int e = 0; e < 4; ++e) acc[d + e] += w * t[e];
-            }
-        }
-    }
-    const float inv = L > 0.f ? 1.f / L : 0.f;
-    h16_t* o = reinterpret_cast<h16_t*>(p.out_o) + row * p.ldo + hh * p.dh;
-#pragma unroll
-    for (int d = 0; d < 32; d += 4) {
-        if (d < p.dh) {
-            h16x4 v;
-#pragma unroll
-            for (int e = 0; e < 4; ++e) v[e] = (h16_t)(acc[d + e] * inv);
-            *reinterpret_cast<h16x4*>(o + d) = v;
-        }
-    }
-    p.lse2[((int64_t)b * p.H + hh) * p.Lq + q] = M + __builtin_amdgcn_logf(L);
-}
-
-__global__ void attn_delta_bf16(Args p) {
-    const int64_t idx = (int64_t)blockIdx.x * blockDim.x + threadIdx.x;
-    const int64_t total = (int64_t)p.B * p.Lq * p.H;
-    if (idx >= total) return;
-    const int hh = (int)(idx % p.H);
-    const int64_t row = idx / p.H;
-    const int b = (int)(row / p.Lq), q = (int)(row % p.Lq);
-    const h16_t* o = reinterpret_cast<const h16_t*>(p.o) + row * p.ldo + hh * p.dh;
-    const h16_t* d = reinterpret_cast<const h16_t*>(p.d_o) + row * p.lddo + hh * p.dh;
-    float s = 0.f;
-    for (int i = 0; i < p.dh; i += 8) {
-        const h16x8 a = *reinterpret_cast<const h16x8*>(o + i), c = *reinterpret_cast<const h16x8*>(d + i);
-#pragma unroll
-        for (int e = 0; e < 8; ++e) s += (float)a[e] * (float)c[e];
-    }
-    p.delta[((int64_t)b * p.H + hh) * p.Lq + q] = s;
-    if (p.ksplit > 1) {
-        float* z = p.ws_dq + row * (p.H * p.dh) + hh * p.dh;
-        for (int i = 0; i < p.dh; i += 4) *reinterpret_cast<f32x4*>(z + i) = f32x4{0.f, 0.f, 0.f, 0.f};
-    }
-}
-
-__global__ void attn_dq_finish_bf16(Args p) {
-    const int64_t idx = (int64_t)blockIdx.x * blockDim.x + threadIdx.x;
-    const int64_t total = (int64_t)p.B * p.Lq * p.H;
-    if (idx >= total) return;
-    const int hh = (int)(idx % p.H);
-    const int64_t row = idx / p.H;
-    const float* z = p.ws_dq + row * (p.H * p.dh) + hh * p.dh;
-    h16_t* o = reinterpret_cast<h16_t*>(p.dq) + row * p.lddq + hh * p.dh;
-    for (int i = 0; i < p.dh; i += 4) {
-        const f32x4 t = *reinterpret_cast<const f32x4*>(z + i);
-        h16x4 v;
-#pragma unroll
-        for (int e = 0; e < 4; ++e) v[e] = (h16_t)(t[e] * p.scale);
-        *reinterpret_cast<h16x4*>(o + i) = v;
-    }
-}
-
-template <bool MASKED>
-__global__ __launch_bounds__(256, 2) void attn_bwd_dq_bf16(Args p) {
-    const uint64_t dseed = drop_seed_at(p.drop_seed, p.drop_step);
-    __shared__ __attribute__((aligned(16))) char smem[4 * IMG + 2 * KT * 4];
-    char* sK = smem;
-    char* sV = smem + 2 * IMG;
-    float* sB = reinterpret_cast<float*>(smem + 4 * IMG);
-
-    const int tid = threadIdx.x, lane = tid & 63, wave = tid >> 6;
-    const int r = lane & 31, h = lane >> 5;
-    const int b = blockIdx.z, hh = blockIdx.y;
-    const int qt = blockIdx.x / p.ksplit, sp = blockIdx.x % p.ksplit;
-    const int qrow = qt * 128 + wave * 32 + r;
-    const bool qvalid = qrow < p.Lq;
-    const h16_t* Q = reinterpret_cast<const h16_t*>(p.q) + (int64_t)b * p.Lq * p.ldq + hh * p.dh;
-    const h16_t* dO = reinterpret_cast<const h16_t*>(p.d_o) + (int64_t)b * p.Lq * p.lddo + hh * p.dh;
-    const h16_t* K = reinterpret_cast<const h16_t*>(p.k) + (int64_t)b * p.Lk * p.ldk + hh * p.dh;
-    const h16_t* V = reinterpret_cast<const h16_t*>(p.v) + (int64_t)b * p.Lk * p.ldv + hh * p.dh;
-    const float* kb = p.kbias ? p.kbias + (int64_t)b * p.Lk : nullptr;
-    const float c = p.premul != 0.f ? 1.f : p.scale * LOG2E;
-
-    uint4 qb[2], dob[2];
-    load_lane_block(qb, Q, p.ldq, qrow, qvalid, p.dh, h);
-    load_lane_block(dob, dO, p.lddo, qrow, qvalid, p.dh, h);
-    const int64_t sidx = ((int64_t)b * p.H + hh) * p.Lq + qrow;
-    const float nlse = qvalid ? -p.lse2[sidx] : -INFINITY;
-    const float dl = qvalid ? p.delta[sidx] : 0.f;
-
-    f32x16 dQ = zero16();
-    const int t0 = sp * p.tiles_per_split;
-    const int nt = min((p.Lk + KT - 1) / KT, t0 + p.tiles_per_split);
-    Stage sk, sv;
-    load_regs(sk, K, p.ldk, t0 * KT, p.Lk, p.dh, tid);
-    load_regs(sv, V, p.ldv, t0 * KT, p.Lk, p.dh, tid);
-    store_lds(sK, sk, tid);
-    store_lds(sV, sv, tid);
-    if (MASKED) stage_bias(sB, kb, t0 * KT, p.Lk, tid);
-    __syncthreads();
-
-    for (int t = t0; t < nt; ++t) {
-        const int cur = (t - t0) & 1;
-        if (t + 1 < nt) {
-            load_regs(sk, K, p.ldk, (t + 1) * KT, p.Lk, p.dh, tid);
-            load_regs(sv, V, p.ldv, (t + 1) * KT, p.Lk, p.dh, tid);
-        }
-        const char* kimg = sK + cur * IMG;
-        const char* vimg = sV + cur * IMG;
-        const float* bias = sB + cur * KT;
-#pragma unroll 2
-        for (int sub = 0; sub < 4; ++sub) {
-            uint4 a[2];
-            read_rows(a, kimg, sub * 32 + r, h);
-            f32x16 S = mma_first(a, qb);
-            read_rows(a, vimg, sub * 32 + r, h);
-            f32x16 dP = mma_first(a, dob);
-            if (p.drop_p > 0.f) {
-                const uint32_t rm = drop_row(drop_seed32(dseed), (((uint64_t)b * p.H + hh) * p.Lq + (qvalid ? qrow : 0)));
-                const uint32_t thr = drop_thr16(p.drop_p);
-#pragma unroll
-                for (int g = 0; g < 4; ++g)
-#pragma unroll
-                    for (int e = 0; e < 4; e += 2) {
-                        float s0, s1;
-                        attn_drop2(rm, t * KT + sub * 32 + 8 * g + 4 * h + e, thr, p.drop_inv, s0, s1);
-                        dP[4 * g + e] *= s0;
-                        dP[4 * g + e + 1] *= s1;
-                    }
-            }
-            if (MASKED) {
-#pragma unroll
-                for (int g = 0; g < 4; ++g) {
-                    const f32x4 bb = *reinterpret_cast<const f32x4*>(bias + sub * 32 + 8 * g + 4 * h);
-#pragma unroll
-                    for (int e = 0; e < 4; ++e) {
-                        const float pe = __builtin_amdgcn_exp2f(__builtin_fmaf(S[4 * g + e], c, bb[e] + nlse));
-                        S[4 * g + e] = pe * (dP[4 * g + e] - dl);
-                    }
-                }
-            } else {
-#pragma unroll
-                for (int i = 0; i < 16; ++i) {
-                    const float pe = __builtin_amdgcn_exp2f(__builtin_fmaf(S[i], c, nlse));
-                    S[i] = pe * (dP[i] - dl);
-                }
-            }
-            read_tr(a, kimg, sub, lane);
-            mma_second(dQ, a, S);
-        }
-        if (t + 1 < nt) {
-            store_lds(sK + (cur ^ 1) * IMG, sk, tid);
-            store_lds(sV + (cur ^ 1) * IMG, sv, tid);
-            if (MASKED) stage_bias(sB + (cur ^ 1) * KT, kb, (t + 1) * KT, p.Lk, tid);
-        }
-        __syncthreads();
-    }
-    if (p.ksplit > 1) {
-        if (qvalid) {
-            float* z = p.ws_dq + ((int64_t)b * p.Lq + qrow) * (p.H * p.dh) + hh * p.dh;
-#pragma unroll
-            for (int g = 0; g < 4; ++g) {
-                const int d0 = 8 * g + 4 * h;
-                if (d0 < p.dh) {
-#pragma unroll
-                    for (int e = 0; e < 4; ++e) atomicAdd(z + d0 + e, dQ[4 * g + e]);
-                }
-            }
-        }
-        return;
-    }
-    h16_t* dQo = reinterpret_cast<h16_t*>(p.dq) + (int64_t)b * p.Lq * p.lddq + hh * p.dh;
-    store_acc(dQ, dQo, p.lddq, qrow, qvalid, p.dh, h, p.scale);
-}
-
-template <bool KBIAS>
-__global__ __launch_bounds__(256, 2) void attn_bwd_dkdv_bf16(Args p) {
-    const uint64_t dseed = drop_seed_at(p.drop_seed, p.drop_step);
-    __shared__ __attribute__((aligned(16))) char smem[4 * IMG + 4 * KT * 4];
-    char* sQ = smem;
-    char* sdO = smem + 2 * IMG;
-    float* sL = reinterpret_cast<float*>(smem + 4 * IMG);
-    float* sD = sL + 2 * KT;
-
-    const int tid = threadIdx.x, lane = tid & 63, wave = tid >> 6;
-    const int r = lane & 31, h = lane >> 5;
-    const int b = blockIdx.z, hh = blockIdx.y;
-    const int krow = blockIdx.x * 128 + wave * 32 + r;
-    const bool kvalid = krow < p.Lk;
-    const h16_t* Q = reinterpret_cast<const h16_t*>(p.q) + (int64_t)b * p.Lq * p.ldq + hh * p.dh;
-    const h16_t* dO = reinterpret_cast<const h16_t*>(p.d_o) + (int64_t)b * p.Lq * p.lddo + hh * p.dh;
-    const h16_t* K = reinterpret_cast<const h16_t*>(p.k) + (int64_t)b * p.Lk * p.ldk + hh * p.dh;
-    const h16_t* V = reinterpret_cast<const h16_t*>(p.v) + (int64_t)b * p.Lk * p.ldv + hh * p.dh;
-    const float c = p.premul != 0.f ? 1.f : p.scale * LOG2E;
-    const float kbl = kvalid ? (p.kbias ? p.kbias[(int64_t)b * p.Lk + krow] * LOG2E : 0.f) : -INFINITY;
-    const float* lse_g = p.lse2 + ((int64_t)b * p.H + hh) * p.Lq;
-    const float* dl_g = p.delta + ((int64_t)b * p.H + hh) * p.Lq;
-
-    uint4 kbk[2], vbk[2];
-    load_lane_block(kbk, K, p.ldk, krow, kvalid, p.dh, h);
-    load_lane_block(vbk, V, p.ldv, krow, kvalid, p.dh, h);
-
-    f32x16 dK = zero16(), dV = zero16();
-    const int nt = (p.Lq + KT - 1) / KT;
-    Stage sq, sdo;
-    float rl = 0.f, rd = 0.f;
-    auto load_stats = [&](int row0) {
-        if (tid < KT) {
-            const int qi = row0 + tid;
-            rl = qi < p.Lq ? -lse_g[qi] : -INFINITY;
-            rd = qi < p.Lq ? dl_g[qi] : 0.f;
-        }
-    };
-    auto store_stats = [&](int buf) {
-        if (tid < KT) { sL[buf * KT + tid] = rl; sD[buf * KT + tid] = rd; }
-    };
-    load_regs(sq, Q, p.ldq, 0, p.Lq, p.dh, tid);
-    load_regs(sdo, dO, p.lddo, 0, p.Lq, p.dh, tid);
-    load_stats(0);
-    store_lds(sQ, sq, tid);
-    store_lds(sdO, sdo, tid);
-    store_stats(0);
-    __syncthreads();
-
-    for (int t = 0; t < nt; ++t) {
-        const int cur = t & 1;
-        if (t + 1 < nt) {
-            load_regs(sq, Q, p.ldq, (t + 1) * KT, p.Lq, p.dh, tid);
-            load_regs(sdo, dO, p.lddo, (t + 1) * KT, p.Lq, p.dh, tid);
-            load_stats((t + 1) * KT);
-        }
-        const char* qimg = sQ + cur * IMG;
-        const char* doimg = sdO + cur * IMG;
-        const float* nl = sL + cur * KT;
-        const float* dd = sD + cur * KT;
-#pragma unroll 1
-        for (int sub = 0; sub < 4; ++sub) {
-            uint4 a[2];
-            read_rows(a, qimg, sub * 32 + r, h);
-            f32x16 S = mma_first(a, kbk);
-#pragma unroll
-            for (int g = 0; g < 4; ++g) {
-                const f32x4 ls = *reinterpret_cast<const f32x4*>(nl + sub * 32 + 8 * g + 4 * h);
-#pragma unroll
-                for (int e = 0; e < 4; ++e)
-                    S[4 * g + e] = __builtin_amdgcn_exp2f(__builtin_fmaf(S[4 * g + e], c, KBIAS ? kbl + ls[e] : ls[e]));
-            }
-            read_tr(a, doimg, sub, lane);
-            f32x16 MS;
-#pragma unroll
-            for (int i = 0; i < 16; ++i) MS[i] = 1.f;
-            if (p.drop_p > 0.f) {
-                const uint32_t s0 = drop_seed32(dseed), thr = drop_thr16(p.drop_p), odd = (uint32_t)lane & 1u;
-                const uint64_t rbase = ((uint64_t)b * p.H + hh) * p.Lq;
-                const bool rows32 = rbase + (uint64_t)p.Lq <= 0xffffffffull;
-#pragma unroll
-                for (int g = 0; g < 4; ++g)
-#pragma unroll
-                    for (int e = 0; e < 4; e += 2) {
-                        const int q0 = t * KT + sub * 32 + 8 * g + 4 * h + e;
-                        const int qm = min(q0 + (int)odd, p.Lq - 1);
-                        const uint32_t rm = rows32 ? (s0 ^ (((uint32_t)rbase + (uint32_t)qm) * 0x9E3779B1u)) : drop_row(s0, rbase + (uint64_t)qm);
-                        const uint32_t mine = drop_bits(rm, (uint32_t)krow >> 1);
-                        const uint32_t other = (uint32_t)__builtin_amdgcn_mov_dpp((int)mine, 0xB1, 0xf, 0xf, true);
-                        MS[4 * g + e] = drop_pick(odd ? other : mine, odd, thr, p.drop_inv);
-                        MS[4 * g + e + 1] = drop_pick(odd ? mine : other, odd, thr, p.drop_inv);
-                    }
-                f32x16 Pd = S;
-#pragma unroll
-                for (int i = 0; i < 16; ++i) Pd[i] *= MS[i];
-                mma_second(dV, a, Pd);
-            } else {
-                mma_second(dV, a, S);
-            }
-            read_rows(a, doimg, sub * 32 + r, h);
-            f32x16 dP = mma_first(a, vbk);
-            if (p.drop_p > 0.f) {
-#pragma unroll
-                for (int i = 0; i < 16; ++i) dP[i] *= MS[i];
-            }
-#pragma unroll
-            for (int g = 0; g < 4; ++g) {
-                const f32x4 dl = *reinterpret_cast<const f32x4*>(dd + sub * 32 + 8 * g + 4 * h);
-#pragma unroll
-                for (int e = 0; e < 4; ++e) S[4 * g + e] = S[4 * g + e] * (dP[4 * g + e] - dl[e]);
-            }
-            read_tr(a, qimg, sub, lane);
-            mma_second(dK, a, S);
-        }
-        if (t + 1 < nt) {
-            store_lds(sQ + (cur ^ 1) * IMG, sq, tid);
-            store_lds(sdO + (cur ^ 1) * IMG, sdo, tid);
-            store_stats(cur ^ 1);
-        }
-        __syncthreads();
-    }
-    h16_t* dKo = reinterpret_cast<h16_t*>(p.dk) + (int64_t)b * p.Lk * p.lddk + hh * p.dh;
-    h16_t* dVo = reinterpret_cast<h16_t*>(p.dv) + (int64_t)b * p.Lk * p.lddv + hh * p.dh;
-    store_acc(dK, dKo, p.lddk, krow, kvalid, p.dh, h, p.premul != 0.f ? p.scale / p.premul : p.scale);
-    store_acc(dV, dVo, p.lddv, krow, kvalid, p.dh, h, 1.f);
-}
-
-__device__ __forceinline__ f32x16 splat16(float x) {
-    f32x16 z;
-#pragma unroll
-    for (int i = 0; i < 16; ++i) z[i] = x;
-    return z;
-}
-__device__ __forceinline__ f32x16 mma_first_c(const uint4 (&a)[2], const uint4 (&b)[2], const f32x16& c0) {
-    f32x16 acc;
-    asm("s_nop 1\n\tv_mfma_f32_32x32x16_" SVOL_H16_ASM " %0, %1, %2, %3"
-        : "=&v"(acc)
-        : "v"(__builtin_bit_cast(h16x8, a[0])), "v"(__builtin_bit_cast(h16x8, b[0])), "v"(c0));
-    return SVOL_MFMA_32x32x16_H16(__builtin_bit_cast(h16x8, a[1]), __builtin_bit_cast(h16x8, b[1]), acc, 0, 0,
-                                                   0);
-}
-__device__ __forceinline__ f32x16 rows16(const float* v, int sub, int h) {
-    f32x16 z;
-
-#pragma unroll
-    for (int g = 0; g < 4; ++g) {
-        const f32x4 t = *reinterpret_cast<const f32x4*>(v + sub * 32 + 8 * g + 4 * h);
-#pragma unroll
-        for (int e = 0; e < 4; ++e) z[4 * g + e] = t[e];
-    }
-    return z;
-}
-
 __device__ __forceinline__ void block_coords(const Args& p, int& xt, int& hh, int& b) {
     if (p.head_xcd) {
         const int id = blockIdx.x, xcd = id & 7, slot = id >> 3;
@@ -699,6 +204,508 @@
         hh = blockIdx.y;
         b = blockIdx.z;
     }
+}
+__device__ __forceinline__ void block_coords_uniform(const Args& p, int& xt, int& hh, int& b) {
+    block_coords(p, xt, hh, b);
+    xt = __builtin_amdgcn_readfirstlane(xt);
+    hh = __builtin_amdgcn_readfirstlane(hh);
+    b = __builtin_amdgcn_readfirstlane(b);
+}
+
+template <bool MASKED>
+__global__ __launch_bounds__(256, 2) void attn_fwd_bf16(Args p) {
+    const uint64_t dseed = drop_seed_at(p.drop_seed, p.drop_step);
+    __shared__ __attribute__((aligned(16))) char smem[4 * IMG + 2 * KT * 4];
+    char* sK = smem;
+    char* sV = smem + 2 * IMG;
+    float* sB = reinterpret_cast<float*>(smem + 4 * IMG);
+
+    const int tid = threadIdx.x, lane = tid & 63, wave = tid >> 6;
+    const int r = lane & 31, h = lane >> 5;
+    int xt, hh, b;
+    block_coords_uniform(p, xt, hh, b);
+    const int qt = xt / p.ksplit, sp = xt % p.ksplit;
+    const int qrow = qt * 128 + wave * 32 + r;
+    const bool qvalid = qrow < p.Lq;
+    const h16_t* Q = reinterpret_cast<const h16_t*>(p.q) + (int64_t)b * p.Lq * p.ldq + hh * p.dh;
+    const h16_t* K = reinterpret_cast<const h16_t*>(p.k) + (int64_t)b * p.Lk * p.ldk + hh * p.dh;
+    const h16_t* V = reinterpret_cast<const h16_t*>(p.v) + (int64_t)b * p.Lk * p.ldv + hh * p.dh;
+    const float* kb = p.kbias ? p.kbias + (int64_t)b * p.Lk : nullptr;
+    const float c = p.premul != 0.f ? 1.f : p.scale * LOG2E;
+
+    uint4 qb[2];
+    load_lane_block(qb, Q, p.ldq, qrow, qvalid, p.dh, h);
+
+    float m = -INFINITY, l = 0.f;
+    f32x16 O = zero16();
+
+    const int t0 = sp * p.tiles_per_split;
+    const int nt = min((p.Lk + KT - 1) / KT, t0 + p.tiles_per_split);
+    Stage sk, sv;
+    load_regs(sk, K, p.ldk, t0 * KT, p.Lk, p.dh, tid);
+    load_regs(sv, V, p.ldv, t0 * KT, p.Lk, p.dh, tid);
+    store_lds(sK, sk, tid);
+    store_lds(sV, sv, tid);
+    if (MASKED) stage_bias(sB, kb, t0 * KT, p.Lk, tid);
+    __syncthreads();
+
+    for (int t = t0; t < nt; ++t) {
+        const int cur = (t - t0) & 1;
+        if (t + 1 < nt) {
+            load_regs(sk, K, p.ldk, (t + 1) * KT, p.Lk, p.dh, tid);
+            load_regs(sv, V, p.ldv, (t + 1) * KT, p.Lk, p.dh, tid);
+        }
+        const char* kimg = sK + cur * IMG;
+        const char* vimg = sV + cur * IMG;
+        const float* bias = sB + cur * KT;
+        f32x16 S[4];
+#pragma unroll
+        for (int sub = 0; sub < 4; ++sub) {
+            uint4 ka[2];
+            read_rows(ka, kimg, sub * 32 + r, h);
+            S[sub] = mma_first(ka, qb);
+        }
+        mfma_results_ready(S[0], S[1], S[2], S[3]);
+        if (MASKED) {
+#pragma unroll
+            for (int sub = 0; sub < 4; ++sub)
+#pragma unroll
+                for (int g = 0; g < 4; ++g) {
+                    const f32x4 bb = *reinterpret_cast<const f32x4*>(bias + sub * 32 + 8 * g + 4 * h);
+#pragma unroll
+                    for (int e = 0; e < 4; ++e) S[sub][4 * g + e] = S[sub][4 * g + e] * c + bb[e];
+                }
+        }
+        float ml[4];
+#pragma unroll
+        for (int sub = 0; sub < 4; ++sub) {
+            float mm = max3(S[sub][0], S[sub][1], S[sub][2]);
+#pragma unroll
+            for (int i = 3; i < 15; i += 2) mm = max3(mm, S[sub][i], S[sub][i + 1]);
+            ml[sub] = max3(mm, S[sub][15], mm);
+        }
+        float mloc = max3(ml[0], ml[1], fmaxf(ml[2], ml[3]));
+        {
+            const HalfPair sw = swap_halves(__builtin_bit_cast(unsigned, mloc));
+            mloc = fmaxf(__builtin_bit_cast(float, sw.lo), __builtin_bit_cast(float, sw.hi));
+        }
+        const float thr = MASKED ? LAZY_THR : LAZY_THR / c;
+        if (__any(mloc > m + thr)) {
+            const float m_new = fmaxf(m, mloc);
+            const float m_use = (m_new == -INFINITY) ? 0.f : m_new;
+            const float alpha = __builtin_amdgcn_exp2f(MASKED ? (m - m_use) : (m - m_use) * c);
+            l *= alpha;
+#pragma unroll
+            for (int i = 0; i < 16; ++i) O[i] *= alpha;
+            m = m_new;
+        }
+        const float m_use = (m == -INFINITY) ? 0.f : m;
+        const float mc = MASKED ? -m_use : -m_use * c;
+        float ls[4] = {0.f, 0.f, 0.f, 0.f};
+#pragma unroll
+        for (int sub = 0; sub < 4; ++sub)
+#pragma unroll
+            for (int i = 0; i < 16; ++i) {
+                S[sub][i] = __builtin_amdgcn_exp2f(MASKED ? S[sub][i] + mc : __builtin_fmaf(S[sub][i], c, mc));
+                ls[sub] += S[sub][i];
+            }
+        l += (ls[0] + ls[1]) + (ls[2] + ls[3]);
+        if (p.drop_p > 0.f) {
+            const uint32_t rm = drop_row(drop_seed32(dseed), (((uint64_t)b * p.H + hh) * p.Lq + (qvalid ? qrow : 0)));
+            const uint32_t thr = drop_thr16(p.drop_p);
+#pragma unroll
+            for (int sub = 0; sub < 4; ++sub)
+#pragma unroll
+                for (int g = 0; g < 4; ++g)
+#pragma unroll
+                    for (int e = 0; e < 4; e += 2) {
+                        float s0, s1;
+                        attn_drop2(rm, t * KT + sub * 32 + 8 * g + 4 * h + e, thr, p.drop_inv, s0, s1);
+                        S[sub][4 * g + e] *= s0;
+                        S[sub][4 * g + e + 1] *= s1;
+                    }
+        }
+#pragma unroll
+        for (int sub = 0; sub < 4; ++sub) {
+            uint4 va[2];
+            read_tr(va, vimg, sub, lane);
+            mma_second(O, va, S[sub]);
+        }
+        if (t + 1 < nt) {
+            store_lds(sK + (cur ^ 1) * IMG, sk, tid);
+            store_lds(sV + (cur ^ 1) * IMG, sv, tid);
+            if (MASKED) stage_bias(sB + (cur ^ 1) * KT, kb, (t + 1) * KT, p.Lk, tid);
+        }
+        __syncthreads();
+    }
+    const float lt = l + __shfl_xor(l, 32, 64);
+    const float m2 = MASKED ? m : m * c;
+    if (p.ksplit > 1) {
+        if (qvalid) {
+            float* wo = p.ws_o + (((int64_t)sp * p.B + b) * p.Lq + qrow) * (p.H * p.dh) + hh * p.dh;
+#pragma unroll
+            for (int g = 0; g < 4; ++g) {
+                const int d0 = 8 * g + 4 * h;
+                if (d0 < p.dh) *reinterpret_cast<f32x4*>(wo + d0) = f32x4{O[4 * g], O[4 * g + 1], O[4 * g + 2], O[4 * g + 3]};
+            }
+            if (h == 0) {
+                float* wm = p.ws_ml + ((((int64_t)sp * p.B + b) * p.H + hh) * p.Lq + qrow) * 2;
+                wm[0] = m2;
+                wm[1] = lt;
+            }
+        }
+        return;
+    }
+    const float inv = lt > 0.f ? 1.f / lt : 0.f;
+    h16_t* Oo = reinterpret_cast<h16_t*>(p.out_o) + (int64_t)b * p.Lq * p.ldo + hh * p.dh;
+    store_acc(O, Oo, p.ldo, qrow, qvalid, p.dh, h, inv);
+    if (qvalid && h == 0) p.lse2[((int64_t)b * p.H + hh) * p.Lq + qrow] = m2 + __builtin_amdgcn_logf(lt);
+}
+
+__global__ void attn_combine_bf16(Args p) {
+    const int64_t idx = (int64_t)blockIdx.x * blockDim.x + threadIdx.x;
+    const int64_t total = (int64_t)p.B * p.Lq * p.H;
+    if (idx >= total) return;
+    const int hh = (int)(idx % p.H);
+    const int64_t row = idx / p.H;
+    const int b = (int)(row / p.Lq), q = (int)(row % p.Lq);
+    float M = -INFINITY;
+    for (int i = 0; i < p.ksplit; ++i) M = fmaxf(M, p.ws_ml[((((int64_t)i * p.B + b) * p.H + hh) * p.Lq + q) * 2]);
+    float L = 0.f, acc[32];
+#pragma unroll
+    for (int d = 0; d < 32; ++d) acc[d] = 0.f;
+    for (int i = 0; i < p.ksplit; ++i) {
+        const float* ml = p.ws_ml + ((((int64_t)i * p.B + b) * p.H + hh) * p.Lq + q) * 2;
+        if (ml[0] == -INFINITY) continue;
+        const float w = __builtin_amdgcn_exp2f(ml[0] - M);
+        L += w * ml[1];
+        const float* po = p.ws_o + (((int64_t)i * p.B + b) * p.Lq + q) * (p.H * p.dh) + hh * p.dh;
+#pragma unroll
+        for (int d = 0; d < 32; d += 4) {
+            if (d < p.dh) {
+                const f32x4 t = *reinterpret_cast<const f32x4*>(po + d);
+#pragma unroll
+                for (int e = 0; e < 4; ++e) acc[d + e] += w * t[e];
+            }
+        }
+    }
+    const float inv = L > 0.f ? 1.f / L : 0.f;
+    h16_t* o = reinterpret_cast<h16_t*>(p.out_o) + row * p.ldo + hh * p.dh;
+#pragma unroll
+    for (int d = 0; d < 32; d += 4) {
+        if (d < p.dh) {
+            h16x4 v;
+#pragma unroll
+            for (int e = 0; e < 4; ++e) v[e] = (h16_t)(acc[d + e] * inv);
+            *reinterpret_cast<h16x4*>(o + d) = v;
+        }
+    }
+    p.lse2[((int64_t)b * p.H + hh) * p.Lq + q] = M + __builtin_amdgcn_logf(L);
+}
+
+__global__ void attn_delta_bf16(Args p) {
+    const int64_t idx = (int64_t)blockIdx.x * blockDim.x + threadIdx.x;
+    const int64_t total = (int64_t)p.B * p.Lq * p.H;
+    if (idx >= total) return;
+    const int hh = (int)(idx % p.H);
+    const int64_t row = idx / p.H;
+    const int b = (int)(row / p.Lq), q = (int)(row % p.Lq);
+    const h16_t* o = reinterpret_cast<const h16_t*>(p.o) + row * p.ldo + hh * p.dh;
+    const h16_t* d = reinterpret_cast<const h16_t*>(p.d_o) + row * p.lddo + hh * p.dh;
+    float s = 0.f;
+    for (int i = 0; i < p.dh; i += 8) {
+        const h16x8 a = *reinterpret_cast<const h16x8*>(o + i), c = *reinterpret_cast<const h16x8*>(d + i);
+#pragma unroll
+        for (int e = 0; e < 8; ++e) s += (float)a[e] * (float)c[e];
+    }
+    p.delta[((int64_t)b * p.H + hh) * p.Lq + q] = s;
+    if (p.ksplit > 1) {
+        float* z = p.ws_dq + row * (p.H * p.dh) + hh * p.dh;
+        for (int i = 0; i < p.dh; i += 4) *reinterpret_cast<f32x4*>(z + i) = f32x4{0.f, 0.f, 0.f, 0.f};
+    }
+}
+
+__global__ void attn_dq_finish_bf16(Args p) {
+    const int64_t idx = (int64_t)blockIdx.x * blockDim.x + threadIdx.x;
+    const int64_t total = (int64_t)p.B * p.Lq * p.H;
+    if (idx >= total) return;
+    const int hh = (int)(idx % p.H);
+    const int64_t row = idx / p.H;
+    const float* z = p.ws_dq + row * (p.H * p.dh) + hh * p.dh;
+    h16_t* o = reinterpret_cast<h16_t*>(p.dq) + row * p.lddq + hh * p.dh;
+    for (int i = 0; i < p.dh; i += 4) {
+        const f32x4 t = *reinterpret_cast<const f32x4*>(z + i);
+        h16x4 v;
+#pragma unroll
+        for (int e = 0; e < 4; ++e) v[e] = (h16_t)(t[e] * p.scale);
+        *reinterpret_cast<h16x4*>(o + i) = v;
+    }
+}
+
+template <bool MASKED>
+__global__ __launch_bounds__(256, 2) void attn_bwd_dq_bf16(Args p) {
+    const uint64_t dseed = drop_seed_at(p.drop_seed, p.drop_step);
+    __shared__ __attribute__((aligned(16))) char smem[4 * IMG + 2 * KT * 4];
+    char* sK = smem;
+    char* sV = smem + 2 * IMG;
+    float* sB = reinterpret_cast<float*>(smem + 4 * IMG);
+
+    const int tid = threadIdx.x, lane = tid & 63, wave = tid >> 6;
+    const int r = lane & 31, h = lane >> 5;
+    const int b = blockIdx.z, hh = blockIdx.y;
+    const int qt = blockIdx.x / p.ksplit, sp = blockIdx.x % p.ksplit;
+    const int qrow = qt * 128 + wave * 32 + r;
+    const bool qvalid = qrow < p.Lq;
+    const h16_t* Q = reinterpret_cast<const h16_t*>(p.q) + (int64_t)b * p.Lq * p.ldq + hh * p.dh;
+    const h16_t* dO = reinterpret_cast<const h16_t*>(p.d_o) + (int64_t)b * p.Lq * p.lddo + hh * p.dh;
+    const h16_t* K = reinterpret_cast<const h16_t*>(p.k) + (int64_t)b * p.Lk * p.ldk + hh * p.dh;
+    const h16_t* V = reinterpret_cast<const h16_t*>(p.v) + (int64_t)b * p.Lk * p.ldv + hh * p.dh;
+    const float* kb = p.kbias ? p.kbias + (int64_t)b * p.Lk : nullptr;
+    const float c = p.premul != 0.f ? 1.f : p.scale * LOG2E;
+
+    uint4 qb[2], dob[2];
+    load_lane_block(qb, Q, p.ldq, qrow, qvalid, p.dh, h);
+    load_lane_block(dob, dO, p.lddo, qrow, qvalid, p.dh, h);
+    const int64_t sidx = ((int64_t)b * p.H + hh) * p.Lq + qrow;
+    const float nlse = qvalid ? -p.lse2[sidx] : -INFINITY;
+    const float dl = qvalid ? p.delta[sidx] : 0.f;
+
+    f32x16 dQ = zero16();
+    const int t0 = sp * p.tiles_per_split;
+    const int nt = min((p.Lk + KT - 1) / KT, t0 + p.tiles_per_split);
+    Stage sk, sv;
+    load_regs(sk, K, p.ldk, t0 * KT, p.Lk, p.dh, tid);
+    load_regs(sv, V, p.ldv, t0 * KT, p.Lk, p.dh, tid);
+    store_lds(sK, sk, tid);
+    store_lds(sV, sv, tid);
+    if (MASKED) stage_bias(sB, kb, t0 * KT, p.Lk, tid);
+    __syncthreads();
+
+    for (int t = t0; t < nt; ++t) {
+        const int cur = (t - t0) & 1;
+        if (t + 1 < nt) {
+            load_regs(sk, K, p.ldk, (t + 1) * KT, p.Lk, p.dh, tid);
+            load_regs(sv, V, p.ldv, (t + 1) * KT, p.Lk, p.dh, tid);
+        }
+        const char* kimg = sK + cur * IMG;
+        const char* vimg = sV + cur * IMG;
+        const float* bias = sB + cur * KT;
+#pragma unroll 2
+        for (int sub = 0; sub < 4; ++sub) {
+            uint4 a[2];
+            read_rows(a, kimg, sub * 32 + r, h);
+            f32x16 S = mma_first(a, qb);
+            read_rows(a, vimg, sub * 32 + r, h);
+            f32x16 dP = mma_first(a, dob);
+            if (p.drop_p > 0.f) {
+                const uint32_t rm = drop_row(drop_seed32(dseed), (((uint64_t)b * p.H + hh) * p.Lq + (qvalid ? qrow : 0)));
+                const uint32_t thr = drop_thr16(p.drop_p);
+#pragma unroll
+                for (int g = 0; g < 4; ++g)
+#pragma unroll
+                    for (int e = 0; e < 4; e += 2) {
+                        float s0, s1;
+                        attn_drop2(rm, t * KT + sub * 32 + 8 * g + 4 * h + e, thr, p.drop_inv, s0, s1);
+                        dP[4 * g + e] *= s0;
+                        dP[4 * g + e + 1] *= s1;
+                    }
+            }
+            if (MASKED) {
+#pragma unroll
+                for (int g = 0; g < 4; ++g) {
+                    const f32x4 bb = *reinterpret_cast<const f32x4*>(bias + sub * 32 + 8 * g + 4 * h);
+#pragma unroll
+                    for (int e = 0; e < 4; ++e) {
+                        const float pe = __builtin_amdgcn_exp2f(__builtin_fmaf(S[4 * g + e], c, bb[e] + nlse));
+                        S[4 * g + e] = pe * (dP[4 * g + e] - dl);
+                    }
+                }
+            } else {
+#pragma unroll
+                for (int i = 0; i < 16; ++i) {
+                    const float pe = __builtin_amdgcn_exp2f(__builtin_fmaf(S[i], c, nlse));
+                    S[i] = pe * (dP[i] - dl);
+                }
+            }
+            read_tr(a, kimg, sub, lane);
+            mma_second(dQ, a, S);
+        }
+        if (t + 1 < nt) {
+            store_lds(sK + (cur ^ 1) * IMG, sk, tid);
+            store_lds(sV + (cur ^ 1) * IMG, sv, tid);
+            if (MASKED) stage_bias(sB + (cur ^ 1) * KT, kb, (t + 1) * KT, p.Lk, tid);
+        }
+        __syncthreads();
+    }
+    if (p.ksplit > 1) {
+        if (qvalid) {
+            float* z = p.ws_dq + ((int64_t)b * p.Lq + qrow) * (p.H * p.dh) + hh * p.dh;
+#pragma unroll
+            for (int g = 0; g < 4; ++g) {
+                const int d0 = 8 * g + 4 * h;
+                if (d0 < p.dh) {
+#pragma unroll
+                    for (int e = 0; e < 4; ++e) atomicAdd(z + d0 + e, dQ[4 * g + e]);
+                }
+            }
+        }
+        return;
+    }
+    h16_t* dQo = reinterpret_cast<h16_t*>(p.dq) + (int64_t)b * p.Lq * p.lddq + hh * p.dh;
+    store_acc(dQ, dQo, p.lddq, qrow, qvalid, p.dh, h, p.scale);
+}
+
+template <bool KBIAS>
+__global__ __launch_bounds__(256, 2) void attn_bwd_dkdv_bf16(Args p) {
+    const uint64_t dseed = drop_seed_at(p.drop_seed, p.drop_step);
+    __shared__ __attribute__((aligned(16))) char smem[4 * IMG + 4 * KT * 4];
+    char* sQ = smem;
+    char* sdO = smem + 2 * IMG;
+    float* sL = reinterpret_cast<float*>(smem + 4 * IMG);
+    float* sD = sL + 2 * KT;
+
+    const int tid = threadIdx.x, lane = tid & 63, wave = tid >> 6;
+    const int r = lane & 31, h = lane >> 5;
+    const int b = blockIdx.z, hh = blockIdx.y;
+    const int krow = blockIdx.x * 128 + wave * 32 + r;
+    const bool kvalid = krow < p.Lk;
+    const h16_t* Q = reinterpret_cast<const h16_t*>(p.q) + (int64_t)b * p.Lq * p.ldq + hh * p.dh;
+    const h16_t* dO = reinterpret_cast<const h16_t*>(p.d_o) + (int64_t)b * p.Lq * p.lddo + hh * p.dh;
+    const h16_t* K = reinterpret_cast<const h16_t*>(p.k) + (int64_t)b * p.Lk * p.ldk + hh * p.dh;
+    const h16_t* V = reinterpret_cast<const h16_t*>(p.v) + (int64_t)b * p.Lk * p.ldv + hh * p.dh;
+    const float c = p.premul != 0.f ? 1.f : p.scale * LOG2E;
+    const float kbl = kvalid ? (p.kbias ? p.kbias[(int64_t)b * p.Lk + krow] * LOG2E : 0.f) : -INFINITY;
+    const float* lse_g = p.lse2 + ((int64_t)b * p.H + hh) * p.Lq;
+    const float* dl_g = p.delta + ((int64_t)b * p.H + hh) * p.Lq;
+
+    uint4 kbk[2], vbk[2];
+    load_lane_block(kbk, K, p.ldk, krow, kvalid, p.dh, h);
+    load_lane_block(vbk, V, p.ldv, krow, kvalid, p.dh, h);
+
+    f32x16 dK = zero16(), dV = zero16();
+    const int nt = (p.Lq + KT - 1) / KT;
+    Stage sq, sdo;
+    float rl = 0.f, rd = 0.f;
+    auto load_stats = [&](int row0) {
+        if (tid < KT) {
+            const int qi = row0 + tid;
+            rl = qi < p.Lq ? -lse_g[qi] : -INFINITY;
+            rd = qi < p.Lq ? dl_g[qi] : 0.f;
+        }
+    };
+    auto store_stats = [&](int buf) {
+        if (tid < KT) { sL[buf * KT + tid] = rl; sD[buf * KT + tid] = rd; }
+    };
+    load_regs(sq, Q, p.ldq, 0, p.Lq, p.dh, tid);
+    load_regs(sdo, dO, p.lddo, 0, p.Lq, p.dh, tid);
+    load_stats(0);
+    store_lds(sQ, sq, tid);
+    store_lds(sdO, sdo, tid);
+    store_stats(0);
+    __syncthreads();
+
+    for (int t = 0; t < nt; ++t) {
+        const int cur = t & 1;
+        if (t + 1 < nt) {
+            load_regs(sq, Q, p.ldq, (t + 1) * KT, p.Lq, p.dh, tid);
+            load_regs(sdo, dO, p.lddo, (t + 1) * KT, p.Lq, p.dh, tid);
+            load_stats((t + 1) * KT);
+        }
+        const char* qimg = sQ + cur * IMG;
+        const char* doimg = sdO + cur * IMG;
+        const float* nl = sL + cur * KT;
+        const float* dd = sD + cur * KT;
+#pragma unroll 1
+        for (int sub = 0; sub < 4; ++sub) {
+            uint4 a[2];
+            read_rows(a, qimg, sub * 32 + r, h);
+            f32x16 S = mma_first(a, kbk);
+#pragma unroll
+            for (int g = 0; g < 4; ++g) {
+                const f32x4 ls = *reinterpret_cast<const f32x4*>(nl + sub * 32 + 8 * g + 4 * h);
+#pragma unroll
+                for (int e = 0; e < 4; ++e)
+                    S[4 * g + e] = __builtin_amdgcn_exp2f(__builtin_fmaf(S[4 * g + e], c, KBIAS ? kbl + ls[e] : ls[e]));
+            }
+            read_tr(a, doimg, sub, lane);
+            f32x16 MS;
+#pragma unroll
+            for (int i = 0; i < 16; ++i) MS[i] = 1.f;
+            if (p.drop_p > 0.f) {
+                const uint32_t s0 = drop_seed32(dseed), thr = drop_thr16(p.drop_p), odd = (uint32_t)lane & 1u;
+                const uint64_t rbase = ((uint64_t)b * p.H + hh) * p.Lq;
+                const bool rows32 = rbase + (uint64_t)p.Lq <= 0xffffffffull;
+#pragma unroll
+                for (int g = 0; g < 4; ++g)
+#pragma unroll
+                    for (int e = 0; e < 4; e += 2) {
+                        const int q0 = t * KT + sub * 32 + 8 * g + 4 * h + e;
+                        const int qm = min(q0 + (int)odd, p.Lq - 1);
+                        const uint32_t rm = rows32 ? (s0 ^ (((uint32_t)rbase + (uint32_t)qm) * 0x9E3779B1u)) : drop_row(s0, rbase + (uint64_t)qm);
+                        const uint32_t mine = drop_bits(rm, (uint32_t)krow >> 1);
+                        const uint32_t other = (uint32_t)__builtin_amdgcn_mov_dpp((int)mine, 0xB1, 0xf, 0xf, true);
+                        MS[4 * g + e] = drop_pick(odd ? other : mine, odd, thr, p.drop_inv);
+                        MS[4 * g + e + 1] = drop_pick(odd ? mine : other, odd, thr, p.drop_inv);
+                    }
+                f32x16 Pd = S;
+#pragma unroll
+                for (int i = 0; i < 16; ++i) Pd[i] *= MS[i];
+                mma_second(dV, a, Pd);
+            } else {
+                mma_second(dV, a, S);
+            }
+            read_rows(a, doimg, sub * 32 + r, h);
+            f32x16 dP = mma_first(a, vbk);
+            if (p.drop_p > 0.f) {
+#pragma unroll
+                for (int i = 0; i < 16; ++i) dP[i] *= MS[i];
+            }
+#pragma unroll
+            for (int g = 0; g < 4; ++g) {
+                const f32x4 dl = *reinterpret_cast<const f32x4*>(dd + sub * 32 + 8 * g + 4 * h);
+#pragma unroll
+                for (int e = 0; e < 4; ++e) S[4 * g + e] = S[4 * g + e] * (dP[4 * g + e] - dl[e]);
+            }
+            read_tr(a, qimg, sub, lane);
+            mma_second(dK, a, S);
+        }
+        if (t + 1 < nt) {
+            store_lds(sQ + (cur ^ 1) * IMG, sq, tid);
+            store_lds(sdO + (cur ^ 1) * IMG, sdo, tid);
+            store_stats(cur ^ 1);
+        }
+        __syncthreads();
+    }
+    h16_t* dKo = reinterpret_cast<h16_t*>(p.dk) + (int64_t)b * p.Lk * p.lddk + hh * p.dh;
+    h16_t* dVo = reinterpret_cast<h16_t*>(p.dv) + (int64_t)b * p.Lk * p.lddv + hh * p.dh;
+    store_acc(dK, dKo, p.lddk, krow, kvalid, p.dh, h, p.premul != 0.f ? p.scale / p.premul : p.scale);
+    store_acc(dV, dVo, p.lddv, krow, kvalid, p.dh, h, 1.f);
+}
+
+__device__ __forceinline__ f32x16 splat16(float x) {
+    f32x16 z;
+#pragma unroll
+    for (int i = 0; i < 16; ++i) z[i] = x;
+    return z;
+}
+__device__ __forceinline__ f32x16 mma_first_c(const uint4 (&a)[2], const uint4 (&b)[2], const f32x16& c0) {
+    f32x16 acc;
+    asm("s_nop 1\n\tv_mfma_f32_32x32x16_" SVOL_H16_ASM " %0, %1, %2, %3"
+        : "=&v"(acc)
+        : "v"(__builtin_bit_cast(h16x8, a[0])), "v"(__builtin_bit_cast(h16x8, b[0])), "v"(c0));
+    return SVOL_MFMA_32x32x16_H16(__builtin_bit_cast(h16x8, a[1]), __builtin_bit_cast(h16x8, b[1]), acc, 0, 0,
+                                                   0);
+}
+__device__ __forceinline__ f32x16 rows16(const float* v, int sub, int h) {
+    f32x16 z;
+
+#pragma unroll
+    for (int g = 0; g < 4; ++g) {
+        const f32x4 t = *reinterpret_cast<const f32x4*>(v + sub * 32 + 8 * g + 4 * h);
+#pragma unroll
+        for (int e = 0; e < 4; ++e) z[4 * g + e] = t[e];
+    }
+    return z;
 }
 
 __device__ __forceinline__ unsigned split_bf16x2(float x) {
@@ -1431,7 +1438,8 @@
     float* sRed = reinterpret_cast<float*>(smem);
     const int tid = threadIdx.x, lane = tid & 63, wave = tid >> 6;
     const int r = lane & 31, h = lane >> 5;
-    const int b = blockIdx.z, hh = blockIdx.y;
+    int xt, hh, b;
+    block_coords_uniform(p, xt, hh, b);
     const h16_t* Q = reinterpret_cast<const h16_t*>(p.q) + (int64_t)b * p.Lq * p.ldq + hh * 32;
     const h16_t* dO = reinterpret_cast<const h16_t*>(p.d_o) + (int64_t)b * p.Lq * p.lddo + hh * 32;
     const h16_t* K = reinterpret_cast<const h16_t*>(p.k) + (int64_t)b * p.Lk * p.ldk + hh * 32;
@@ -1442,7 +1450,7 @@
     const float kmul = p.premul != 0.f ? p.scale / p.premul : p.scale;
     const int nsub = (p.Lq + 31) >> 5;
     const int ntk = (p.Lk + KT - 1) / KT;
-    const int t0 = blockIdx.x * p.tiles_per_split, t1 = min(ntk, t0 + p.tiles_per_split);
+    const int t0 = xt * p.tiles_per_split, t1 = min(ntk, t0 + p.tiles_per_split);
     Stage st;
     {
         Stage sq, sdo;
@@ -2431,7 +2439,7 @@
     Fwd fwd; Bwd bwd;
     int ntk, fwd_ksplit, fwd_tps, bwd_ksplit, bwd_tps;
     Grid gf, gq, gk;
-    int fq_tps; dim3 fq_grid;
+    int fq_tps; Grid fq_grid;
     int64_t need_cls, need_redo, need_sp, need_ksplit, need;
 };
 static Plan attn_plan(int B, int H, int Lq, int Lk, int dh, bool premul, bool kbias, bool dropout, bool ws, int64_t ws_bytes,
@@ -2452,11 +2460,13 @@
     pl.fwd_ksplit = (ws && !pl.pre) ? plan_ksplit(B, H, Lq, Lk, dh, ws_bytes / 4, &pl.fwd_tps) : 1;
     pl.bwd_ksplit = det ? 1 : pl.fwd_ksplit;
     pl.bwd_tps = det ? ntk : pl.fwd_tps;
-    const int hx = (pl.pre && (B * H) % 8 == 0) ? (((B * H) % 16 == 0 && H % 2 == 0 && dh == 32) ? 2 : 1) : 0;
-    auto grid = [&](int nx) {
-        return hx ? Grid{dim3((unsigned)(B * H * nx)), hx, nx, 0} : Grid{dim3((unsigned)nx, (unsigned)H, (unsigned)B), 0, 0, 0};
+    const int xcd_deal = (B * H) % 8 == 0 ? (((B * H) % 16 == 0 && H % 2 == 0 && dh == 32) ? 2 : 1) : 0;
+    const int hx = pl.pre ? xcd_deal : 0;
+    auto grid_of = [&](int deal, int nx) {
+        return deal ? Grid{dim3((unsigned)(B * H * nx)), deal, nx, 0} : Grid{dim3((unsigned)nx, (unsigned)H, (unsigned)B), 0, 0, 0};
     };
-    pl.gf = grid(nq128 * pl.fwd_ksplit);
+    auto grid = [&](int nx) { return grid_of(hx, nx); };
+    pl.gf = grid_of(xcd_deal, nq128 * pl.fwd_ksplit);
     pl.gq = pl.pre ? grid((Lq + 255) / 256) : grid(nq128 * pl.bwd_ksplit);
     if (hx) pl.gq.tail_last = (Lq % 256 >= 1 && Lq % 256 <= 128 && pl.gq.nxt > 1) ? 1 : 0;
     pl.gk = grid((Lk + 127) / 128);
@@ -2472,7 +2482,7 @@
     else pl.bwd = pl.masked ? Bwd::two_pass_m : Bwd::two_pass_u;
     const int chunks = min(ntk, max(1, 512 / (B * H)));
     pl.fq_tps = (ntk + chunks - 1) / chunks;
-    pl.fq_grid = dim3((unsigned)((ntk + pl.fq_tps - 1) / pl.fq_tps), (unsigned)H, (unsigned)B);
+    pl.fq_grid = grid_of(xcd_deal, (ntk + pl.fq_tps - 1) / pl.fq_tps);
     return pl;
 }
 static Plan attn_plan(const AttnCall& c) {
@@ -2563,9 +2573,8 @@
     case Bwd::bwd_pre: dq = attn_bwd_dq_bf16_pre, dkdv = attn_bwd_dkdv_bf16_pre; break;
     case Bwd::fq_m:
     case Bwd::fq_u: {
-        Args pf = pq;
-        pf.tiles_per_split = pl.fq_tps;
-        hipLaunchKernelGGL(pl.bwd == Bwd::fq_m ? attn_bwd_fq_bf16<true> : attn_bwd_fq_bf16<false>, pl.fq_grid, wg, 0, s, pf);
+        const Args pf = make_args(c, pl.bwd_ksplit, pl.fq_tps, pl.fq_grid);
+        hipLaunchKernelGGL(pl.bwd == Bwd::fq_m ? attn_bwd_fq_bf16<true> : attn_bwd_fq_bf16<false>, pl.fq_grid.dim, wg, 0, s, pf);
         hipLaunchKernelGGL(attn_dq_finish_bf16, gd, wg, 0, s, pq);
         break;
     }
diff --git a/svol_amd/csrc/gemm_ws_bf16.hip b/svol_amd/csrc/gemm_ws_bf16.hip
--- a/svol_amd/csrc/gemm_ws_bf16.hip
+++ b/svol_amd/csrc/gemm_ws_bf16.hip
@@ -6,7 +6,7 @@
     const h16_t* A; const h16_t* W; void* C;
     const float* bias; const float* colscale; h16_t* pre; const void* res; const h16_t* aux; float* colsum;
     int64_t lda, ldw, ldc, ldp, ldr, ldaux;
-    int M, N, act, tiles_per_wg, nchunk;
+    int M, N, act, tiles_per_wg, nchunk, ncg;
 };
 
 typedef __attribute__((address_space(3))) void* lds_void_ptr;
@@ -35,6 +35,13 @@
 template <> struct WsCfg<1> { static constexpr int SLOT = A_PLANE + TR * 256 * 4, STG = 3, ND = 6; };
 template <> struct WsCfg<2> { static constexpr int SLOT = 2 * A_PLANE, STG = 4, ND = 4; };
 
+struct WsWork { int chunk, cg; };
+__device__ __forceinline__ WsWork ws_work(const WsArgs& p) {
+    const int id = blockIdx.x, slot = id >> 3, g8 = slot / p.ncg;
+    return WsWork{g8 * 8 + (id & 7), slot - g8 * p.ncg};
+}
+static inline int64_t ws_grid(int64_t nchunk, int64_t ncg) { return ncg == 1 ? nchunk : (nchunk + 7) / 8 * 8 * ncg; }
+
 template <int MODE>
 __device__ __forceinline__ void gemm_ws_body(const WsArgs& p) {
     constexpr int SLOT = WsCfg<MODE>::SLOT, STG = WsCfg<MODE>::STG, ND = WsCfg<MODE>::ND;
@@ -42,7 +49,9 @@
     const int tid = threadIdx.x, lane = tid & 63;
     const int wave = __builtin_amdgcn_readfirstlane(tid >> 6);
     const int fr = lane & 15, fq = lane >> 4;
-    const int chunk_id = blockIdx.x % p.nchunk, cg = blockIdx.x / p.nchunk;
+    const WsWork wk = ws_work(p);
+    if (wk.chunk >= p.nchunk) return;
+    const int chunk_id = wk.chunk, cg = wk.cg;
     const int cg0 = cg * 256;
     const int c0 = cg0 + wave * 64;
     const bool active = c0 < p.N;
@@ -295,7 +304,9 @@
     const int tid = threadIdx.x, lane = tid & 63;
     const int wave = __builtin_amdgcn_readfirstlane(tid >> 6);
     const int fr = lane & 15, fq = lane >> 4;
-    const int chunk_id = blockIdx.x % p.nchunk, cg = blockIdx.x / p.nchunk;
+    const WsWork wk = ws_work(p);
+    if (wk.chunk >= p.nchunk) return;
+    const int chunk_id = wk.chunk, cg = wk.cg;
     const int cg0 = cg * 256;
     const int c0 = cg0 + wave * 64;
     const bool active = c0 < p.N;
@@ -569,10 +580,10 @@
         const int64_t t8 = (ntile + n8 - 1) / n8;
         if (t8 >= 1 && (ntile + t8 - 1) / t8 == n8) { tpw = t8; nchunk = n8; }
     }
-    if (nchunk * ncg > (1ll << 30)) return SVOL_E_UNSUPPORTED;
+    if (ws_grid(nchunk, ncg) > (1ll << 30)) return SVOL_E_UNSUPPORTED;
     p = WsArgs{(const h16_t*)c.A, (const h16_t*)c.B, c.C, c.bias, c.colscale, (h16_t*)c.pre, c.res, (const h16_t*)c.aux, c.colsum,
-               c.lda, c.ldb, c.ldc, c.ldp, c.ldr, c.ldaux, (int)M, (int)N, act, (int)tpw, (int)nchunk};
-    grid = dim3((unsigned)(ncg * nchunk));
+               c.lda, c.ldb, c.ldc, c.ldp, c.ldr, c.ldaux, (int)M, (int)N, act, (int)tpw, (int)nchunk, (int)ncg};
+    grid = dim3((unsigned)ws_grid(nchunk, ncg));
     kern = mode == 0 ? gemm_ws_bf16_m0 : (mode == 1 ? gemm_ws_bf16_m1 : gemm_ws_bf16_m2);
     if (mode == 0) {
         if (act == SVOL_ACT_NONE && !c.pre) kern = c.colscale ? gemm_wsp_bf16_none_scale : gemm_wsp_bf16_none;
```

Result: no change. 15490, median of 6 (+0.5%).
